# ParsaEsmati/SEA

Hardware: AMD Instinct MI355X
Metric: rollout steps/sec (full-context forward, recompute mode) on cylinder_flow-shaped fields (higher is better)
Workload: dtype bf16

## Files before the change

include/sea_hip.h:

```cpp
#ifndef SEA_HIP_H
#define SEA_HIP_H

#include <stddef.h>
#include <stdint.h>

#ifdef __cplusplus
extern "C" {
#endif

#define SEA_ABI_VERSION 8

enum { SEA_F32 = 0, SEA_BF16 = 1 };

enum {
    SEA_OK = 0,
    SEA_EINVAL = -1,
    SEA_ELAUNCH = -2,
    SEA_EUNSUPPORTED = -3
};

int sea_abi_version(void);
const char* sea_last_error(void);
const char* sea_last_form(int* a, int* b);
int sea_struct_sizes(int* out, int cap);
// ... 368 lines not shown
    int64_t p_stride;
    int32_t S, M, N, ldp, ldr, ldc32, ldcact;
    float bias_scale;
} SeaSplitkGroup;
int sea_splitk_finish(const SeaSplitkGroup* groups, int n_groups, int dtype, void* stream);

#define SEA_MAX_AQKV_GROUPS 4
typedef struct {
    const float* X;
    const float* cond;
    const float* w1;
    const float* b1;
    const void* W2c;
    const float* b2c;
    const float* gamma;
    const float* beta;
    const void* Wqkv;
    const float* bqkv;
    void* Q;
    void* K;
    void* Vt;
    int32_t ldx, ldw2c, ldw, M, E, N3;
    const float* w13;
    const float* b13;
    const void* W3;
    const float* b3;
    void* mod3;
    int32_t ldw3, ldmod3;
    uint32_t* memo_stamps;
    void* memo_mods;
    const uint32_t* memo_epoch;
    int32_t* memo_count;
    uint32_t* memo_rows;
    int32_t ldmemo, pad_;
} SeaAdalnQkv;
int sea_adaln_qkv(const SeaAdalnQkv* groups, int n_groups, const SeaQkvCommon* common, const SeaGemmGroup* riders, int n_riders, const SeaSiluGroup* silu, int n_silu,
                  const float* silu_c, int silu_M, const SeaIbParams* ib, float eps, int dtype, void* stream);

#define SEA_CHAIN_MAX_PROJ 6
#define SEA_CHAIN_MAX_GROUPS 3
typedef struct {
    const void* att[SEA_XTAIL_MAX_SEG];
    const void* Wp[SEA_XTAIL_MAX_SEG];
    const void* a2;
    const void* W2;
    const float* b2;
    const float* Xin;
    float* X;
    void* Xact;
    int32_t n_seg, ldatt, ldwp, lda2, ldw2, ldxin, ldx, ldxact;
    int32_t M, D, E, has_down, n_proj;
    float bias_scale;
    SeaGemmNormGroup down;
    SeaQkvGroup proj[SEA_CHAIN_MAX_PROJ];
} SeaRowChain;

int sea_row_chain(const SeaRowChain* params, int n_groups, const SeaQkvCommon* common, float eps, int dtype, void* stream);
struct SeaIbParams_;
int sea_row_chain_riders(const SeaRowChain* params, int n_groups, const SeaQkvCommon* common, const SeaGemmGroup* riders, int n_riders, int tile0, int n_tiles,
                         const struct SeaIbParams_* ib, float eps, int dtype, void* stream);

enum { SEA_OP_GEMM = 1, SEA_OP_QKV = 2, SEA_OP_ATTN = 3, SEA_OP_NORM = 4, SEA_OP_SILU = 5, SEA_OP_IB = 6, SEA_OP_CONVERT = 8, SEA_OP_GEMM_NORM = 9, SEA_OP_XTAIL = 10, SEA_OP_MLP1 = 11, SEA_OP_MLP2 = 13, SEA_OP_GEMM_FEW = 14, SEA_OP_QKV_FEW = 15, SEA_OP_CHAIN = 16, SEA_OP_ADALN = 17, SEA_OP_MLPB = 18, SEA_OP_AQKV = 19, SEA_OP_SPLITK = 20 };
typedef struct {
    int32_t op, n, dtype, i0, i1, i2, i3;
    float f0;
    const void* p0;
    const void* p1;
    int64_t l0, l1, l2, l3;
} SeaLaunchRec;
int sea_run_list(const SeaLaunchRec* recs, int n_recs, void* stream);

typedef struct {
    void* addr;
    int32_t kind;
    int32_t pad_;
    int64_t base, stride;
} SeaStepPatch;
int sea_run_list_steps(const SeaLaunchRec* recs, int n_recs, const SeaStepPatch* patches, int n_patches, int step0, int n_steps, void* stream);

int sea_unpatchify(const float* in, int64_t sb, int64_t sp, int64_t sf, int64_t sc, const int32_t* index_map, const int32_t* point_slot,
                   const float* scale, const float* shift, float* out, int B, int P, int F, int C, int n_points, void* stream);

int sea_patchify(const float* in, const int32_t* index_map, const float* scale, const float* shift, float* out, int64_t sb, int64_t sp, int64_t sf,
                 int64_t sc, int B, int P, int F, int C_map, int C_out, int n_points, float pad_value, void* stream);

#define SEA_KV_MAX_FIELDS 4
typedef struct {
    const float* gamma;
    const float* beta;
    const void* mod;
    int32_t ldmod, pad_;
} SeaKvNorm;
typedef struct {
// ... 258 lines not shown
```

sea_amd/_native.py:

```python
from __future__ import annotations

import ctypes as C
import os
from typing import Optional

import torch

_HERE = os.path.dirname(os.path.abspath(__file__))
LIB_PATH = os.path.join(_HERE, "csrc", "libsea_hip.so")

SEA_F32, SEA_BF16 = 0, 1
ABI_VERSION = 8
MAX_GROUPS = 16
CTL_GRAD_NORM, CTL_CLIP, CTL_INV_BC1, CTL_INV_SQRT_BC2, CTL_APPLIED, CTL_STEP, CTL_SKIPPED, CTL_CLIPPED, CTL_WORDS = range(9)
MAX_ATTN_PROBLEMS = 8
MAX_NORM_GROUPS = 16
MAX_SILU_GROUPS = 24

_vp, _i32, _i64, _f32 = C.c_void_p, C.c_int32, C.c_int64, C.c_float


class SeaDropout(C.Structure):
    _fields_ = [("seed", C.c_uint32), ("stream", C.c_uint32), ("thr", _i32), ("mode", _i32)]

# ... 84 lines not shown

class SeaLaunchRec(C.Structure):
    _fields_ = [("op", _i32), ("n", _i32), ("dtype", _i32), ("i0", _i32), ("i1", _i32), ("i2", _i32), ("i3", _i32), ("f0", _f32),
                ("p0", _vp), ("p1", _vp), ("l0", _i64), ("l1", _i64), ("l2", _i64), ("l3", _i64)]

MAX_GEMM_NORM_GROUPS = 8


class SeaGemmNormGroup(C.Structure):
    _fields_ = [("A", _vp), ("W", _vp), ("bias", _vp), ("R", _vp), ("C32", _vp), ("mod", _vp), ("gamma", _vp), ("beta", _vp),
                ("Y32", _vp), ("Yact", _vp), ("mean", _vp), ("rstd", _vp),
                ("lda", _i32), ("ldw", _i32), ("ldr", _i32), ("ldc32", _i32), ("ldmod", _i32), ("ldy32", _i32), ("ldyact", _i32),
                ("M", _i32), ("N", _i32), ("K", _i32),
                ("n_seg", _i32), ("a_seg_stride", _i64), ("bias_scale", _f32), ("ldcact", _i32), ("Cact", _vp),
                ("ib_c", _vp), ("ib_w1", _vp), ("ib_b1", _vp), ("ib_lnw", _vp), ("ib_lnb", _vp), ("ib_w2", _vp), ("ib_b2", _vp),
                ("ib_h", _i32), ("pad_", _i32)]


XTAIL_MAX_SEG = 4
XTAIL_MAX_GROUPS = 4
MAX_SILU_IB = 4


class SeaExchangeTail(C.Structure):
    _fields_ = [("att", _vp * XTAIL_MAX_SEG), ("Wp", _vp * XTAIL_MAX_SEG), ("Wup", _vp), ("bup", _vp), ("X", _vp), ("Xact", _vp),
                ("n_seg", _i32), ("ldatt", _i32), ("ldwp", _i32), ("ldwup", _i32), ("ldx", _i32), ("ldxact", _i32),
                ("M", _i32), ("D", _i32), ("E", _i32), ("has_down", _i32), ("bias_scale", _f32),
                ("down", SeaGemmNormGroup)]


CHAIN_MAX_PROJ = 6
CHAIN_MAX_GROUPS = 3
CHAIN_MAX_RIDERS = 8


class SeaRowChain(C.Structure):
    _fields_ = [("att", _vp * XTAIL_MAX_SEG), ("Wp", _vp * XTAIL_MAX_SEG), ("a2", _vp), ("W2", _vp), ("b2", _vp), ("Xin", _vp), ("X", _vp), ("Xact", _vp),
                ("n_seg", _i32), ("ldatt", _i32), ("ldwp", _i32), ("lda2", _i32), ("ldw2", _i32), ("ldxin", _i32), ("ldx", _i32), ("ldxact", _i32),
                ("M", _i32), ("D", _i32), ("E", _i32), ("has_down", _i32), ("n_proj", _i32), ("bias_scale", _f32),
                ("down", SeaGemmNormGroup), ("proj", SeaQkvGroup * CHAIN_MAX_PROJ)]


MAX_ADALN_GROUPS = 16


class SeaAdalnGroup(C.Structure):
    _fields_ = [("A", _vp), ("W", _vp), ("bias", _vp), ("X", _vp), ("gamma", _vp), ("beta", _vp), ("Yact", _vp), ("Y32", _vp), ("mean", _vp), ("rstd", _vp),
                ("lda", _i32), ("ldw", _i32), ("ldx", _i32), ("ldyact", _i32), ("ldy32", _i32), ("M", _i32), ("d", _i32), ("K", _i32)]


MAX_SPLITK_GROUPS = 8


class SeaEncBlock(C.Structure):
    _fields_ = [(n, _vp) for n in ("Zin", "Zout", "wqkv", "bqkv", "wo", "w1", "b1", "lnw", "lnb", "w2", "b2", "g1", "g2", "dZout", "dZin",
                                   "n1", "dqkv", "att", "dz1", "n2", "dh", "hg", "dz2", "u1", "u2", "u3w", "u3b", "ws")] + \
                [("ws_floats", _i64), ("B", _i32), ("P", _i32), ("W", _i32), ("H", _i32), ("eps", _f32), ("pad_", _i32)]


class SeaSplitkGroup(C.Structure):
    _fields_ = [("P", _vp), ("bias", _vp), ("R", _vp), ("C32", _vp), ("Cact", _vp), ("p_stride", _i64), ("S", _i32), ("M", _i32), ("N", _i32), ("ldp", _i32),
                ("ldr", _i32), ("ldc32", _i32), ("ldcact", _i32), ("bias_scale", _f32)]


MAX_AQKV_GROUPS = 4
AQKV_MAX_SILU = 8
# ... 188 lines not shown
    L.sea_rownorm.argtypes = [C.POINTER(SeaNormGroup), C.c_int, C.c_int, C.c_int, C.c_int, C.c_int, C.c_float, C.c_int, _vp]
    L.sea_gemm_fewrows.argtypes = [C.POINTER(SeaGemmGroup), C.POINTER(SeaNormGroup), C.c_int, C.c_int, C.c_int, C.c_float, C.c_int, _vp]
    L.sea_gemm_fewrows.restype = C.c_int
    L.sea_qkv_rope_fewrows.argtypes = [C.POINTER(SeaQkvGroup), C.POINTER(SeaNormGroup), C.c_int, C.POINTER(SeaQkvCommon), C.c_float, C.c_int, _vp]
    L.sea_qkv_rope_fewrows.restype = C.c_int
    L.sea_silu_outer.argtypes = [C.POINTER(SeaSiluGroup), C.c_int, _vp, C.c_int, C.c_int, _vp]
    L.sea_ib_add.argtypes = [C.POINTER(SeaIbParams), _vp]
    L.sea_convert_f32_to_act.argtypes = [_vp, _i64, _vp, _i64, _i64, _i64, C.c_int, _vp]
    L.sea_selftest_mfma.restype = C.c_int
    L.sea_wgrad_grouped.argtypes = [C.POINTER(SeaWgradGroup), C.c_int, C.c_int, _vp]
    L.sea_transpose_weights.argtypes = [_vp, _vp, C.c_int, _vp, _vp, C.c_int, C.c_int, _vp]
    L.sea_rownorm_bwd.argtypes = [C.POINTER(SeaNormBwdGroup), C.c_int, C.c_int, C.c_int, C.c_int, C.c_int, C.c_int, C.c_int, C.c_int, _vp, _i64, _vp]
    L.sea_silu_outer_bwd.argtypes = [C.POINTER(SeaSiluBwdGroup), C.c_int, _vp, C.c_int, C.c_int, _vp, _i64, _vp]
    L.sea_ib_bwd.argtypes = [C.POINTER(SeaIbBwdParams), _vp]
    L.sea_silu_outer_bwd_dc.argtypes = [C.POINTER(SeaSiluBwdGroup), C.c_int, _vp, _vp, C.c_int, C.c_int, _vp, _i64, _vp]
    L.sea_silu_outer_bwd_dc_ws_floats.argtypes = [C.POINTER(SeaSiluBwdGroup), C.c_int, C.c_int]
    L.sea_silu_outer_bwd_dc_ws_floats.restype = _i64
    L.sea_ib_bwd_dc.argtypes = [C.POINTER(SeaIbBwdParams), _vp, _vp]
    L.sea_attention_bwd.argtypes = [C.POINTER(SeaAttnBwdParams), C.c_int, _vp]
    L.sea_dropout_mask.argtypes = [_vp, _i64, _i64, C.c_uint32, C.c_uint32, _i32, _vp]
    L.sea_dropout_mask.restype = C.c_int
    L.sea_unpatchify.argtypes = [_vp, _i64, _i64, _i64, _i64, _vp, _vp, _vp, _vp, _vp, C.c_int, C.c_int, C.c_int, C.c_int, C.c_int, _vp]
    L.sea_unpatchify.restype = C.c_int
    L.sea_gemm_rownorm.argtypes = [C.POINTER(SeaGemmNormGroup), C.c_int, C.c_float, C.c_int, _vp]
    L.sea_gemm_rownorm.restype = C.c_int
    L.sea_exchange_tail.argtypes = [C.POINTER(SeaExchangeTail), C.c_int, C.c_float, C.c_int, _vp]
    L.sea_exchange_tail.restype = C.c_int
    L.sea_gemm_adaln.argtypes = [C.POINTER(SeaAdalnGroup), C.c_int, C.c_float, C.c_int, _vp]
    L.sea_gemm_adaln.restype = C.c_int
    L.sea_row_chain.argtypes = [C.POINTER(SeaRowChain), C.c_int, C.POINTER(SeaQkvCommon), C.c_float, C.c_int, _vp]
    L.sea_row_chain.restype = C.c_int
    L.sea_row_chain_riders.argtypes = [C.POINTER(SeaRowChain), C.c_int, C.POINTER(SeaQkvCommon), C.POINTER(SeaGemmGroup), C.c_int, C.c_int, C.c_int, C.POINTER(SeaIbParams), C.c_float, C.c_int, _vp]
    L.sea_row_chain_riders.restype = C.c_int
    L.sea_patchify.argtypes = [_vp, _vp, _vp, _vp, _vp, _i64, _i64, _i64, _i64, C.c_int, C.c_int, C.c_int, C.c_int, C.c_int, C.c_int, C.c_float, _vp]
    L.sea_patchify.restype = C.c_int
    L.sea_silu_outer_ib.argtypes = [C.POINTER(SeaSiluGroup), C.c_int, _vp, C.c_int, C.c_int, _vp, C.c_int, _vp]
    L.sea_silu_outer_ib.restype = C.c_int
    L.sea_mlp_fc1_ln_gelu.argtypes = [C.POINTER(SeaMlpGroup), C.c_int, C.c_float, C.c_int, _vp]
    L.sea_mlp_fc1_ln_gelu.restype = C.c_int
    L.sea_mlp_fc2_proj_norm.argtypes = [C.POINTER(SeaMlp2Group), C.c_int, C.c_float, C.c_int, _vp]
    L.sea_mlp_fc2_proj_norm.restype = C.c_int
    L.sea_mlp_block.argtypes = [C.POINTER(SeaMlpGroup), C.POINTER(SeaMlp2Group), C.c_int, C.c_float, C.c_int, _vp]
    L.sea_mlp_block.restype = C.c_int
    L.sea_adaln_qkv.argtypes = [C.POINTER(SeaAdalnQkv), C.c_int, C.POINTER(SeaQkvCommon), C.POINTER(SeaGemmGroup), C.c_int, C.POINTER(SeaSiluGroup), C.c_int, _vp, C.c_int,
                                C.POINTER(SeaIbParams), C.c_float, C.c_int, _vp]
    L.sea_adaln_qkv.restype = C.c_int
    L.sea_splitk_finish.argtypes = [C.POINTER(SeaSplitkGroup), C.c_int, C.c_int, _vp]
    L.sea_splitk_finish.restype = C.c_int
    L.sea_encoder_block_ws_floats.argtypes = [C.c_int, C.c_int, C.c_int]
    L.sea_encoder_block_ws_floats.restype = _i64
    for name in ("sea_encoder_block_fwd", "sea_encoder_block_bwd"):
        getattr(L, name).argtypes = [C.POINTER(SeaEncBlock), C.c_int, _vp]
        getattr(L, name).restype = C.c_int
    L.sea_run_list.argtypes = [C.POINTER(SeaLaunchRec), C.c_int, _vp]
    L.sea_run_list.restype = C.c_int
    L.sea_run_list_steps.argtypes = [C.POINTER(SeaLaunchRec), C.c_int, C.POINTER(SeaStepPatch), C.c_int, C.c_int, C.c_int, _vp]
    L.sea_run_list_steps.restype = C.c_int
    L.sea_kv_rollout.argtypes = [C.POINTER(SeaKvGlobal), C.POINTER(SeaKvLayer), C.c_int, C.c_int, C.c_uint32, C.c_int, _vp]
    L.sea_kv_rollout.restype = C.c_int
    L.sea_kv_arena_words.argtypes = [C.POINTER(SeaKvGlobal)]
    L.sea_kv_arena_words.restype = C.c_int64
    L.sea_kv_debug_stamps.argtypes = [_vp]
    L.sea_kv_debug_stamps.restype = None
    L.sea_kv_cache_fill.argtypes = [C.POINTER(SeaKvFill), C.c_int, C.c_int, _vp]
    L.sea_kv_cache_fill.restype = C.c_int
    L.sea_kv_cache_fork.argtypes = [C.POINTER(SeaKvFork), C.c_int, C.c_int, _vp]
# ... 26 lines not shown
    L.sea_ensemble_verify_ws_bytes.restype = _i64
    for name in ("sea_attention_bwd", "sea_wgrad_grouped", "sea_transpose_weights", "sea_rownorm_bwd", "sea_silu_outer_bwd", "sea_ib_bwd",
                 "sea_silu_outer_bwd_dc", "sea_ib_bwd_dc"):
        getattr(L, name).restype = C.c_int
    L.sea_mse_fwd_bwd.argtypes = [_vp, _vp, _vp, _vp, _vp, C.c_int, _i64, C.c_float, _vp]
    L.sea_relative_mse.argtypes = [_vp, _vp, _vp, _i64, C.c_int, _vp]
    L.sea_adamw_flat.argtypes = [_vp, _vp, _vp, _vp, _vp, C.c_int, _i64, C.c_float, C.c_float, C.c_float, C.c_float, C.c_float,
                                 C.c_int, C.c_float, _vp]
    L.sea_grad_norm_ctl.argtypes = [_vp, _i64, C.c_float, C.c_float, C.c_int, C.c_float, C.c_float, _vp, C.c_int, _vp, _vp]
    L.sea_adamw_flat_ctl.argtypes = [_vp, _vp, _vp, _vp, _vp, C.c_int, _i64, C.c_float, C.c_float, C.c_float, C.c_float, C.c_float,
                                     C.c_float, _vp, _vp]
    for name in ("sea_gemm_grouped", "sea_qkv_rope_grouped", "sea_attention_fwd", "sea_rownorm", "sea_silu_outer",
                 "sea_ib_add", "sea_convert_f32_to_act", "sea_device_info", "sea_mse_fwd_bwd", "sea_relative_mse",
                 "sea_adamw_flat", "sea_grad_norm_ctl", "sea_adamw_flat_ctl"):
        getattr(L, name).restype = C.c_int
    if L.sea_abi_version() != ABI_VERSION:
        raise NativeLibraryError(f"{LIB_PATH}: ABI version {L.sea_abi_version()} != {ABI_VERSION}; rebuild (python -m sea_amd.build --force)")
    _lib = L
    return L


ABI_STRUCTS = (SeaGemmGroup, SeaQkvGroup, SeaQkvCommon, SeaAttnProblem, SeaAttnParams, SeaNormGroup, SeaSiluGroup,
               SeaIbParams, SeaWgradGroup, SeaNormBwdGroup, SeaSiluBwdGroup, SeaIbBwdParams, SeaAttnBwdProblem, SeaAttnBwdParams,
               SeaDropout, SeaLaunchRec, SeaGemmNormGroup, SeaExchangeTail, SeaMlpGroup, SeaMlp2Group, SeaKvNorm, SeaKvField, SeaKvPair, SeaKvLayer, SeaKvGlobal, SeaStepPatch, SeaRowChain, SeaAdalnGroup, SeaAdalnQkv, SeaSplitkGroup, SeaEncBlock,
               SeaKvFill, SeaKvFork)

EXPORTED_SYMBOLS = (
    "sea_abi_version", "sea_last_error", "sea_last_form", "sea_struct_sizes", "sea_device_info", "sea_gemm_grouped", "sea_qkv_rope_grouped",
    "sea_attention_fwd", "sea_rownorm", "sea_silu_outer", "sea_ib_add", "sea_convert_f32_to_act", "sea_selftest_mfma",
    "sea_mse_fwd_bwd", "sea_relative_mse", "sea_adamw_flat", "sea_grad_norm_ctl", "sea_adamw_flat_ctl",
    "sea_wgrad_grouped", "sea_transpose_weights", "sea_rownorm_bwd", "sea_silu_outer_bwd", "sea_ib_bwd",
    "sea_attention_bwd", "sea_dropout_mask", "sea_run_list", "sea_run_list_steps", "sea_unpatchify", "sea_gemm_rownorm", "sea_exchange_tail", "sea_patchify", "sea_silu_outer_ib", "sea_mlp_fc1_ln_gelu", "sea_mlp_fc2_proj_norm", "sea_kv_rollout", "sea_kv_arena_words", "sea_kv_debug_stamps",
    "sea_kv_cache_fill", "sea_kv_cache_fork", "sea_kv_cache_gather", "sea_decode_mse", "sea_decode_member_sse", "sea_decode_member_moments", "sea_decode_sensor_sse", "sea_decode_sensor_grad", "sea_resample_systematic", "sea_enkf_transform", "sea_enkf_transform_gram", "sea_decode_member_gram", "sea_ensemble_mix", "sea_ensemble_verify", "sea_ensemble_verify_ws_bytes",
    "sea_gemm_fewrows", "sea_qkv_rope_fewrows", "sea_row_chain", "sea_row_chain_riders", "sea_gemm_adaln", "sea_mlp_block", "sea_adaln_qkv", "sea_splitk_finish",
    "sea_encoder_block_ws_floats", "sea_encoder_block_fwd", "sea_encoder_block_bwd",
    "sea_silu_outer_bwd_dc", "sea_silu_outer_bwd_dc_ws_floats", "sea_ib_bwd_dc",
)


def check(rc: int, what: str = "") -> None:
    if rc != 0:
        msg = lib().sea_last_error()
        raise RuntimeError(f"libsea_hip {what} failed (code {rc}): {msg.decode() if msg else '?'}")


def dtype_code(dt: torch.dtype) -> int:
    if dt == torch.float32:
        return SEA_F32
    if dt == torch.bfloat16:
        return SEA_BF16
    raise ValueError(f"sea_amd: activation dtype must be float32 or bfloat16, got {dt}")


def require_gpu(t: torch.Tensor, name: str = "tensor") -> None:
    if not t.is_cuda:
        raise RuntimeError(
            f"sea_amd: {name} is on {t.device}; this path runs only on an MI355X through libsea_hip.so "
            "(no CPU fallback — the CPU oracle lives under oracle/ for tests only)")


def require_same_operand(out: torch.Tensor, target: torch.Tensor, what: str, f32: bool = False) -> None:
    if target.shape != out.shape:
        raise ValueError(f"sea_amd: {what}: target shape {tuple(target.shape)} does not match output shape {tuple(out.shape)}")
    if target.device != out.device:
        raise ValueError(f"sea_amd: {what}: target is on {target.device}, output on {out.device}")
    if f32 and target.dtype != torch.float32:
        raise ValueError(f"sea_amd: {what}: target dtype {target.dtype} must be torch.float32 (output shape {tuple(out.shape)})")
# ... 9 lines not shown
```

sea_amd/csrc/adaln_qkv.hip:

```cpp
#include "gemm_tile.hpp"
#include "ib_rows.hpp"
#include <stdlib.h>

#define SEA_AQKV_MAX_SILU 8

struct AqkvLaunch {
    SeaAdalnQkv g[SEA_MAX_AQKV_GROUPS];
    int tile_start[SEA_MAX_AQKV_GROUPS + 1];
    int n_groups;
    float eps;
    SeaQkvCommon c;
    ChainRiderPod rg[SEA_CHAIN_MAX_RIDERS];
    int n_riders, rider_n;
    SeaSiluGroup sg[SEA_AQKV_MAX_SILU];
    int n_silu, silu_wgs, ib_wgs, M_r;
    const float* cond_r;
    SeaIbParams ib;
    unsigned long long* stamps;
    int probe;
};
static_assert(sizeof(AqkvLaunch) <= 4096, "kernel arguments of sea_adaln_qkv");

static unsigned long long* g_aqkv_stamps = nullptr;
extern "C" void sea_aqkv_debug_stamps(unsigned long long* buf) { g_aqkv_stamps = buf; }
// ... 43 lines not shown
};

template <bool HAS3>
__global__ __launch_bounds__(512) void adaln_qkv_kernel(const AqkvLaunch L) {
    using T = __bf16;
    using C = AqkvCfg;
    constexpr int E = C::E, KC = C::KC, BM = C::BM, NW = C::NW, KTA = C::KTA, KTB = C::KTB;
    extern __shared__ __attribute__((aligned(16))) char smem[];
    const int total = L.tile_start[L.n_groups];
    if ((int)blockIdx.x >= total + L.rider_n) {
        const int x = (int)blockIdx.x - total - L.rider_n;
        const int lane_ = threadIdx.x & 63, wave_ = threadIdx.x >> 6;
        uint32_t* rst = L.g[0].memo_stamps != nullptr ? L.g[0].memo_rows : nullptr;
        uint32_t r_c = 0, r_e = 0;
        int r_row = -1;
        if (rst != nullptr) {
            const int per_g_ = (L.M_r + 63) >> 6;
            const int set = x < L.silu_wgs ? x / per_g_ : L.n_silu;
            const int b0 = (x < L.silu_wgs ? x - set * per_g_ : x - L.silu_wgs) * 64;
            rst += (int64_t)set * L.M_r * 2;
            int ok = 1;
            if (wave_ == 0 && b0 + lane_ < L.M_r) {
                r_row = b0 + lane_;
                r_c = __float_as_uint(L.cond_r[r_row]);
                r_e = *L.g[0].memo_epoch;
                const uint2 st = reinterpret_cast<const uint2*>(rst)[r_row];
                ok = st.x == r_c && st.y == r_e;
            }
            const int all_ok = __all(ok);
            if (threadIdx.x == 0) *reinterpret_cast<int*>(smem) = all_ok;
            __syncthreads();
            const bool r_hit = __builtin_amdgcn_readfirstlane(*reinterpret_cast<const int*>(smem)) != 0;
            if (L.g[0].memo_count != nullptr && threadIdx.x == 0) atomicAdd(L.g[0].memo_count + (r_hit ? 0 : 1), 1);
            if (r_hit) return;
            if (r_row >= 0) reinterpret_cast<uint2*>(rst)[r_row] = make_uint2(r_c, r_e);
        }
        if (x < L.silu_wgs) {
            const int per_g = (L.M_r + 63) >> 6;
            const int gy = x / per_g;
            const SeaSiluGroup& S = L.sg[gy];
            const int row0 = (x - gy * per_g) * 64 + wave_ * 8;
            if (row0 >= L.M_r) return;
            float cv[8];
#pragma unroll
            for (int i = 0; i < 8; ++i) cv[i] = L.cond_r[row0 + i < L.M_r ? row0 + i : L.M_r - 1];
            T* out = static_cast<T*>(S.Hid) + (int64_t)row0 * S.ld;
            for (int k = lane_ * 4; k < S.K2; k += 256) {
                float w[4], bb[4];
                load4(S.w1 + k, w);
                load4(S.b1 + k, bb);
#pragma unroll
                for (int i = 0; i < 8; ++i) {
                    if (row0 + i < L.M_r)
                        store4(out + (int64_t)i * S.ld + k, silu_f(w[0] * cv[i] + bb[0]), silu_f(w[1] * cv[i] + bb[1]), silu_f(w[2] * cv[i] + bb[2]), silu_f(w[3] * cv[i] + bb[3]));
                }
            }
        } else {
            const int row0 = (x - L.silu_wgs) * 64 + wave_ * 8;
            for (int i = 0; i < 8; ++i) {
                const int row = row0 + i;
                if (row < L.ib.M) ib_store_row(L.ib, L.cond_r[row], row, lane_);
            }
        }
        return;
    }
    if ((int)blockIdx.x >= total) {
// ... 474 lines not shown
    if (memo && !hit && wave == 0 && lane < 32 && m0 + lane < M) reinterpret_cast<uint2*>(G.memo_stamps)[m0 + lane] = make_uint2(my_c, my_e);
}

extern "C" int sea_adaln_qkv(const SeaAdalnQkv* groups, int n_groups, const SeaQkvCommon* common, const SeaGemmGroup* riders, int n_riders, const SeaSiluGroup* silu, int n_silu,
                             const float* silu_c, int silu_M, const SeaIbParams* ib, float eps, int dtype, void* stream) {
    SEA_REQUIRE(groups != nullptr && common != nullptr && n_groups >= 1 && n_groups <= SEA_MAX_AQKV_GROUPS, "sea_adaln_qkv: n_groups=%d out of range", n_groups);
    const int E = groups[0].E;
    if (dtype != SEA_BF16 || E != AqkvCfg::E || common->H * common->hd != E || (common->hd != 32 && common->hd != 16)) {
        sea_set_error("sea_adaln_qkv: unsupported dtype / shape (dtype=%d E=%d H=%d hd=%d): bf16, E = 256, head dim 16 or 32, H * hd = E", dtype, E, common->H, common->hd);
        return SEA_EUNSUPPORTED;
    }
    SEA_REQUIRE(common->rope && common->T >= 1 && common->cap >= common->pos0 + common->T && common->pos0 >= 0 && common->cap % 8 == 0, "sea_adaln_qkv: bad rotary table / cache geometry (T=%d pos0=%d cap=%d)",
                common->T, common->pos0, common->cap);
    AqkvLaunch L;
    memset(&L, 0, sizeof(L));
    const bool memo_count = sea_tune("memo_count", 0) != 0;
    int total = 0;
    for (int i = 0; i < n_groups; ++i) {
        const SeaAdalnQkv& G = groups[i];
        SEA_REQUIRE(G.E == E && G.M >= 1 && G.M % common->T == 0, "sea_adaln_qkv[%d]: the groups of a launch share E; M = B * T", i);
        SEA_REQUIRE(G.X && G.cond && G.w1 && G.b1 && G.W2c && G.gamma && G.Wqkv && G.Q && G.K && G.Vt, "sea_adaln_qkv[%d]: null pointer", i);
        SEA_REQUIRE(G.ldx % 4 == 0 && G.ldx >= E && G.ldw2c % 8 == 0 && G.ldw2c >= 2 * E && G.ldw % 8 == 0 && G.ldw >= E, "sea_adaln_qkv[%d]: bad strides", i);
        SEA_REQUIRE(sea_aligned16(G.X) && sea_aligned16(G.w1) && sea_aligned16(G.b1) && sea_aligned16(G.W2c) && sea_aligned16(G.b2c) && sea_aligned16(G.gamma) && sea_aligned16(G.beta) &&
                        sea_aligned16(G.Wqkv) && sea_aligned16(G.bqkv) && sea_aligned16(G.Q) && sea_aligned16(G.K) && sea_aligned16(G.Vt),
                    "sea_adaln_qkv[%d]: pointers must be 16-byte aligned", i);
        SEA_REQUIRE((int64_t)(G.M / common->T) * common->H * common->cap * common->hd < (1ll << 31), "sea_adaln_qkv[%d]: attention tensors must stay below 2^31 elements", i);
        if (G.W3 != nullptr) {
            SEA_REQUIRE(G.w13 && G.b13 && G.mod3 && G.N3 == AqkvCfg::K3 && G.ldw3 % 8 == 0 && G.ldw3 >= G.N3 && G.ldmod3 % 8 == 0 && G.ldmod3 >= G.N3 && sea_aligned16(G.w13) && sea_aligned16(G.b13) &&
                            sea_aligned16(G.W3) && sea_aligned16(G.b3) && sea_aligned16(G.mod3),
                        "sea_adaln_qkv[%d]: third layer: null / misaligned pointer, bad stride, or N3 = %d != 256", i, G.N3);
        }
        if (G.memo_stamps != nullptr) {
            SEA_REQUIRE(G.memo_mods && G.memo_epoch && G.ldmemo % 8 == 0 && G.ldmemo >= 2 * E && sea_aligned16(G.memo_mods) && ((uintptr_t)G.memo_stamps & 7) == 0 &&
                            ((uintptr_t)G.memo_epoch & 3) == 0 && ((uintptr_t)G.memo_count & 3) == 0 && ((uintptr_t)G.memo_rows & 7) == 0,
                        "sea_adaln_qkv[%d]: condition memo: null / misaligned pointer or bad stride (ldmemo=%d)", i, G.ldmemo);
        }
        L.g[i] = G;
        if (!memo_count) L.g[i].memo_count = nullptr;
        L.tile_start[i] = total;
        total += (G.M + 31) / 32;
    }
    L.tile_start[n_groups] = total;
    L.n_groups = n_groups;
    L.eps = eps;
    L.c = *common;
    SEA_REQUIRE(n_riders >= 0 && n_riders <= SEA_CHAIN_MAX_RIDERS && (n_riders == 0 || riders != nullptr), "sea_adaln_qkv: bad rider arguments");
    int rider_total = 0;
    for (int i = 0; i < n_riders; ++i) {
        const SeaGemmGroup& G = riders[i];
        SEA_REQUIRE(G.A && !G.silu_c && G.W && G.Cact && !G.C32 && !G.R && !G.Z && G.act == 0 && G.drop.thr == 0 && G.n_seg == 1, "sea_adaln_qkv: rider %d is not a plain bf16 group (A, W, bias, Cact only)", i);
        SEA_REQUIRE(G.M >= 1 && G.N >= 8 && G.N % 8 == 0 && G.K >= 64 && G.K % 64 == 0 && G.lda % 8 == 0 && G.lda >= G.K && G.ldw % 8 == 0 && G.ldw >= G.K && G.ldcact % 8 == 0 && G.ldcact >= G.N,
                    "sea_adaln_qkv: rider %d: bad shape M=%d N=%d K=%d (whole 64-wide K-tiles) lda=%d ldw=%d ldcact=%d", i, G.M, G.N, G.K, G.lda, G.ldw, G.ldcact);
        SEA_REQUIRE(sea_aligned16(G.A) && sea_aligned16(G.W) && sea_aligned16(G.bias) && sea_aligned16(G.Cact), "sea_adaln_qkv: rider %d: pointers must be 16-byte aligned", i);
        ChainRiderPod& R = L.rg[i];
        R.A = G.A; R.W = G.W; R.bias = G.bias; R.Cact = G.Cact;
        R.lda = G.lda; R.ldw = G.ldw; R.ldcact = G.ldcact; R.M = G.M; R.N = G.N; R.K = G.K;
        R.tile_start = rider_total;
        rider_total += ((G.M + 127) / 128) * ((G.N + 127) / 128);
    }
    L.n_riders = n_riders;
    L.rider_n = rider_total;
    SEA_REQUIRE(n_silu >= 0 && n_silu <= SEA_AQKV_MAX_SILU && (n_silu == 0 || (silu != nullptr && silu_c != nullptr && silu_M >= 1)), "sea_adaln_qkv: bad silu rider arguments (n_silu=%d)", n_silu);
    for (int i = 0; i < n_silu; ++i) {
        SEA_REQUIRE(silu[i].w1 && silu[i].b1 && silu[i].Hid && silu[i].K2 >= 4 && silu[i].K2 % 4 == 0 && silu[i].ld >= silu[i].K2 && silu[i].ld % 4 == 0 && sea_aligned16(silu[i].w1) &&
                        sea_aligned16(silu[i].b1) && sea_aligned16(silu[i].Hid),
                    "sea_adaln_qkv: silu rider %d: null / misaligned pointer or bad shape", i);
        L.sg[i] = silu[i];
// ... 33 lines not shown
```

sea_amd/csrc/chain.hip:

```cpp
#include "norm_epilogue.hpp"
#include "gemm_tile.hpp"
#include "ib_rows.hpp"
#include <stdlib.h>

struct ChainLaunch {
    SeaRowChain p[SEA_CHAIN_MAX_GROUPS];
    SeaQkvCommon c;
    float eps;
    int n_groups;
    unsigned long long* stamps;
    ChainRiderPod rg[SEA_CHAIN_MAX_RIDERS];
    int n_riders, rider_t0, rider_n, ib_wgs;
    SeaIbParams ib;
};
static_assert(sizeof(ChainLaunch) <= 4096, "kernel arguments of sea_row_chain");

static unsigned long long* g_chain_stamps = nullptr;
extern "C" void sea_chain_debug_stamps(unsigned long long* buf) { g_chain_stamps = buf; }

template <int D, int E, int MI>
struct ChainCfg {
    static constexpr int BM = 16 * MI, BKB = 128, BK = 64;
    static constexpr int KTD = D / BK, KTE = E / BK;
    static constexpr int AT_BYTES = BM * E * 2;
    static constexpr int YT_BYTES = BM * D * 2;
    static constexpr int WH_BYTES = E * D * 2;
    static constexpr int ROPE_BYTES = 2048;
    static constexpr int BIAS_BYTES = 4096;
    static constexpr int RED_BYTES = MI * 512;
    static constexpr int LDS_BYTES = AT_BYTES + YT_BYTES + 2 * WH_BYTES + ROPE_BYTES + BIAS_BYTES + RED_BYTES;
    static constexpr int SMAX = E / D;
    static constexpr int NI1 = D / 64, NI2 = E / 64, NI3 = D / 64, NI4 = 2 * D / 64;
    static_assert(E == 2 * D && LDS_BYTES <= 160 * 1024 && SMAX * D * D * 2 <= WH_BYTES && (KTE / 2) * E * BKB <= WH_BYTES && D * E * 2 <= WH_BYTES, "LDS plan of sea_row_chain");
};

__device__ __forceinline__ void glds16_x4(const void* p0, const void* p1, const void* p2, const void* p3, unsigned l0, unsigned l1, unsigned l2, unsigned l3) {
    unsigned keep;
    asm volatile(
        "s_mov_b32 %0, m0\n\t"
        "s_mov_b32 m0, %5\n\ts_nop 0\n\tglobal_load_lds_dwordx4 %1, off\n\t"
        "s_mov_b32 m0, %6\n\ts_nop 0\n\tglobal_load_lds_dwordx4 %2, off\n\t"
        "s_mov_b32 m0, %7\n\ts_nop 0\n\tglobal_load_lds_dwordx4 %3, off\n\t"
        "s_mov_b32 m0, %8\n\ts_nop 0\n\tglobal_load_lds_dwordx4 %4, off\n\t"
        "s_mov_b32 m0, %0"
        : "=&s"(keep) : "v"(p0), "v"(p1), "v"(p2), "v"(p3), "s"(l0), "s"(l1), "s"(l2), "s"(l3) : "memory");
}
// ... 98 lines not shown
    static constexpr const float* ib_b1 = nullptr;
    static constexpr const float* ib_lnw = nullptr;
    static constexpr const float* ib_lnb = nullptr;
    static constexpr const float* ib_w2 = nullptr;
    static constexpr const float* ib_b2 = nullptr;
    static constexpr int ib_h = 0, ldr = 0, ldc32 = 0, ldcact = 0;
    int M, ldmod, ldy32, ldyact;
    const float* bias;
    const void* mod;
    const float* gamma;
    const float* beta;
    float* Y32;
    void* Yact;
    float* mean;
    float* rstd;
};

template <int D, int E, int MI>
__global__ __launch_bounds__(256) void row_chain_kernel(const ChainLaunch L) {
    using T = __bf16;
    using C = ChainCfg<D, E, MI>;
    constexpr int BM = C::BM, KTD = C::KTD, KTE = C::KTE, NI1 = C::NI1, NI2 = C::NI2, NI3 = C::NI3, NI4 = C::NI4, SMAX = C::SMAX;
    constexpr int A_KTS = BM * 128;
    extern __shared__ __attribute__((aligned(16))) char smem[];
    const int tid = threadIdx.x, lane = tid & 63, wave = tid >> 6;
    const int r = lane & 15, g = lane >> 4;
    if ((int)blockIdx.y == L.n_groups) {
        const int x = blockIdx.x;
        if (x < L.rider_n) {
            const int tile = L.rider_t0 + x;
            int gi = 0;
            while (gi + 1 < L.n_riders && tile >= L.rg[gi + 1].tile_start) ++gi;
            const ChainRiderPod& R = L.rg[gi];
            ChainRiderGroup G;
            G.A = R.A; G.W = R.W; G.bias = R.bias; G.Cact = R.Cact;
            G.lda = R.lda; G.ldw = R.ldw; G.ldcact = R.ldcact; G.M = R.M; G.N = R.N; G.K = R.K;
            const int t = tile - R.tile_start;
            const int tiles_n = (R.N + 127) / 128;
            gemm_tile_body<T, 128, 128, true, true, false>(G, t / tiles_n, t % tiles_n, smem, 0);
        } else if (x < L.rider_n + L.ib_wgs) {
            const int row0 = (x - L.rider_n) * 64 + wave * 16;
            for (int i = 0; i < 16; ++i) {
                const int row = row0 + i;
                if (row < L.ib.M) ib_store_row(L.ib, L.ib.c[row], row, lane);
            }
        }
        return;
    }
    ChainParams pl;
    {
        const uint32_t* raw = reinterpret_cast<const uint32_t*>(&L.p[0]) + (size_t)blockIdx.y * (sizeof(SeaRowChain) / 4);
#pragma unroll
        for (int k = 0; k < 4; ++k) {
            const int dw = k * 64 + lane;
            pl.v[k] = dw < (int)(sizeof(SeaRowChain) / 4) ? raw[dw] : 0u;
        }
    }
    const int M = CP_I32(M), S = CP_I32(n_seg);
    const int m0 = blockIdx.x * BM;
    if (m0 >= M) return;
    unsigned long long* stp = L.stamps != nullptr ? L.stamps + (size_t)(blockIdx.y * gridDim.x + blockIdx.x) * 16 : nullptr;
    int stn = 0;
    auto stamp = [&]() {
        if (stp != nullptr && tid == 0 && stn < 16) stp[stn] = wall_clock64();
        ++stn;
    };
    stamp();
    char* AT = smem;
    char* YT = AT + C::AT_BYTES;
    char* WA = YT + C::YT_BYTES;
    char* WB = WA + C::WH_BYTES;
    float* s_rope = reinterpret_cast<float*>(WB + C::WH_BYTES);
    float* s_bias = reinterpret_cast<float*>(reinterpret_cast<char*>(s_rope) + C::ROPE_BYTES);
    float* red = reinterpret_cast<float*>(reinterpret_cast<char*>(s_bias) + C::BIAS_BYTES);
    const unsigned lds0 = __builtin_amdgcn_readfirstlane((unsigned)(uintptr_t)smem);
    const unsigned at_l = lds0, wa_l = lds0 + C::AT_BYTES + C::YT_BYTES, wb_l = wa_l + C::WH_BYTES;
    const int wv = __builtin_amdgcn_readfirstlane(wave);
    const T* W2 = CP_PTR(const T*, W2);
    const int ldw2 = CP_I32(ldw2);
    const bool has_down = CP_I32(has_down) != 0;
    const int n_proj = has_down ? CP_I32(n_proj) : 0;
    const T* Wd = CP_PTR(const T*, down.W);
    const int ldwd = CP_I32(down.ldw);

    if (S > 0) {
        const int ldatt = CP_I32(ldatt), ldwp = CP_I32(ldwp);
#pragma unroll
        for (int s = 0; s < SMAX; ++s) {
            if (s < S) {
                const T* att = reinterpret_cast<const T*>(cp_dyn_u64(pl, CP_DW(att) + 2 * s));
                const T* Wp = reinterpret_cast<const T*>(cp_dyn_u64(pl, CP_DW(Wp) + 2 * s));
                chain_dma_a(att, ldatt, m0, M - 1, BM, KTD, at_l + (unsigned)(s * KTD * A_KTS), wv, lane);
                chain_dma_w(Wp, ldwp, D, 0, KTD, wa_l + (unsigned)(s * D * D * 2), wv, lane);
            }
        }
        chain_dma_w(W2, ldw2, E, 0, KTD, wb_l, wv, lane);
    } else {
        chain_dma_a(CP_PTR(const T*, a2), CP_I32(lda2), m0, M - 1, BM, KTE, at_l, wv, lane);
        chain_dma_w(W2, ldw2, E, 0, KTE / 2, wa_l, wv, lane);
        chain_dma_w(W2, ldw2, E, (KTE / 2) * 64, KTE / 2, wb_l, wv, lane);
    }
    stamp();
    int mrow[MI];
    bool mok[MI];
#pragma unroll
    for (int i = 0; i < MI; ++i) {
        const int m = m0 + i * 16 + r;
        mok[i] = m < M;
        mrow[i] = mok[i] ? m : M - 1;
    }
    const float* b2 = CP_PTR(const float*, b2);
    const float* Xin = CP_PTR(const float*, Xin);
    const int ldxin = CP_I32(ldxin);
    const float bias_scale = CP_F32(bias_scale);
    float bv2[NI2][4], rv2[MI][NI2][4];
#pragma unroll
    for (int j = 0; j < NI2; ++j) {
        const int n = wave * (E / 4) + j * 16 + g * 4;
#pragma unroll
        for (int q = 0; q < 4; ++q) bv2[j][q] = 0.f;
        if (b2 != nullptr) load4(b2 + n, bv2[j]);
#pragma unroll
        for (int i = 0; i < MI; ++i) load4(Xin + (int64_t)mrow[i] * ldxin + n, rv2[i][j]);
    }
    ChainNormGroup<D, E> Gd;
    Gd.M = M;
    Gd.bias = CP_PTR(const float*, down.bias);
    Gd.mod = CP_PTR(const void*, down.mod);
    Gd.ldmod = CP_I32(down.ldmod);
    Gd.gamma = CP_PTR(const float*, down.gamma);
    Gd.beta = CP_PTR(const float*, down.beta);
    Gd.Y32 = CP_PTR(float*, down.Y32);
    Gd.ldy32 = CP_I32(down.ldy32);
    Gd.Yact = CP_PTR(void*, down.Yact);
    Gd.ldyact = CP_I32(down.ldyact);
    Gd.mean = CP_PTR(float*, down.mean);
    Gd.rstd = CP_PTR(float*, down.rstd);
    NormEpilogue<T, NI3, true, true, true> epi3[MI];
    if (has_down) {
#pragma unroll
        for (int i = 0; i < MI; ++i) epi3[i].prefetch(Gd, mrow[i], wave * (D / 4), g);
    }
    const int hd = L.c.hd, hd2 = hd >> 1, Tlen = L.c.T, pos0 = L.c.pos0;
    if (n_proj > 0) {
        for (int idx = tid; idx < BM * hd2; idx += 256) {
            const int i = idx / hd2, k = idx - i * hd2;
            int m = m0 + i;
            m = m < M ? m : M - 1;
            const int t = m % Tlen;
            const float2 cs = reinterpret_cast<const float2*>(L.c.rope)[(int64_t)(pos0 + t) * hd2 + k];
            reinterpret_cast<float2*>(s_rope)[idx] = cs;
        }
        int boff = 0;
        for (int e = 0; e < n_proj; ++e) {
            const int base = CP_DW(proj) + e * (int)(sizeof(SeaQkvGroup) / 4);
            const float* bias = reinterpret_cast<const float*>(cp_dyn_u64(pl, base + QK_DW(bias)));
            const int N = (int)cp_dyn_u32(pl, base + QK_DW(N));
            for (int n = tid; n < N; n += 256) s_bias[boff + n] = bias != nullptr ? bias[n] : 0.f;
            boff += N;
        }
    }
#pragma unroll
    for (int j = 0; j < NI2; ++j)
#pragma unroll
        for (int q = 0; q < 4; ++q) {
            touch(bv2[j][q]);
#pragma unroll
            for (int i = 0; i < MI; ++i) touch(rv2[i][j][q]);
        }
    if (has_down) {
#pragma unroll
        for (int i = 0; i < MI; ++i)
#pragma unroll
            for (int j = 0; j < NI3; ++j)
#pragma unroll
                for (int q = 0; q < 4; ++q) {
                    touch(epi3[i].bv[j][q]); touch(epi3[i].gm[j][q]); touch(epi3[i].bt[j][q]); touch(epi3[i].mw[j][q]); touch(epi3[i].mb[j][q]);
                }
    }
    stamp();
    asm volatile("s_waitcnt vmcnt(0)" ::: "memory");
    __syncthreads();
    stamp();

    f32x4 acc2[MI][NI2];
#pragma unroll
    for (int i = 0; i < MI; ++i)
#pragma unroll
        for (int j = 0; j < NI2; ++j) acc2[i][j] = f32x4{0.f, 0.f, 0.f, 0.f};
    if (S > 0) {
        float gsum[MI][NI1][4];
#pragma unroll
        for (int i = 0; i < MI; ++i)
#pragma unroll
            for (int j = 0; j < NI1; ++j)
#pragma unroll
                for (int q = 0; q < 4; ++q) gsum[i][j][q] = 0.f;
#pragma unroll
        for (int s = 0; s < SMAX; ++s) {
            if (s < S) {
                f32x4 acc1[MI][NI1];
#pragma unroll
                for (int i = 0; i < MI; ++i)
#pragma unroll
                    for (int j = 0; j < NI1; ++j) acc1[i][j] = f32x4{0.f, 0.f, 0.f, 0.f};
                chain_mma<MI, NI1>(AT + s * KTD * A_KTS, A_KTS, WA + s * D * D * 2, D * 128, wave * (D / 4), KTD, NI1, r, g, acc1);
#pragma unroll
                for (int i = 0; i < MI; ++i)
#pragma unroll
                    for (int j = 0; j < NI1; ++j)
#pragma unroll
                        for (int q = 0; q < 4; ++q) gsum[i][j][q] += gelu_erf(acc1[i][j][q]);
            }
        }
#pragma unroll
        for (int i = 0; i < MI; ++i)
#pragma unroll
            for (int j = 0; j < NI1; ++j) {
                const int kk = wave * (D / 4) + j * 16 + g * 4;
                store4(reinterpret_cast<T*>(YT + (kk >> 6) * A_KTS + (i * 16 + r) * 128 + ((((kk & 63) >> 3) ^ (r & 7)) << 4) + (kk & 7) * 2), gsum[i][j][0], gsum[i][j][1], gsum[i][j][2],
                       gsum[i][j][3]);
            }
        lds_barrier();
        if (has_down) chain_dma_w(Wd, ldwd, D, 0, KTE, wa_l, wv, lane);
        chain_mma<MI, NI2>(YT, A_KTS, WB, E * 128, wave * (E / 4), KTD, NI2, r, g, acc2);
    } else {
        chain_mma<MI, NI2>(AT, A_KTS, WA, E * 128, wave * (E / 4), KTE / 2, NI2, r, g, acc2);
        lds_barrier();
        if (has_down) chain_dma_w(Wd, ldwd, D, 0, KTE, wa_l, wv, lane);
        chain_mma<MI, NI2>(AT + (KTE / 2) * A_KTS, A_KTS, WB, E * 128, wave * (E / 4), KTE / 2, NI2, r, g, acc2);
    }
    lds_barrier();
    stamp();
    int e_next = 0;
    auto burst = [&](unsigned half_l, int& e_lo, int& e_hi) {
        e_lo = e_next;
        int bytes = 0;
        while (e_next < n_proj) {
            const int base = CP_DW(proj) + e_next * (int)(sizeof(SeaQkvGroup) / 4);
            const int N = (int)cp_dyn_u32(pl, base + QK_DW(N));
            if (bytes + N * D * 2 > C::WH_BYTES) break;
            chain_dma_w(reinterpret_cast<const T*>(cp_dyn_u64(pl, base + QK_DW(W))), (int)cp_dyn_u32(pl, base + QK_DW(ldw)), N, 0, KTD, half_l + (unsigned)bytes, wv, lane);
            bytes += N * D * 2;
            ++e_next;
        }
        e_hi = e_next;
    };
    int b_lo[2] = {0, 0}, b_hi[2] = {0, 0};
    if (n_proj > 0) burst(wb_l, b_lo[0], b_hi[0]);
    float v2[MI][NI2][4];
#pragma unroll
    for (int i = 0; i < MI; ++i)
#pragma unroll
        for (int j = 0; j < NI2; ++j) {
            const int n = wave * (E / 4) + j * 16 + g * 4;
#pragma unroll
            for (int q = 0; q < 4; ++q) v2[i][j][q] = acc2[i][j][q] + bv2[j][q] * bias_scale + rv2[i][j][q];
            store4(reinterpret_cast<T*>(AT + (n >> 6) * A_KTS + (i * 16 + r) * 128 + ((((n & 63) >> 3) ^ (r & 7)) << 4) + (n & 7) * 2), v2[i][j][0], v2[i][j][1], v2[i][j][2], v2[i][j][3]);
        }
    asm volatile("s_waitcnt vmcnt(0)" ::: "memory");
    stamp();
    {
        float* X = CP_PTR(float*, X);
        T* Xact = CP_PTR(T*, Xact);
        const int ldx = CP_I32(ldx), ldxact = CP_I32(ldxact);
#pragma unroll
        for (int i = 0; i < MI; ++i) {
            if (!mok[i]) continue;
            float* xr_ = X + (int64_t)(m0 + i * 16 + r) * ldx + wave * (E / 4) + g * 4;
            T* xa_ = Xact != nullptr ? Xact + (int64_t)(m0 + i * 16 + r) * ldxact + wave * (E / 4) + g * 4 : nullptr;
#pragma unroll
            for (int j = 0; j < NI2; ++j) {
                store4(xr_ + j * 16, v2[i][j][0], v2[i][j][1], v2[i][j][2], v2[i][j][3]);
                if (xa_ != nullptr) store4(xa_ + j * 16, v2[i][j][0], v2[i][j][1], v2[i][j][2], v2[i][j][3]);
            }
        }
    }
    stamp();
    if (!has_down) return;
    lds_barrier();
    {
        f32x4 acc3[MI][NI3];
#pragma unroll
        for (int i = 0; i < MI; ++i)
#pragma unroll
            for (int j = 0; j < NI3; ++j) acc3[i][j] = f32x4{0.f, 0.f, 0.f, 0.f};
        chain_mma<MI, NI3>(AT, A_KTS, WA, D * 128, wave * (D / 4), KTE, NI3, r, g, acc3);
#pragma unroll
        for (int i = 0; i < MI; ++i)
            epi3[i].finish(Gd, acc3[i], m0 + i * 16 + r, wave * (D / 4), r, g, wave, L.eps, red + i * 128, n_proj > 0 ? YT + i * 16 * 128 : nullptr, A_KTS);
    }
    stamp();
    if (n_proj == 0) return;
    const int Hh = L.c.H, cap = L.c.cap, Ea = Hh * hd;
    const int hd_sh = 31 - __builtin_clz((unsigned)hd);
    uint32_t offq[MI], offk[MI], offv[MI];
#pragma unroll
    for (int i = 0; i < MI; ++i) {
        const int b_ = mrow[i] / Tlen;
        const int t_ = mrow[i] - b_ * Tlen;
        offq[i] = (uint32_t)((b_ * Hh * Tlen + t_) << hd_sh);
        offk[i] = (uint32_t)((b_ * Hh * cap + pos0 + t_) << hd_sh);
        offv[i] = (uint32_t)(b_ * Hh * hd * cap + pos0 + t_);
    }
    const float q_scale = L.c.q_scale;
    int cur = 0;
    int boff = 0;
    for (;;) {
        asm volatile("s_waitcnt vmcnt(0)" ::: "memory");
        lds_barrier();
        stamp();
        if (e_next < n_proj) burst(cur ? wb_l : wa_l, b_lo[cur ^ 1], b_hi[cur ^ 1]);
        else b_lo[cur ^ 1] = b_hi[cur ^ 1] = 0;
        const char* Wh = cur ? WA : WB;
        int woff = 0;
        for (int e = b_lo[cur]; e < b_hi[cur]; ++e) {
            const int base = CP_DW(proj) + e * (int)(sizeof(SeaQkvGroup) / 4);
            const int N = (int)cp_dyn_u32(pl, base + QK_DW(N));
            if (N == D) {
                constexpr int NQ = D / 64;
                f32x4 acc4[MI][NQ];
#pragma unroll
                for (int i = 0; i < MI; ++i)
#pragma unroll
                    for (int j = 0; j < NQ; ++j) acc4[i][j] = f32x4{0.f, 0.f, 0.f, 0.f};
                chain_mma<MI, NQ>(YT, A_KTS, Wh + woff, D * 128, wave * (D / 4), KTD, NQ, r, g, acc4);
// ... 48 lines not shown
                        const int h = nb >> hd_sh;
                        const uint32_t hoffv = (uint32_t)(((h << hd_sh) + dd) * cap);
                        const float4 bq = *reinterpret_cast<const float4*>(s_bias + boff + D + nb + g * 4);
#pragma unroll
                        for (int i = 0; i < MI; ++i) {
                            if (!mok[i]) continue;
                            const float v0 = acc4[i][j][0] + bq.x, v1 = acc4[i][j][1] + bq.y, v2q = acc4[i][j][2] + bq.z, v3 = acc4[i][j][3] + bq.w;
                            T* d_ = vt + (offv[i] + hoffv);
                            d_[0] = (T)v0;
                            d_[(uint32_t)cap] = (T)v1;
                            d_[2u * (uint32_t)cap] = (T)v2q;
                            d_[3u * (uint32_t)cap] = (T)v3;
                            if (vo != nullptr) store4(vo + (offk[i] + ((uint32_t)(h * cap) << hd_sh) + (uint32_t)dd), v0, v1, v2q, v3);
                        }
                    }
                }
            }
            woff += N * D * 2;
            boff += N;
        }
        stamp();
        if (b_hi[cur ^ 1] == b_lo[cur ^ 1]) break;
        cur ^= 1;
    }
}


template <typename K>
static int set_lds_chain(K kernel, int bytes) {
    return hipFuncSetAttribute(reinterpret_cast<const void*>(kernel), hipFuncAttributeMaxDynamicSharedMemorySize, bytes) == hipSuccess ? 0 : -1;
}

static int row_chain_launch(const SeaRowChain* params, int n_groups, const SeaQkvCommon* common, const SeaGemmGroup* riders, int n_riders, int tile0, int n_tiles,
                            const SeaIbParams* ib, float eps, int dtype, void* stream);

extern "C" int sea_row_chain(const SeaRowChain* params, int n_groups, const SeaQkvCommon* common, float eps, int dtype, void* stream) {
    return row_chain_launch(params, n_groups, common, nullptr, 0, 0, 0, nullptr, eps, dtype, stream);
}

extern "C" int sea_row_chain_riders(const SeaRowChain* params, int n_groups, const SeaQkvCommon* common, const SeaGemmGroup* riders, int n_riders, int tile0, int n_tiles,
                                    const SeaIbParams* ib, float eps, int dtype, void* stream) {
    return row_chain_launch(params, n_groups, common, riders, n_riders, tile0, n_tiles, ib, eps, dtype, stream);
}

static int row_chain_launch(const SeaRowChain* params, int n_groups, const SeaQkvCommon* common, const SeaGemmGroup* riders, int n_riders, int tile0, int n_tiles,
                            const SeaIbParams* ib, float eps, int dtype, void* stream) {
    SEA_REQUIRE(params != nullptr && n_groups >= 1 && n_groups <= SEA_CHAIN_MAX_GROUPS, "sea_row_chain: n_groups=%d out of range", n_groups);
    ChainLaunch L;
    memset(&L, 0, sizeof(L));
    L.eps = eps;
    L.n_groups = n_groups;
    L.stamps = g_chain_stamps;
    SEA_REQUIRE(n_riders >= 0 && n_riders <= SEA_CHAIN_MAX_RIDERS && (n_riders == 0 || riders != nullptr) && tile0 >= 0 && n_tiles >= 0, "sea_row_chain_riders: bad rider arguments");
    int rider_total = 0;
    for (int i = 0; i < n_riders; ++i) {
        const SeaGemmGroup& G = riders[i];
        SEA_REQUIRE(dtype == SEA_BF16 && G.A && !G.silu_c && G.W && G.Cact && !G.C32 && !G.R && !G.Z && G.act == 0 && G.drop.thr == 0 && G.n_seg == 1,
                    "sea_row_chain_riders[%d]: a rider is a plain bf16 group (A, W, bias, Cact only)", i);
        SEA_REQUIRE(G.M >= 1 && G.N >= 8 && G.N % 8 == 0 && G.K >= 64 && G.K % 64 == 0 && G.lda % 8 == 0 && G.lda >= G.K && G.ldw % 8 == 0 && G.ldw >= G.K && G.ldcact % 8 == 0 && G.ldcact >= G.N,
                    "sea_row_chain_riders[%d]: bad shape M=%d N=%d K=%d (whole 64-wide K-tiles) lda=%d ldw=%d ldcact=%d", i, G.M, G.N, G.K, G.lda, G.ldw, G.ldcact);
        SEA_REQUIRE(sea_aligned16(G.A) && sea_aligned16(G.W) && sea_aligned16(G.bias) && sea_aligned16(G.Cact), "sea_row_chain_riders[%d]: pointers must be 16-byte aligned", i);
        ChainRiderPod& R = L.rg[i];
        R.A = G.A; R.W = G.W; R.bias = G.bias; R.Cact = G.Cact;
        R.lda = G.lda; R.ldw = G.ldw; R.ldcact = G.ldcact; R.M = G.M; R.N = G.N; R.K = G.K;
        R.tile_start = rider_total;
        rider_total += ((G.M + 127) / 128) * ((G.N + 127) / 128);
    }
    SEA_REQUIRE(tile0 + n_tiles <= rider_total, "sea_row_chain_riders: tiles [%d, %d) of %d", tile0, tile0 + n_tiles, rider_total);
    L.n_riders = n_riders; L.rider_t0 = tile0; L.rider_n = n_tiles;
    if (ib != nullptr) {
        SEA_REQUIRE(ib->X[0] && ib->c && ib->w1 && ib->M >= 1 && ib->E >= 4 && ib->E % 4 == 0 && ib->ldx >= ib->E && ib->mode >= 0 && ib->mode <= 2 &&
                        (ib->mode != 0 || (ib->b1 && ib->lnw && ib->lnb && ib->w2 && ib->b2 && ib->h >= 1 && ib->h <= 64)),
                    "sea_row_chain_riders: bad info-bottleneck rider");
        L.ib = *ib;
        L.ib_wgs = (ib->M + 63) / 64;
    }
    const int D = params[0].D, E = params[0].E;
    int m_max = 0, any_proj = 0;
    for (int gi = 0; gi < n_groups; ++gi) {
        const SeaRowChain& P = params[gi];
        const bool shape_ok = (P.D == 128 && P.E == 256) || (P.D == 64 && P.E == 128);
        if (dtype != SEA_BF16 || !shape_ok || P.n_seg < 0 || P.n_seg * P.D > P.E) {
            sea_set_error("sea_row_chain: unsupported dtype / shape (dtype=%d D=%d E=%d n_seg=%d): bf16, (D,E) in {(128,256),(64,128)}, n_seg*D <= E", dtype, P.D, P.E, P.n_seg);
            return SEA_EUNSUPPORTED;
        }
        SEA_REQUIRE(P.D == D && P.E == E, "sea_row_chain[%d]: the groups of a launch share their widths", gi);
        SEA_REQUIRE(P.M >= 1 && P.W2 && P.Xin && P.X && sea_aligned16(P.W2) && sea_aligned16(P.b2) && sea_aligned16(P.Xin) && sea_aligned16(P.X) && sea_aligned16(P.Xact),
                    "sea_row_chain[%d]: null / misaligned pointer", gi);
        const int K2 = P.n_seg > 0 ? P.D : P.E;
        SEA_REQUIRE(P.ldw2 % 8 == 0 && P.ldw2 >= K2 && P.ldxin % 4 == 0 && P.ldxin >= P.E && P.ldx % 4 == 0 && P.ldx >= P.E && (!P.Xact || (P.ldxact % 4 == 0 && P.ldxact >= P.E)),
                    "sea_row_chain[%d]: bad strides", gi);
        if (P.n_seg == 0) SEA_REQUIRE(P.a2 && sea_aligned16(P.a2) && P.lda2 % 8 == 0 && P.lda2 >= P.E, "sea_row_chain[%d]: a2: null / misaligned / short rows", gi);
        else SEA_REQUIRE(P.ldatt % 8 == 0 && P.ldatt >= P.D && P.ldwp % 8 == 0 && P.ldwp >= P.D, "sea_row_chain[%d]: bad segment strides", gi);
        for (int s = 0; s < P.n_seg; ++s)
            SEA_REQUIRE(P.att[s] && sea_aligned16(P.att[s]) && P.Wp[s] && sea_aligned16(P.Wp[s]), "sea_row_chain[%d]: segment %d: null / misaligned operand", gi, s);
        L.p[gi] = P;
        SEA_REQUIRE(P.n_proj >= 0 && P.n_proj <= SEA_CHAIN_MAX_PROJ && (P.n_proj == 0 || P.has_down), "sea_row_chain[%d]: n_proj=%d (projections read the normalised rows: has_down)", gi, P.n_proj);
        if (P.has_down) {
            const SeaGemmNormGroup& G = P.down;
            SEA_REQUIRE(G.W && G.gamma && (G.Y32 || G.Yact || P.n_proj > 0) && G.ldw % 8 == 0 && G.ldw >= P.E, "sea_row_chain[%d]: down: null pointer or bad ldw", gi);
            SEA_REQUIRE((!G.Y32 || (G.ldy32 % 4 == 0 && G.ldy32 >= P.D)) && (!G.Yact || (G.ldyact % 4 == 0 && G.ldyact >= P.D)) && (!G.mod || (G.ldmod % 4 == 0 && G.ldmod >= 2 * P.D)),
                        "sea_row_chain[%d]: down: bad output / modulation strides", gi);
            SEA_REQUIRE(sea_aligned16(G.W) && sea_aligned16(G.bias) && sea_aligned16(G.mod) && sea_aligned16(G.gamma) && sea_aligned16(G.beta) && sea_aligned16(G.Y32) && sea_aligned16(G.Yact),
                        "sea_row_chain[%d]: down: pointers must be 16-byte aligned", gi);
            SeaGemmNormGroup& Gd = L.p[gi].down;
            Gd.M = P.M; Gd.N = P.D; Gd.K = P.E; Gd.n_seg = 1; Gd.bias_scale = 1.0f;
            Gd.R = nullptr; Gd.C32 = nullptr; Gd.Cact = nullptr; Gd.ib_c = nullptr;
        }
        int nsum = 0;
        for (int e = 0; e < P.n_proj; ++e) {
            const SeaQkvGroup& Q = P.proj[e];
            SEA_REQUIRE(common != nullptr, "sea_row_chain: projections need the SeaQkvCommon");
            const int Ea = common->H * common->hd;
            SEA_REQUIRE(Q.W && sea_aligned16(Q.W) && sea_aligned16(Q.bias) && Q.ldw % 8 == 0 && Q.ldw >= P.D && Q.K == P.D && (Q.N == P.D / 2 || Q.N == P.D || Q.N == 2 * P.D) && Q.N % 64 == 0,
                        "sea_row_chain[%d]: projection %d: W [N, D] with N in {D, 2D} (multiples of 64), K = D (N=%d K=%d ldw=%d)", gi, e, Q.N, Q.K, Q.ldw);
            SEA_REQUIRE((Q.N == P.D && Q.col0 == 0) || (Q.N == 2 * P.D && Q.col0 == P.D), "sea_row_chain[%d]: projection %d: a q entry (N = D, col0 = 0) or a k | v entry (N = 2 D, col0 = D), not N=%d col0=%d", gi, e, Q.N, Q.col0);
            SEA_REQUIRE(Q.col0 >= 0 && Q.col0 % 16 == 0 && Q.col0 + Q.N <= 3 * Ea && Ea == P.D, "sea_row_chain[%d]: projection %d: columns [%d,%d) outside [0,%d) / H hd != D", gi, e, Q.col0, Q.col0 + Q.N, 3 * Ea);
            const bool hasq = Q.col0 < Ea, hask = Q.col0 < 2 * Ea && Q.col0 + Q.N > Ea, hasv = Q.col0 + Q.N > 2 * Ea;
            SEA_REQUIRE((!hasq || Q.Qout) && (!hask || Q.Kout) && (!hasv || Q.Vtout) && sea_aligned16(Q.Qout) && sea_aligned16(Q.Kout) && sea_aligned16(Q.Vtout) && sea_aligned16(Q.Vout),
                        "sea_row_chain[%d]: projection %d: missing / misaligned output pointer", gi, e);
            nsum += Q.N;
            any_proj = 1;
        }
        SEA_REQUIRE(nsum * 4 <= 4096, "sea_row_chain[%d]: the projections' output columns sum to %d (at most 1024)", gi, nsum);
        m_max = P.M > m_max ? P.M : m_max;
    }
    if (any_proj) {
        const SeaQkvCommon& c = *common;
        if (c.hd < 16 || (c.hd & (c.hd - 1)) != 0) {
            sea_set_error("sea_row_chain: unsupported head dim %d (a power of two >= 16: a 16-column block of a projection lies inside one head)", c.hd);
            return SEA_EUNSUPPORTED;
        }
        SEA_REQUIRE(c.rope != nullptr && c.H >= 1 && c.hd >= 4 && c.hd % 4 == 0 && c.T >= 1 && c.pos0 >= 0 && c.cap >= c.pos0 + c.T && m_max % c.T == 0,
                    "sea_row_chain: bad common H=%d hd=%d T=%d pos0=%d cap=%d (M=%d)", c.H, c.hd, c.T, c.pos0, c.cap, m_max);
        SEA_REQUIRE((int64_t)(m_max / c.T + 1) * c.H * c.cap * c.hd < ((int64_t)1 << 31) && (int64_t)(c.pos0 + c.T) * (c.hd / 2) < ((int64_t)1 << 30),
                    "sea_row_chain: attention tensors too large for 32-bit element offsets");
        L.c = c;
    }
    const int forced = sea_tune("chain_rows", 0);
    int mi = ((m_max + 15) / 16) * n_groups <= 256 ? 1 : 2;
    if (forced == 16) mi = 1;
    if (forced == 32) mi = 2;
    if (any_proj && 16 * mi * (L.c.hd / 2) * 8 > 2048) {
        if (mi == 2 && 16 * (L.c.hd / 2) * 8 <= 2048) mi = 1;
        else {
            sea_set_error("sea_row_chain: head dim %d: the rotary rows of a workgroup do not fit their LDS block", L.c.hd);
            return SEA_EUNSUPPORTED;
        }
    }
    hipStream_t s = static_cast<hipStream_t>(stream);
    const int chain_x = (m_max + 16 * mi - 1) / (16 * mi), rider_x = L.rider_n + L.ib_wgs;
    const dim3 grid(chain_x > rider_x ? chain_x : rider_x, n_groups + (rider_x > 0 ? 1 : 0));
    constexpr int rider_lds = GemmMainloop<__bf16, 128, 128>::DMA_LDS_BYTES;
#define LAUNCH_CH(DD, EE, MM)                                                                                   \
    do {                                                                                                        \
        constexpr int own_ = ChainCfg<DD, EE, MM>::LDS_BYTES;                                                   \
        constexpr int max_ = own_ > rider_lds ? own_ : rider_lds;                                               \
        static int once = set_lds_chain(row_chain_kernel<DD, EE, MM>, max_);                                    \
        (void)once;                                                                                             \
        row_chain_kernel<DD, EE, MM><<<grid, dim3(256), (L.rider_n > 0 ? max_ : own_), s>>>(L);                 \
    } while (0)
    if (D == 128) { if (mi == 1) LAUNCH_CH(128, 256, 1); else LAUNCH_CH(128, 256, 2); }
    else { if (mi == 1) LAUNCH_CH(64, 128, 1); else LAUNCH_CH(64, 128, 2); }
#undef LAUNCH_CH
    SEA_CHECK_LAUNCH("sea_row_chain");
    return SEA_OK;
}
```

sea_amd/csrc/core.hip:

```cpp
#include "sea_common.hpp"
#include <stdlib.h>

static thread_local char g_err[512] = "";

void sea_set_error(const char* fmt, ...) {
    va_list ap;
    va_start(ap, fmt);
    vsnprintf(g_err, sizeof(g_err), fmt, ap);
    va_end(ap);
}

int sea_tune(const char* key, int dflt) {
    const char* e = getenv("SEA_TUNE");
    if (e == nullptr) return dflt;
    const size_t n = strlen(key);
    for (const char* p = e; *p;) {
        while (*p == ',' || *p == ' ') ++p;
        if (strncmp(p, key, n) == 0 && p[n] == '=') return atoi(p + n + 1);
        while (*p && *p != ',') ++p;
    }
    return dflt;
}

static thread_local const char* g_form = "";
// ... 28 lines not shown
    const int sizes[] = {(int)sizeof(SeaGemmGroup), (int)sizeof(SeaQkvGroup), (int)sizeof(SeaQkvCommon), (int)sizeof(SeaAttnProblem),
                         (int)sizeof(SeaAttnParams), (int)sizeof(SeaNormGroup), (int)sizeof(SeaSiluGroup), (int)sizeof(SeaIbParams),
                         (int)sizeof(SeaWgradGroup), (int)sizeof(SeaNormBwdGroup), (int)sizeof(SeaSiluBwdGroup), (int)sizeof(SeaIbBwdParams),
                         (int)sizeof(SeaAttnBwdProblem), (int)sizeof(SeaAttnBwdParams), (int)sizeof(SeaDropout), (int)sizeof(SeaLaunchRec),
                         (int)sizeof(SeaGemmNormGroup), (int)sizeof(SeaExchangeTail), (int)sizeof(SeaMlpGroup), (int)sizeof(SeaMlp2Group), (int)sizeof(SeaKvNorm), (int)sizeof(SeaKvField),
                         (int)sizeof(SeaKvPair), (int)sizeof(SeaKvLayer), (int)sizeof(SeaKvGlobal), (int)sizeof(SeaStepPatch), (int)sizeof(SeaRowChain), (int)sizeof(SeaAdalnGroup), (int)sizeof(SeaAdalnQkv), (int)sizeof(SeaSplitkGroup), (int)sizeof(SeaEncBlock),
                         (int)sizeof(SeaKvFill), (int)sizeof(SeaKvFork)};
    const int n = (int)(sizeof(sizes) / sizeof(sizes[0]));
    for (int i = 0; i < n && i < cap; ++i) out[i] = sizes[i];
    return n;
}

extern "C" int sea_run_list(const SeaLaunchRec* recs, int n_recs, void* stream) {
    SEA_REQUIRE(recs != nullptr && n_recs >= 0, "sea_run_list: bad arguments");
    for (int i = 0; i < n_recs; ++i) {
        const SeaLaunchRec& R = recs[i];
        int rc;
        switch (R.op) {
            case SEA_OP_GEMM: rc = sea_gemm_grouped(static_cast<const SeaGemmGroup*>(R.p0), R.n, R.dtype, stream); break;
            case SEA_OP_QKV: rc = sea_qkv_rope_grouped(static_cast<const SeaQkvGroup*>(R.p0), R.n, static_cast<const SeaQkvCommon*>(R.p1), R.dtype, stream); break;
            case SEA_OP_ATTN: rc = sea_attention_fwd(static_cast<const SeaAttnParams*>(R.p0), R.dtype, stream); break;
            case SEA_OP_NORM: rc = sea_rownorm(static_cast<const SeaNormGroup*>(R.p0), R.n, R.i0, R.i1, R.i2, R.i3, R.f0, R.dtype, stream); break;
            case SEA_OP_SILU: rc = sea_silu_outer_ib(static_cast<const SeaSiluGroup*>(R.p0), R.n, static_cast<const float*>(R.p1), R.i0, R.dtype,
                                                     reinterpret_cast<const SeaIbParams*>(static_cast<intptr_t>(R.l0)), (int)R.l1, stream); break;
            case SEA_OP_IB: rc = sea_ib_add(static_cast<const SeaIbParams*>(R.p0), stream); break;
            case SEA_OP_CONVERT: rc = sea_convert_f32_to_act(static_cast<const float*>(R.p0), R.l0, const_cast<void*>(R.p1), R.l1, R.l2, R.l3, R.dtype, stream); break;
            case SEA_OP_GEMM_NORM: rc = sea_gemm_rownorm(static_cast<const SeaGemmNormGroup*>(R.p0), R.n, R.f0, R.dtype, stream); break;
            case SEA_OP_XTAIL: rc = sea_exchange_tail(static_cast<const SeaExchangeTail*>(R.p0), R.n, R.f0, R.dtype, stream); break;
            case SEA_OP_MLP1: rc = sea_mlp_fc1_ln_gelu(static_cast<const SeaMlpGroup*>(R.p0), R.n, R.f0, R.dtype, stream); break;
            case SEA_OP_MLP2: rc = sea_mlp_fc2_proj_norm(static_cast<const SeaMlp2Group*>(R.p0), R.n, R.f0, R.dtype, stream); break;
            case SEA_OP_GEMM_FEW: rc = sea_gemm_fewrows(static_cast<const SeaGemmGroup*>(R.p0), static_cast<const SeaNormGroup*>(R.p1), R.n, R.i0, R.i1, R.f0, R.dtype, stream); break;
            case SEA_OP_QKV_FEW: rc = sea_qkv_rope_fewrows(static_cast<const SeaQkvGroup*>(R.p0), reinterpret_cast<const SeaNormGroup*>(R.l0), R.n, static_cast<const SeaQkvCommon*>(R.p1), R.f0,
                                                           R.dtype, stream); break;
            case SEA_OP_CHAIN: rc = sea_row_chain_riders(static_cast<const SeaRowChain*>(R.p0), R.n, static_cast<const SeaQkvCommon*>(R.p1), reinterpret_cast<const SeaGemmGroup*>(static_cast<intptr_t>(R.l0)),
                                                         R.i0, R.i1, R.i2, reinterpret_cast<const SeaIbParams*>(static_cast<intptr_t>(R.l1)), R.f0, R.dtype, stream); break;
            case SEA_OP_ADALN: rc = sea_gemm_adaln(static_cast<const SeaAdalnGroup*>(R.p0), R.n, R.f0, R.dtype, stream); break;
            case SEA_OP_SPLITK: rc = sea_splitk_finish(static_cast<const SeaSplitkGroup*>(R.p0), R.n, R.dtype, stream); break;
            case SEA_OP_MLPB: rc = sea_mlp_block(static_cast<const SeaMlpGroup*>(R.p0), static_cast<const SeaMlp2Group*>(R.p1), R.n, R.f0, R.dtype, stream); break;
            case SEA_OP_AQKV: rc = sea_adaln_qkv(static_cast<const SeaAdalnQkv*>(R.p0), R.n, static_cast<const SeaQkvCommon*>(R.p1), reinterpret_cast<const SeaGemmGroup*>(static_cast<intptr_t>(R.l0)), R.i0,
                                                 reinterpret_cast<const SeaSiluGroup*>(static_cast<intptr_t>(R.l1)), R.i1, reinterpret_cast<const float*>(static_cast<intptr_t>(R.l2)), R.i2,
                                                 reinterpret_cast<const SeaIbParams*>(static_cast<intptr_t>(R.l3)), R.f0, R.dtype, stream); break;
            default: sea_set_error("sea_run_list[%d]: unknown op %d", i, R.op); return SEA_EINVAL;
        }
        if (rc != SEA_OK) return rc;
    }
    return SEA_OK;
}

extern "C" int sea_run_list_steps(const SeaLaunchRec* recs, int n_recs, const SeaStepPatch* patches, int n_patches, int step0, int n_steps, void* stream) {
    SEA_REQUIRE(recs != nullptr && n_recs >= 0 && n_patches >= 0 && (n_patches == 0 || patches != nullptr) && step0 >= 0 && n_steps >= 0, "sea_run_list_steps: bad arguments");
    for (int i = 0; i < n_patches; ++i)
        SEA_REQUIRE(patches[i].addr != nullptr && (patches[i].kind == 0 || patches[i].kind == 1), "sea_run_list_steps: patch %d: null address or bad kind %d", i, patches[i].kind);
    for (int s = step0; s < step0 + n_steps; ++s) {
        for (int i = 0; i < n_patches; ++i) {
            const SeaStepPatch& P = patches[i];
            const int64_t v = P.base + (int64_t)s * P.stride;
            if (P.kind == 0) *static_cast<int32_t*>(P.addr) = (int32_t)v;
            else *static_cast<int64_t*>(P.addr) = v;
        }
        const int rc = sea_run_list(recs, n_recs, stream);
        if (rc != SEA_OK) return rc;
    }
    return SEA_OK;
}

extern "C" int sea_device_info(int* cu_count, char* arch, int arch_len) {
    hipDeviceProp_t prop;
    int dev = 0;
// ... 72 lines not shown
```

sea_amd/csrc/norm_epilogue.hpp:

```cpp
#pragma once
#include "gemm_core.hpp"

__device__ __forceinline__ float group_sum4(float x) {
    x += __shfl_xor(x, 16);
    x += __shfl_xor(x, 32);
    return x;
}

#define SEA_IB_FUSED_MAX_H 8

template <typename GT>
__device__ __forceinline__ void ib_hidden(const GT& G, int row, float (&hid)[SEA_IB_FUSED_MAX_H]) {
    const int h = G.ib_h;
    const float cv = G.ib_c[row];
    float pre[SEA_IB_FUSED_MAX_H], mean = 0.f, var = 0.f;
#pragma unroll
    for (int k = 0; k < SEA_IB_FUSED_MAX_H; ++k) {
        pre[k] = k < h ? G.ib_w1[k] * cv + G.ib_b1[k] : 0.f;
        mean += pre[k];
    }
    mean /= (float)h;
#pragma unroll
    for (int k = 0; k < SEA_IB_FUSED_MAX_H; ++k) {
        pre[k] = k < h ? pre[k] - mean : 0.f;
// ... 120 lines not shown
#pragma unroll
        for (int j = 0; j < NI; ++j) {
            if (col0 + j * 16 < N) {
#pragma unroll
                for (int q = 0; q < 4; ++q) {
                    const float c = v[j][q] - mean;
                    sq4[q] = fma1(c, c, sq4[q]);
                }
            }
        }
        float sq = add1(add1(sq4[0], sq4[1]), add1(sq4[2], sq4[3]));
        sq = group_sum4(sq);
        if constexpr (XWAVE) {
            if (g == 0) red[64 + wave * 16 + r] = sq;
            norm_barrier<RAWBAR>();
            sq = (red[64 + r] + red[80 + r]) + (red[96 + r] + red[112 + r]);
        }
        const float rstd = 1.0f / sqrtf(sq * inv_n + eps);
        if (lds_y != nullptr) {
#pragma unroll
            for (int j = 0; j < NI; ++j) {
                const int n = col0 + j * 16 + g * 4;
                if (n >= N) continue;
                if constexpr (!HOIST) fetch_post(G, 0, n, mc);
                const int js = HOIST ? j : 0;
                float o[4];
#pragma unroll
                for (int q = 0; q < 4; ++q) {
                    const float gq = G.mod != nullptr ? gm[js][q] + 1.0f + mw[js][q] : gm[js][q];
                    const float bq = G.mod != nullptr ? bt[js][q] + mb[js][q] : bt[js][q];
                    o[q] = (v[j][q] - mean) * rstd * gq + bq;
                }
                store4(reinterpret_cast<__bf16*>(lds_y + (n >> 6) * lds_kts + r * 128 + ((((n & 63) >> 3) ^ (r & 7)) << 4) + (n & 7) * 2), o[0], o[1], o[2], o[3]);
            }
        }
        if (!mok) return;
        if (g == 0 && (!XWAVE || wave == 0)) {
            if (G.mean != nullptr) G.mean[m] = mean;
            if (G.rstd != nullptr) G.rstd[m] = rstd;
        }
        float* y32 = G.Y32 != nullptr ? G.Y32 + (int64_t)m * G.ldy32 : nullptr;
        T* yact = G.Yact != nullptr ? static_cast<T*>(G.Yact) + (int64_t)m * G.ldyact : nullptr;
        const bool has_mod = G.mod != nullptr;
#pragma unroll
        for (int j = 0; j < NI; ++j) {
            const int n = col0 + j * 16 + g * 4;
            const int js = HOIST ? j : 0;
            if (n >= N) continue;
            if constexpr (!HOIST) fetch_post(G, 0, n, mc);
            float o[4];
#pragma unroll
            for (int q = 0; q < 4; ++q) {
                const float gq = has_mod ? gm[js][q] + 1.0f + mw[js][q] : gm[js][q];
                const float bq = has_mod ? bt[js][q] + mb[js][q] : bt[js][q];
                o[q] = (v[j][q] - mean) * rstd * gq + bq;
            }
            if (y32 != nullptr) store4(y32 + n, o[0], o[1], o[2], o[3]);
            if (yact != nullptr) store4(yact + n, o[0], o[1], o[2], o[3]);
        }
    }
};

__device__ __forceinline__ void glds16_gn(const void* gsrc, unsigned lds_addr) {
    unsigned keep;
    asm volatile("s_mov_b32 %0, m0\n\ts_mov_b32 m0, %2\n\ts_nop 0\n\tglobal_load_lds_dwordx4 %1, off\n\ts_mov_b32 m0, %0"
                 : "=&s"(keep) : "v"(gsrc), "s"(lds_addr) : "memory");
}
```

sea_amd/engine.py:

```python
from __future__ import annotations

import os

import ctypes as C
import re
from typing import Dict, List, Optional, Tuple

import torch

from . import _native as N
from . import _switches
from . import ops
from . import ptrcheck
from .plan_forms import INFERENCE, resolve_forms

_QKV = re.compile(r"^(.*\.)(k|q|v)\.(weight|bias)$")
_QKV_RANK = {("q", "weight"): 0, ("k", "weight"): 1, ("v", "weight"): 2, ("q", "bias"): 3, ("k", "bias"): 4, ("v", "bias"): 5}


_BIND_KEYS = {"X_is_x": ("_x_patches", "X"), "R_is_x": ("_x_patches", "R"), "Xin_is_x": ("_x_patches", "Xin"), "Y_is_out": ("_out_patches", "Y32"),
              "dY_is_dout": ("_dout_patches", "dY")}


KV_NO_POOL = ("sea_amd: the KV-cache rollout does not cover exchange_mode='pool' (its sinusoidal positions are relative to the window); "
# ... 170 lines not shown
                                                  self._t_desc.data_ptr(), self._t_tiles.data_ptr(), self._t_desc.shape[0], self._t_total,
                                                  N.stream_ptr()), "weight transpose")
            self._synced_T_version = v

    def actT(self, name: str, rows: Optional[int] = None) -> torch.Tensor:
        o, shp = self.offsets[name]
        r = shp[0] if rows is None else rows
        return self.flat_actT[o:o + r * shp[1]].view(shp[1], r)

    def sync(self, force: bool = False) -> None:
        if self.act_dtype == torch.float32:
            return
        v = self.flat32._version
        if force or v != self._synced_version or self._data_reads != _WatchedParameter.reads:
            self._data_reads = _WatchedParameter.reads
            N.check(N.lib().sea_convert_f32_to_act(self.flat32.data_ptr(), self.n_total, self.flat_act.data_ptr(), self.n_total, 1,
                                                   self.n_total, N.dtype_code(self.act_dtype), N.stream_ptr()), "weight shadow")
            self._synced_version = v
            self.weights_changed()

    def weights_changed(self) -> None:
        self.memo_epoch.add_(1)


class _Rec:
    __slots__ = ("fn", "args", "name", "keep", "lane")

    def __init__(self, fn, args, name, keep=None, lane=0):
        self.fn, self.args, self.name, self.keep, self.lane = fn, list(args), name, keep, lane


class _Riders:

    def __init__(self, arr, tiles: int, hosts: int, caps: Optional[Tuple[int, ...]]):
        self.arr, self.tiles, self.done = arr, tiles, 0
        self.hosts_total = self.hosts_left = hosts
        self.caps, self.host_no = caps, 0

    def take(self):
        left = self.tiles - self.done
        if left <= 0:
            return None
        if self.caps is not None:
            take = min(left, self.caps[self.host_no] if self.host_no < len(self.caps) else 0)
            self.host_no += 1
        else:
            take = left if self.hosts_left <= 1 else min(left, (self.tiles + self.hosts_total - 1) // self.hosts_total)
            self.hosts_left -= 1
        t0, self.done = self.done, self.done + take
        return self.arr, len(self.arr), t0, take


class Plan:
    kind = INFERENCE

    def __init__(self, eng: "TemporalEngine", B: int, T: int, mode: str = "full", save_for_backward: bool = False, cond=None):
        assert mode in ("full", "step")
        self.eng, self.B, self.T, self.mode = eng, B, T, mode
        self._cond_src = cond
        self._hoisted: List[Tuple[object, str, int, int]] = []
        m = eng.model
        self.F, self.H, self.L = m.num_variables, m.n_heads, m.num_layers
        self.Eo, self.E = m.embed_dim, m.internal_embed_dim
        self.concat = m.ib_addition_mode.lower() == "concat"
        self.ib_dim = self.E - self.Eo if self.concat else self.E
        self.D = m.down_dim
        self.S = m.mlp_hidden
        self.M = B * T
        self.dt = eng.act_dtype
        self.code = N.dtype_code(self.dt)
        self.adaln = m.LN_type.lower() == "adaln"
        self.cap = _round_up(m.max_len, 8) if mode == "step" else _round_up(T, 8)
        self.pos0 = 0
        self.records: List[_Rec] = []
        self._cur: List[_Rec] = self.records
        self._keep: List[object] = []
        self._x_patches: List[Tuple[object, str, int]] = []
        self._out_patches: List[Tuple[object, str, int]] = []
        self._c_patches: List[Tuple[object, object]] = []
        self._pos_structs: List[object] = []
        self._drop_structs: List[object] = []
        self._bound = (None, None, None)
        self._bound_tensors = None
        self._audited = False
        self._lane = 0
        self._lane_streams: Dict[int, torch.cuda.Stream] = {}
        self._zero_ib: Optional[torch.Tensor] = None
        self.forms = resolve_forms(m, B, T, mode, self.dt, self.kind, hoisted=cond is not None, hoisted_ib=cond is not None and len(cond.ibufs) == self.L)
        self._mods: Dict[str, torch.Tensor] = {}
        self._riders: Optional[_Riders] = None
        self._front = None
        self.memo_count: Optional[torch.Tensor] = None
        self._build()
        self._find_hoisted()
        self._clist = None
        self._compile_list()

    def _find_hoisted(self) -> None:
        src = self._cond_src
        if src is None:
            return
        spans = []
        for t in list(src.mods.values()) + list(src.ibufs):
            step = self.M * t.stride(0) * t.element_size()
            spans.append((t.data_ptr(), t.data_ptr() + step, step))
        for r in self.records:
            if r.fn is None:
                continue
            roots = [a for a in r.args if isinstance(a, (C.Structure, C.Array))] + ([r.keep] if r.keep is not None else [])
            seen = set()
            for root in roots:
                for st in ptrcheck._walk_structs(root):
                    for path, pval in ptrcheck.iter_pointers(st):
                        name = path[1:]
                        if "[" in name or (C.addressof(st), name) in seen:
                            continue
                        for lo, hi, step in spans:
                            if lo <= pval < hi:
                                seen.add((C.addressof(st), name))
                                self._hoisted.append((st, name, pval, step))
                                break
        self._keep.append(src)

    def set_hoisted_step(self, s: int) -> None:
        for st, field, base, step in self._hoisted:
# ... 104 lines not shown
        common = N.SeaQkvCommon(rope.data_ptr(), self.H, hd, self.T, self.pos0, self.cap, ops.q_scale(hd))
        self._pos_structs.append(common)
        return common

    def _qkv_few(self, groups: List[dict], rope: torch.Tensor, hd: int, name: str, pre=None) -> None:
        n = len(groups)
        assert n <= N.FEW_MAX_GROUPS
        arr = self._array(N.SeaQkvGroup, groups, lambda g, A=None, **d: ops.fill_qkv_group(g, A, M=self.M, **d))
        pa = self._norm_specs(pre, n)
        common = self._qkv_common(rope, hd)
        self._cur.append(self._rec(N.lib().sea_qkv_rope_fewrows, [arr, pa, n, C.byref(common), 1e-5, self.code], name, (arr, pa, common)))

    def _gemm_norm(self, groups: List[dict], name: str) -> None:
        self._grouped(N.lib().sea_gemm_rownorm, N.SeaGemmNormGroup, groups, N.MAX_GEMM_NORM_GROUPS, ops.fill_gemm_norm_group, name, 1e-5, self.code)

    def _xtail(self, att, Wp, Wup, bup, bias_scale, X, down, name: str) -> None:
        P = (N.SeaExchangeTail * 1)()
        ops.fill_exchange_tail(P[0], att, Wp, Wup, bup, bias_scale, X, None, down)
        self._cur.append(self._rec(N.lib().sea_exchange_tail, [P, 1, 1e-5, self.code], name, P))

    def _adaln(self, groups: List[dict], name: str) -> None:
        self._grouped(N.lib().sea_gemm_adaln, N.SeaAdalnGroup, groups, N.MAX_ADALN_GROUPS, ops.fill_adaln_group, name, 1e-5, self.code)

    def _chain(self, groups: List[dict], rope: torch.Tensor, hd: int, name: str) -> None:
        for s in range(0, len(groups), N.CHAIN_MAX_GROUPS):
            chunk = groups[s:s + N.CHAIN_MAX_GROUPS]
            arr = self._array(N.SeaRowChain, chunk, ops.fill_row_chain)
            common = self._qkv_common(rope, hd)
            rd = self._riders.take() if s == 0 and self._riders is not None else None
            if rd is None:
                self._cur.append(self._rec(N.lib().sea_row_chain, [arr, len(chunk), C.byref(common), 1e-5, self.code], name, (arr, common)))
            else:
                rarr, n_r, t0, nt = rd
                self._cur.append(self._rec(N.lib().sea_row_chain_riders, [arr, len(chunk), C.byref(common), rarr, n_r, t0, nt, None, 1e-5, self.code], name, (arr, common, rarr, None)))

    def _qkv(self, groups: List[dict], rope: torch.Tensor, hd: int, name: str) -> None:
        arr = self._array(N.SeaQkvGroup, groups, lambda g, **d: ops.fill_qkv_group(g, M=self.M, **d))
        common = self._qkv_common(rope, hd)
        self._cur.append(self._rec(N.lib().sea_qkv_rope_grouped, [arr, len(groups), C.byref(common), self.code], name, (arr, common)))

    def _attn(self, problems: List[dict], hd: int, ldo: int, name: str, drop=None, src_len: Optional[int] = None) -> None:
        for s in range(0, len(problems), N.MAX_ATTN_PROBLEMS):
            P = N.SeaAttnParams()
            ops.fill_attn_params(P, problems[s:s + N.MAX_ATTN_PROBLEMS], self.B, self.H, hd, self.T, self.pos0 + self.T, self.cap, self.pos0,
                                 (self.eng.model.src_len if src_len is None else src_len), ldo, drop=((0, drop[1] + s, drop[0]) if drop is not None else None))
            if drop is not None:
                self._drop_structs.append(P)
            self._pos_structs.append(P)
            self._cur.append(self._rec(N.lib().sea_attention_fwd, [C.byref(P), self.code], name, P))

    def _cond_mods(self, ib_fold=()) -> Dict[str, torch.Tensor]:
        P, F, E, D, M, L, fm = self.eng.params, self.F, self.E, self.D, self.M, N.lib(), self.forms
        mods: Dict[str, torch.Tensor] = {}
        if not self.adaln:
            return mods
        if self._cond_src is not None:
            return {pre: t[:M] for pre, t in self._cond_src.mods.items()}
        first, rest = [], []
        for l in range(self.L):
            pre = f"blocks.{l}."
            for i in range(F):
                (first if l == 0 else rest).append((f"{pre}ln.exp.{i}.0.", E))
                rest.append((f"{pre}ln.exp.{i}.2.", E))
            if self.eng.model.exchange_mode != "simple":
                for i in range(F):
                    rest.append((f"{pre}ln_cross.{i}.", D))
        for i in range(F):
# ... 13 lines not shown
            self._c_patches.append((rec.args, 2))
            self._cur.append(rec)
        if fm.riders:
            front = first + [(pre_, d) for pre_, d in rest if "ln_cross." in pre_]
            later = [(pre_, d) for pre_, d in rest if (pre_, d) not in front]
            silu_groups, hids = [], {}
            for pre_, d in front + later:
                mods[pre_] = self._buf(M, 2 * d)
                if fm.front_chain and ((pre_, d) in first or (fm.front3 and "ln_cross." in pre_)):
                    continue
                hids[pre_] = self._buf(M, 2 * d)
                silu_groups.append(dict(w1=P.f32_vec(pre_ + "cond_mlp.0.weight", 2 * d), b1=P.f32_vec(pre_ + "cond_mlp.0.bias"), Hid=hids[pre_]))
            front_rows = None
            if fm.front3:
                sarr = (N.SeaSiluGroup * max(len(silu_groups), 1))()
                for g, gd in zip(sarr, silu_groups):
                    ops.fill_silu_group(g, **gd)
                ibp = None
                if ib_todo:
                    ibp = N.SeaIbParams()
                    lpre, ibuf = ib_todo[0]
                    ops.fill_ib_params(ibp, [ibuf], None, **self._ib_layer(lpre))
                    ib_todo.clear()
                front_rows = (sarr, len(silu_groups), ibp)
                silu_groups = []
            for s_ in range(0, len(silu_groups), N.MAX_SILU_GROUPS):
                silu_launch(silu_groups[s_:s_ + N.MAX_SILU_GROUPS], "adaln.silu")
            if fm.adaln_front:
                self._front = ({pre_: hids.get(pre_) for pre_, _ in front}, front_rows)
            else:
                self._gemm([dict(A=hids[pre_], W=P.act(pre_ + "cond_mlp.2.weight"), bias=P.f32_vec(pre_ + "cond_mlp.2.bias"), Cact=mods[pre_]) for pre_, _ in front], "adaln.cond_gemm.front")
            arr = self._array(N.SeaGemmGroup, [dict(A=hids[pre_], W=P.act(pre_ + "cond_mlp.2.weight"), bias=P.f32_vec(pre_ + "cond_mlp.2.bias"),
                                                    Cact=mods[pre_]) for pre_, _ in later], ops.fill_gemm_group)
            self._riders = _Riders(arr, sum(((M + 127) // 128) * ((2 * d + 127) // 128) for _, d in later), F, fm.rider_caps)
            self._keep.append(arr)
            return mods

        def emit(inst, tag):
            silu_groups, gemm_groups = [], []
            if fm.gen_a:
                if ib_todo:
                    silu_launch([], "ib.rows")
                for pre, d in inst:
                    mod = self._buf(M, 2 * d)
                    mods[pre] = mod
                    gemm_groups.append(dict(A=None, M=M, W=P.act(pre + "cond_mlp.2.weight"), bias=P.f32_vec(pre + "cond_mlp.2.bias"), Cact=mod,
                                            silu=dict(w1=P.f32_vec(pre + "cond_mlp.0.weight", 2 * d), b1=P.f32_vec(pre + "cond_mlp.0.bias"))))
                self._gemm(gemm_groups, "adaln.cond_gemm" + tag)
                return
            for pre, d in inst:
                hid = self._buf(M, 2 * d)
                mod = self._buf(M, 2 * d)
                mods[pre] = mod
                silu_groups.append(dict(w1=P.f32_vec(pre + "cond_mlp.0.weight", 2 * d), b1=P.f32_vec(pre + "cond_mlp.0.bias"), Hid=hid))
                gemm_groups.append(dict(A=hid, W=P.act(pre + "cond_mlp.2.weight"), bias=P.f32_vec(pre + "cond_mlp.2.bias"), Cact=mod))
            for s in range(0, len(silu_groups), N.MAX_SILU_GROUPS):
                silu_launch(silu_groups[s:s + N.MAX_SILU_GROUPS], "adaln.silu" + tag)
            self._gemm(gemm_groups, "adaln.cond_gemm" + tag)

        if fm.front_big:
            first = []
        if not fm.split_cond:
            emit(first + rest, "")
            return mods
        if first:
            emit(first, ".first")
        self._fork(1)
# ... 82 lines not shown
                               col0=0, Q=Qs[i], K=Ks[l][i], Vt=Vs[l][i]) for i in range(F)]
            if few:
                self._qkv_few(qkv_groups, rope_s, hd_s, "self.qkv_rope", pre=norm0())
            elif l == 0 and fm.one_launch_front:
                self._front_launch(pre, first, xr, Qs, Ks[l], Vs[l])
            else:
                if l == 0 and fm.adaln_front:
                    hid = self._front[0]
                    ag = []
                    for i in range(F):
                        mp = f"{pre}ln.exp.{i}.0."
                        g = dict(A=hid[mp], W=P.act(mp + "cond_mlp.2.weight"), bias=P.f32_vec(mp + "cond_mlp.2.bias"), X=xr[i], gamma=P.f32_vec(mp + "weight"), beta=P.f32_vec(mp + "bias"), Yact=n_e[i])
                        if first:
                            g.update(ldx=FE, X_is_x=i * Eo * 4)
                        ag.append(g)
                    for key, hid_ in hid.items():
                        if "ln_cross." in key:
                            ag.append(dict(A=hid_, W=P.act(key + "cond_mlp.2.weight"), bias=P.f32_vec(key + "cond_mlp.2.bias"), Yact=mods[key]))
                    self._adaln(ag, "self.cond_adaln0")
                else:
                    self._norm(norm0(), E, "self.adaln0")
                self._qkv([dict(A=n_e[i], **g) for i, g in enumerate(qkv_groups)], rope_s, hd_s, "self.qkv_rope")
            self._attn([dict(Q=Qs[i], K=Ks[l][i], Vt=Vs[l][i], O=att_e[i]) for i in range(F)], hd_s, E, "self.attention")
            groups = []
            for i in range(F):
                g = dict(A=att_e[i], W=P.act(f"{pre}attn.self.{i}.projection.weight"), C32=xr[i], Cact=xa[i])
                if first:
                    g.update(R=xr[i], ldr=FE, R_is_x=i * Eo * 4)
                else:
                    g.update(R=xr[i])
                groups.append(g)
            if chain:
                groups = []
                for i in range(F):
                    proj = []
                    for s_, j in enumerate([j for j in range(F) if j != i]):
                        ca = f"{pre}cross_attn.{i}.{j}."
                        proj.append(dict(W=P.act(ca + "q.weight"), bias=P.f32_vec(ca + "q.bias"), col0=0, Q=Qc2[i][s_]))
                    for a in range(i):
                        ca = f"{pre}cross_attn.{a}.{i}."
                        proj.append(dict(W=P.act(ca + "k.weight", 2 * D), bias=P.f32_vec(ca + "k.bias", 2 * D), col0=D, K=Kc[l][a][i], Vt=Vc[l][a][i]))
                    g = dict(a2=att_e[i], W2=P.act(f"{pre}attn.self.{i}.projection.weight"), Xin=xr[i], X=xr[i], proj=proj,
                             down=dict(W=P.act(f"{pre}cross_down.{i}.weight"), bias=P.f32_vec(f"{pre}cross_down.{i}.bias"), **self._norm_params(f"{pre}ln_cross.{i}.")))
                    if first:
                        g.update(ldxin=FE, Xin_is_x=i * Eo * 4)
                    groups.append(g)
                self._chain(groups, rope_c, hd_c, "self.out_proj_down_qkv")
            else:
                (self._gemm_few if few else self._gemm)(groups, "self.out_proj")
            first = False
            if not cond_joined:
                self._join(1)
                cond_joined = True
            if xmode == "addition":
                ndall = self._buf(F, M, D)
                self._down_norm(pre, range(F), xa, dn, ndall, "add")
                sg = self._buf(M, D)
                self._gemm([dict(A=ndall[0], W=eng.eye(D), n_seg=F, a_seg_stride=M * D, Cact=sg, act=1)], "add.sum_gelu")
                self._gemm([dict(A=sg, W=P.act(f"{pre}cross_up.{i}.weight"), bias=P.f32_vec(f"{pre}cross_up.{i}.bias"), R=xr[i], C32=xr[i])
                            for i in range(F)], "add.up")
            if xmode == "pool":
                FD = F * D
                big = self._buf(M, 2 * FD)
                nrm = [self._buf(M, D) for _ in range(F)]
                pe_t = self._buf(M, D, dtype=f32)
                pe_t.copy_(blk_pe(eng, l)[:T].repeat(B, 1))
                self._down_norm(pre, range(F), xa, dn, nrm, "pool")
                self._gemm([dict(A=nrm[j], W=eng.eye(D), R=pe_t, Cact=big[:, j * D:(j + 1) * D]) for j in range(F)], "pool.pe_add")
                hp, pool = self._buf(M, 2 * D), self._buf(M, D)
                self._gemm([dict(A=big[:, :FD], W=P.act(f"{pre}pool_update.0.weight"), bias=P.f32_vec(f"{pre}pool_update.0.bias"), Cact=hp, act=1)], "pool.update0")
                self._gemm([dict(A=hp, W=P.act(f"{pre}pool_update.2.weight"), bias=P.f32_vec(f"{pre}pool_update.2.bias"), Cact=pool)], "pool.update2")
                Qp = [self._buf(B, H, T, hd_c) for _ in range(F)]
                Kp = [self._buf(B, H, cap, hd_c, zero=True) for _ in range(F)]
                Vp = [self._buf(B, H, hd_c, cap, zero=True) for _ in range(F)]
                att_p = [self._buf(M, D) for _ in range(F)]
                qg = []
# ... 3 lines not shown
                    qg.append(dict(A=pool, W=P.act(ca + "k.weight", 2 * D), bias=P.f32_vec(ca + "k.bias", 2 * D), col0=D, K=Kp[i], Vt=Vp[i]))
                self._qkv(qg, rope_c, hd_c, "pool.qkv_rope")
                self._attn([dict(Q=Qp[i], K=Kp[i], Vt=Vp[i], O=att_p[i]) for i in range(F)], hd_c, D, "pool.attention")
                self._gemm([dict(A=att_p[i], W=P.act(f"{pre}cross_attn.{i}.projection.weight"), Cact=big[:, FD + i * D:FD + (i + 1) * D]) for i in range(F)], "pool.proj")
                sg = [self._buf(M, D) for _ in range(F)]
                self._gemm([dict(A=big[:, i * D:(i + 1) * D], W=eng.eye(D), n_seg=2, a_seg_stride=FD, Cact=sg[i], act=1) for i in range(F)], "pool.sum_gelu")
                self._gemm([dict(A=sg[i], W=P.act(f"{pre}cross_up.{i}.weight"), bias=P.f32_vec(f"{pre}cross_up.{i}.bias"), R=xr[i], C32=xr[i])
                            for i in range(F)], "pool.up")
            if F > 1 and xmode == "sea" and few:
                self._gemm_few([dict(A=xa[j], W=P.act(f"{pre}cross_down.{j}.weight"), bias=P.f32_vec(f"{pre}cross_down.{j}.bias"), C32=dn[j]) for j in range(F)], "cross.down_old")
                for i in range(F):
                    others = [j for j in range(F) if j != i]
                    qkv_groups, qkv_pre, probs, proj_groups = [], [], [], []
                    for s, j in enumerate(others):
                        ca = f"{pre}cross_attn.{i}.{j}."
                        qkv_groups.append(dict(W=P.act(ca + "q.weight"), bias=P.f32_vec(ca + "q.bias"), col0=0, Q=Qc[s]))
                        qkv_pre.append(dict(X=dn[i], **self._norm_params(f"{pre}ln_cross.{i}.")))
                        qkv_groups.append(dict(W=P.act(ca + "k.weight", 2 * D), bias=P.f32_vec(ca + "k.bias", 2 * D), col0=D, K=Kc[l][i][j], Vt=Vc[l][i][j]))
                        qkv_pre.append(dict(X=dn[j], **self._norm_params(f"{pre}ln_cross.{j}.")))
                        probs.append(dict(Q=Qc[s], K=Kc[l][i][j], Vt=Vc[l][i][j], O=att_c[s]))
                        proj_groups.append(dict(A=att_c[s], W=P.act(ca + "projection.weight"), Cact=gp[s], act=1))
                    self._qkv_few(qkv_groups, rope_c, hd_c, f"cross{i}.qkv_rope", pre=qkv_pre)
                    self._attn(probs, hd_c, D, f"cross{i}.attention")
                    self._gemm_few(proj_groups, f"cross{i}.proj_gelu")
                    up = dict(A=gp[0], W=P.act(f"{pre}cross_up.{i}.weight"), bias=P.f32_vec(f"{pre}cross_up.{i}.bias"),
                              bias_scale=float(F - 1), n_seg=F - 1, a_seg_stride=M * D, R=xr[i], C32=xr[i], Cact=(xa[i] if i < F - 1 else None))
                    (self._gemm_few if F == 2 else self._gemm)([up], f"cross{i}.up_sum")
                    if i < F - 1:
                        self._gemm_few([dict(A=xa[i], W=P.act(f"{pre}cross_down.{i}.weight"), bias=P.f32_vec(f"{pre}cross_down.{i}.bias"), C32=dn[i])], f"cross{i}.down_new")
            elif F > 1 and xmode == "sea" and chain:
                for i in range(F):
                    others = [j for j in range(F) if j != i]
                    self._attn([dict(Q=Qc2[i][s_], K=Kc[l][i][j], Vt=Vc[l][i][j], O=att_c[s_]) for s_, j in enumerate(others)], hd_c, D, f"cross{i}.attention")
                    proj = []
                    for b_ in range(i + 1, F):
                        ca = f"{pre}cross_attn.{b_}.{i}."
                        proj.append(dict(W=P.act(ca + "k.weight", 2 * D), bias=P.f32_vec(ca + "k.bias", 2 * D), col0=D, K=Kc[l][b_][i], Vt=Vc[l][b_][i]))
                    down = None
                    if i < F - 1:
                        down = dict(W=P.act(f"{pre}cross_down.{i}.weight"), bias=P.f32_vec(f"{pre}cross_down.{i}.bias"), **self._norm_params(f"{pre}ln_cross.{i}."))
                    self._chain([dict(att=[att_c[s_] for s_ in range(len(others))], Wp=[P.act(f"{pre}cross_attn.{i}.{j}.projection.weight") for j in others],
                                      W2=P.act(f"{pre}cross_up.{i}.weight"), b2=P.f32_vec(f"{pre}cross_up.{i}.bias"), bias_scale=float(F - 1), Xin=xr[i], X=xr[i],
                                      down=down, proj=proj)], rope_c, hd_c, f"cross{i}.tail")
            elif F > 1 and xmode == "sea":
                self._down_norm(pre, range(F), xa, dn, nd_old, "cross", "_old")
                for i in range(F):
                    others = [j for j in range(F) if j != i]
                    qkv_groups, probs, proj_groups = [], [], []
                    for s, j in enumerate(others):
                        src = nd_new[j] if j < i else nd_old[j]
                        ca = f"{pre}cross_attn.{i}.{j}."
                        qkv_groups.append(dict(A=nd_old[i], W=P.act(ca + "q.weight"), bias=P.f32_vec(ca + "q.bias"), col0=0, Q=Qc[s]))
                        qkv_groups.append(dict(A=src, W=P.act(ca + "k.weight", 2 * D), bias=P.f32_vec(ca + "k.bias", 2 * D), col0=D,
                                               K=Kc[l][i][j], Vt=Vc[l][i][j]))
                        probs.append(dict(Q=Qc[s], K=Kc[l][i][j], Vt=Vc[l][i][j], O=att_c[s]))
                        proj_groups.append(dict(A=att_c[s], W=P.act(ca + "projection.weight"), Cact=gp[s], act=1))
                    self._qkv(qkv_groups, rope_c, hd_c, f"cross{i}.qkv_rope")
                    self._attn(probs, hd_c, D, f"cross{i}.attention")
                    if fm.xtail:
                        down = None
                        if i < F - 1:
                            down = dict(W=P.act(f"{pre}cross_down.{i}.weight"), bias=P.f32_vec(f"{pre}cross_down.{i}.bias"), Yact=nd_new[i],
                                        **self._norm_params(f"{pre}ln_cross.{i}."))
                        self._xtail([att_c[s] for s in range(len(others))], [P.act(f"{pre}cross_attn.{i}.{j}.projection.weight") for j in others],
                                    P.act(f"{pre}cross_up.{i}.weight"), P.f32_vec(f"{pre}cross_up.{i}.bias"), float(F - 1), xr[i], down, f"cross{i}.tail")
                        continue
                    self._gemm(proj_groups, f"cross{i}.proj_gelu")
                    up = dict(A=gp[0], W=P.act(f"{pre}cross_up.{i}.weight"), bias=P.f32_vec(f"{pre}cross_up.{i}.bias"),
                              bias_scale=float(F - 1), n_seg=F - 1, a_seg_stride=M * D, R=xr[i], C32=xr[i],
                              Cact=(xa[i] if i < F - 1 else None))
                    self._gemm([up], f"cross{i}.up_sum")
                    if lanes:
                        if i < F - 1:
                            self._fork(2 + i)
                        self._ib(pre, [xr[i]])
                        self._mlp_proj(pre, [i], xr, xm, n_e, hbuf, hg, last, tag=f".f{i}")
# ... 8 lines not shown
            if eng.model.add_info_after_cross and has_ib and not fold_ib:
                self._ib(pre, xr)
            if eng.model.add_info_after_cross and ib_attn:
                self._ib_attn(pre, xr)
            self._mlp_proj(pre, list(range(F)), xr, xa, n_e, hbuf, hg, last, addend=(ibufs[l] if fold_ib else None))

    def _norm_params(self, pre: str) -> dict:
        P = self.eng.params
        if self.adaln:
            return dict(mod=self._mods[pre], gamma=P.f32_vec(pre + "weight"), beta=P.f32_vec(pre + "bias"))
        return dict(gamma=P.f32_vec(pre + "weight"))

    def _down_norm(self, pre, fields, xa, dn, Y, stem: str, suffix: str = "") -> None:
        P = self.eng.params
        lin = lambda j: dict(A=xa[j], W=P.act(f"{pre}cross_down.{j}.weight"), bias=P.f32_vec(f"{pre}cross_down.{j}.bias"))
        if self.forms.down_norm:
            self._gemm_norm([dict(Yact=Y[j], **lin(j), **self._norm_params(f"{pre}ln_cross.{j}.")) for j in fields], f"{stem}.down_norm{suffix}")
        else:
            self._gemm([dict(C32=dn[j], **lin(j)) for j in fields], f"{stem}.down{suffix}")
            self._norm([dict(X=dn[j], Yact=Y[j], **self._norm_params(f"{pre}ln_cross.{j}.")) for j in fields], self.D, f"{stem}.norm{suffix}")

    def _front_launch(self, pre, first, xr, Qs, Ks, Vs) -> None:
        P, F, E, D, M, Eo, fm = self.eng.params, self.F, self.E, self.D, self.M, self.Eo, self.forms
        hid, rows = self._front if fm.front_chain else (None, None)
        if fm.cond_memo and self.memo_count is None:
            self.memo_count = self._buf(2, dtype=torch.int32, zero=True)
        arr = (N.SeaAdalnQkv * F)()
        for g_, i in zip(arr, range(F)):
            mp, lc = f"{pre}ln.exp.{i}.0.", f"{pre}ln_cross.{i}."
            third = dict(w1=P.f32_vec(lc + "cond_mlp.0.weight", 2 * D), b1=P.f32_vec(lc + "cond_mlp.0.bias"), W=P.act(lc + "cond_mlp.2.weight"), bias=P.f32_vec(lc + "cond_mlp.2.bias"),
                         out=self._mods[lc]) if fm.front3 else None
            memo = dict(stamps=self._buf(M, 2, dtype=torch.int32, zero=True), mods=self._mods[mp], epoch=P.memo_epoch, count=self.memo_count) if fm.cond_memo else None
            if memo is not None and i == 0 and rows is not None:
                memo["rows"] = self._buf(rows[1] + 1, M, 2, dtype=torch.int32, zero=True)
            ops.fill_adaln_qkv(g_, X=xr[i], cond=None, w1=P.f32_vec(mp + "cond_mlp.0.weight", 2 * E), b1=P.f32_vec(mp + "cond_mlp.0.bias"), W2c=P.act(mp + "cond_mlp.2.weight"),
                               b2c=P.f32_vec(mp + "cond_mlp.2.bias"), gamma=P.f32_vec(mp + "weight"), beta=P.f32_vec(mp + "bias"), Wqkv=P.act(f"{pre}attn.self.{i}.q.weight", 3 * E),
                               bqkv=P.f32_vec(f"{pre}attn.self.{i}.q.bias", 3 * E), Q=Qs[i], K=Ks[i], Vt=Vs[i], ldx=(F * Eo if first else None), third=third, memo=memo)
            g_.M = M
            self._c_patches.append((g_, "cond"))
            if first:
                self._x_patches.append((g_, "X", i * Eo * 4))
        rg = [key for key in hid if "ln_cross." in key] if fm.front_chain and not fm.front3 else []
        rarr = (N.SeaGemmGroup * max(len(rg), 1))() if fm.front_chain else None
        for g_, key in zip(rarr or (), rg):
            ops.fill_gemm_group(g_, hid[key], P.act(key + "cond_mlp.2.weight"), P.f32_vec(key + "cond_mlp.2.bias"), Cact=self._mods[key])
        common = self._qkv_common(self.eng.rope_self, E // self.H)
        sarr, n_s, ibp = rows if rows is not None else (None, 0, None)
        rec = self._rec(N.lib().sea_adaln_qkv, [arr, F, C.byref(common), (rarr if rg else None), len(rg), (sarr if n_s else None), n_s, None, (M if (n_s or ibp is not None) else 0),
                                                (C.byref(ibp) if ibp is not None else None), 1e-5, self.code], "self.cond_adaln0_qkv_rope", (arr, common, rarr, sarr, ibp))
        if n_s or ibp is not None:
            self._c_patches.append((rec.args, 7))
        self._cur.append(rec)

    def _mlp_proj(self, pre, fields, xr, xm, n_e, hbuf, hg, final_norm, tag="", addend=None) -> bool:
        P, E, S, Eo, FE = self.eng.params, self.E, self.S, self.Eo, self.F * self.Eo
        xo = xr if Eo == E else [t[:, :Eo] for t in xr]

        fm = self.forms
        if fm.few:
            xq = [self._buf(self.M, E, dtype=torch.float32) for _ in fields] if addend is not None else None
            res = xq if addend is not None else [xr[i] for i in fields]
            pre_n = [dict(X=xr[i], **(dict(addend=addend, Xout=xq[k]) if addend is not None else {}), **self._norm_params(f"{pre}ln.exp.{i}.2.")) for k, i in enumerate(fields)]
            self._gemm_few([dict(W=P.act(f"{pre}mlp.{i}.layers.0.weight"), bias=P.f32_vec(f"{pre}mlp.{i}.layers.0.bias"), Cact=hbuf[i]) for i in fields], "mlp.fc1" + tag, pre=pre_n)
            ln_h = [dict(X=hbuf[i], gamma=P.f32_vec(f"{pre}mlp.{i}.layers.1.weight"), beta=P.f32_vec(f"{pre}mlp.{i}.layers.1.bias")) for i in fields]
            fold_ln = fm.few_fold_ln
            if not fold_ln:
                self._norm([dict(Yact=hg[i], **g_) for i, g_ in zip(fields, ln_h)], S, "mlp.ln_gelu" + tag, x_is_act=True, gelu=True)
# ... 259 lines not shown
                c.op, c.p0, c.n, c.i0, c.i1, c.f0, c.dtype = N.OP_GEMM_FEW, addr(a[0]), a[2], a[3], a[4], a[5], a[6]
                c.p1 = addr(a[1]) if a[1] is not None else None
            elif r.fn is L.sea_qkv_rope_fewrows:
                c.op, c.p0, c.n, c.p1, c.f0, c.dtype = N.OP_QKV_FEW, addr(a[0]), a[2], addr(r.keep[2]), a[4], a[5]
                c.l0 = addr(a[1]) if a[1] is not None else 0
            elif r.fn is L.sea_attention_fwd:
                c.op, c.p0, c.dtype = N.OP_ATTN, addr(r.keep), a[1]
            elif r.fn is L.sea_mlp_fc1_ln_gelu:
                c.op, c.p0, c.n, c.f0, c.dtype = N.OP_MLP1, addr(a[0]), a[1], a[2], a[3]
            elif r.fn is L.sea_mlp_fc2_proj_norm:
                c.op, c.p0, c.n, c.f0, c.dtype = N.OP_MLP2, addr(a[0]), a[1], a[2], a[3]
            elif r.fn is L.sea_adaln_qkv:
                c.op, c.p0, c.n, c.p1, c.f0, c.dtype = N.OP_AQKV, addr(a[0]), a[1], addr(r.keep[1]), a[10], a[11]
                c.l0, c.i0 = (addr(a[3]) if a[3] is not None else 0), a[4]
                c.l1, c.i1 = (addr(a[5]) if a[5] is not None else 0), a[6]
                c.l2, c.i2 = (a[7] or 0), a[8]
                if a[8]:
                    relink.append((i, "l2", a, 7))
                c.l3 = addr(r.keep[4]) if r.keep[4] is not None else 0
            elif r.fn is L.sea_splitk_finish:
                c.op, c.p0, c.n, c.dtype = N.OP_SPLITK, addr(a[0]), a[1], a[2]
            elif r.fn is L.sea_mlp_block:
                c.op, c.p0, c.p1, c.n, c.f0, c.dtype = N.OP_MLPB, addr(a[0]), addr(a[1]), a[2], a[3], a[4]
            elif r.fn is L.sea_exchange_tail:
                c.op, c.p0, c.n, c.f0, c.dtype = N.OP_XTAIL, addr(r.keep), a[1], a[2], a[3]
            elif r.fn is L.sea_gemm_adaln:
                c.op, c.p0, c.n, c.f0, c.dtype = N.OP_ADALN, addr(a[0]), a[1], a[2], a[3]
            elif r.fn is L.sea_row_chain:
                c.op, c.p0, c.n, c.p1, c.f0, c.dtype = N.OP_CHAIN, addr(a[0]), a[1], addr(r.keep[1]), a[3], a[4]
            elif r.fn is L.sea_row_chain_riders:
                c.op, c.p0, c.n, c.p1, c.f0, c.dtype = N.OP_CHAIN, addr(a[0]), a[1], addr(r.keep[1]), a[8], a[9]
                c.l0, c.i0, c.i1, c.i2 = addr(a[3]), a[4], a[5], a[6]
                c.l1 = addr(r.keep[3]) if r.keep[3] is not None else 0
            elif r.fn is L.sea_gemm_rownorm:
                c.op, c.p0, c.n, c.f0, c.dtype = N.OP_GEMM_NORM, addr(a[0]), a[1], a[2], a[3]
            elif r.fn is L.sea_rownorm:
                c.op, c.p0, c.n, c.i0, c.i1, c.i2, c.i3, c.f0, c.dtype = N.OP_NORM, addr(a[0]), a[1], a[2], a[3], a[4], a[5], a[6], a[7]
            elif r.fn is L.sea_silu_outer or r.fn is L.sea_silu_outer_ib:
                c.op, c.p0, c.n, c.i0, c.dtype = N.OP_SILU, (addr(a[0]) if a[0] is not None else None), a[1], a[3], a[4]
                if r.fn is L.sea_silu_outer_ib and a[5] is not None:
                    c.l0, c.l1 = addr(a[5]), a[6]
                relink.append((i, "p1", a, 2))
            elif r.fn is L.sea_ib_add:
                c.op, c.p0 = N.OP_IB, addr(r.keep)
            elif r.fn is L.sea_convert_f32_to_act:
                c.op, c.l0, c.p1, c.l1, c.l2, c.l3, c.dtype = N.OP_CONVERT, a[1], a[2], a[3], a[4], a[5], a[6]
                relink.append((i, "p0", a, 0))
            else:
                return
        self._clist = (arr, len(recs), relink)
        self._relink()

    def _relink(self) -> None:
        if self._clist is not None:
            arr, _, relink = self._clist
            for i, field, args, k in relink:
                setattr(arr[i], field, args[k] if (args[k] is not None or field[0] == "p") else 0)

    def run(self, concurrent: bool = False) -> None:
        main = torch.cuda.current_stream()
        stream = main.cuda_stream
        if not concurrent and self._clist is not None:
            rc = N.lib().sea_run_list(self._clist[0], self._clist[1], stream)
            if rc != 0:
                N.check(rc, "plan replay (sea_run_list)")
            return
# ... 343 lines not shown
```

sea_amd/ops.py:

```python
from __future__ import annotations

import ctypes as C
import math
from typing import Dict, Optional, Sequence

import torch

from . import _native as N


def _mat(t: torch.Tensor, name: str) -> torch.Tensor:
    N.require_gpu(t, name)
    if t.dim() != 2 or t.stride(1) != 1:
        raise ValueError(f"{name}: need a 2-D tensor with unit inner stride, got shape {tuple(t.shape)} strides {t.stride()}")
    return t


def fill_gemm_group(g: N.SeaGemmGroup, A, W, bias=None, R=None, C32=None, Cact=None, n_seg=1, a_seg_stride=0, act=0,
                    bias_scale=1.0, M=None, N_=None, K=None, Z=None, silu=None, drop=None, ldr=None, ldc32=None) -> None:
    if silu is not None:
        c = silu.get("c")
        g.silu_c, g.silu_w1, g.silu_b1 = N.ptr(c), silu["w1"].data_ptr(), silu["b1"].data_ptr()
        A, R, Z, n_seg, a_seg_stride, act = None, None, None, 1, 0, 0
        M = c.numel() if M is None else M
# ... 242 lines not shown
    for p_, d in zip(P, groups):
        fill_exchange_tail(p_, d["att"], d["Wp"], d["Wup"], d.get("bup"), d.get("bias_scale", 1.0), d["X"], d.get("Xact"), d.get("down"))
    N.check(N.lib().sea_exchange_tail(P, len(groups), eps, N.dtype_code(dtype), N.stream_ptr()), "sea_exchange_tail")


def fill_adaln_group(g: N.SeaAdalnGroup, A, W, bias=None, X=None, gamma=None, beta=None, Yact=None, Y32=None, mean=None, rstd=None, ldx=None, ldy32=None) -> None:
    g.A, g.lda, g.W, g.ldw, g.bias = A.data_ptr(), A.stride(0), W.data_ptr(), W.stride(0), N.ptr(bias)
    g.X, g.ldx = N.ptr(X), ((ldx if ldx is not None else X.stride(0)) if X is not None else 0)
    g.gamma, g.beta = N.ptr(gamma), N.ptr(beta)
    g.Yact, g.ldyact = N.ptr(Yact), (Yact.stride(0) if Yact is not None else 0)
    g.Y32, g.ldy32 = N.ptr(Y32), ((ldy32 if ldy32 is not None else Y32.stride(0)) if Y32 is not None else 0)
    g.mean, g.rstd = N.ptr(mean), N.ptr(rstd)
    g.M, g.d, g.K = A.shape[0], W.shape[0] // 2, W.shape[1]


def gemm_adaln(groups: Sequence[Dict], eps: float = 1e-5, dtype: torch.dtype = torch.bfloat16) -> None:
    arr = (N.SeaAdalnGroup * len(groups))()
    for g, d in zip(arr, groups):
        fill_adaln_group(g, **d)
    N.check(N.lib().sea_gemm_adaln(arr, len(groups), eps, N.dtype_code(dtype), N.stream_ptr()), "sea_gemm_adaln")


def adaln_qkv_supported(dtype: torch.dtype, E: int, H: int) -> bool:
    return dtype == torch.bfloat16 and E == 256 and H > 0 and E % H == 0 and E // H in (16, 32)


def fill_adaln_qkv(g: N.SeaAdalnQkv, X, cond, w1, b1, W2c, b2c, gamma, beta, Wqkv, bqkv, Q, K, Vt, ldx=None, third=None, memo=None) -> None:
    if memo is not None:
        st, tab = memo["stamps"], memo["mods"]
        if st.dtype != torch.int32 or tuple(st.shape) != (X.shape[0], 2) or not st.is_contiguous() or tab.shape[0] != X.shape[0] or tab.shape[1] != W2c.shape[0] or tab.stride(1) != 1:
            raise ValueError(f"adaln_qkv memo: stamps {tuple(st.shape)} {st.dtype} / mods {tuple(tab.shape)} do not fit M = {X.shape[0]}, 2E = {W2c.shape[0]}")
        g.memo_stamps, g.memo_mods, g.ldmemo = st.data_ptr(), tab.data_ptr(), tab.stride(0)
        g.memo_epoch, g.memo_count, g.memo_rows = memo["epoch"].data_ptr(), N.ptr(memo.get("count")), N.ptr(memo.get("rows"))
    g.X, g.ldx, g.cond = X.data_ptr(), (ldx if ldx is not None else X.stride(0)), N.ptr(cond)
    g.w1, g.b1, g.W2c, g.ldw2c, g.b2c = w1.data_ptr(), b1.data_ptr(), W2c.data_ptr(), W2c.stride(0), N.ptr(b2c)
    g.gamma, g.beta, g.Wqkv, g.ldw, g.bqkv = gamma.data_ptr(), N.ptr(beta), Wqkv.data_ptr(), Wqkv.stride(0), N.ptr(bqkv)
    g.Q, g.K, g.Vt = Q.data_ptr(), K.data_ptr(), Vt.data_ptr()
    g.M, g.E = X.shape[0], Wqkv.shape[1]
    if third is not None:
        W3, o3 = third["W"], third["out"]
        g.w13, g.b13, g.W3, g.ldw3, g.b3 = third["w1"].data_ptr(), third["b1"].data_ptr(), W3.data_ptr(), W3.stride(0), N.ptr(third.get("bias"))
        g.mod3, g.ldmod3, g.N3 = o3.data_ptr(), o3.stride(0), W3.shape[0]


def adaln_qkv(groups: Sequence[Dict], rope: torch.Tensor, H: int, hd: int, T: int, pos0: int, cap: int, q_scale: float, riders: Sequence[Dict] = (), silu: Sequence[Dict] = (),
              silu_c: Optional[torch.Tensor] = None, eps: float = 1e-5, dtype: torch.dtype = torch.bfloat16) -> None:
    arr = (N.SeaAdalnQkv * len(groups))()
    for g, d in zip(arr, groups):
        fill_adaln_qkv(g, **d)
    c = N.SeaQkvCommon()
    c.rope, c.H, c.hd, c.T, c.pos0, c.cap, c.q_scale = rope.data_ptr(), H, hd, T, pos0, cap, q_scale
    rarr = None
    if riders:
        rarr = (N.SeaGemmGroup * len(riders))()
        for g, d in zip(rarr, riders):
            fill_gemm_group(g, **d)
    sarr = None
    if silu:
        sarr = (N.SeaSiluGroup * len(silu))()
        for g, gd in zip(sarr, silu):
            fill_silu_group(g, gd["w1"], gd["b1"], gd["Hid"])
    N.check(N.lib().sea_adaln_qkv(arr, len(groups), C.byref(c), rarr, len(riders), sarr, len(silu), (silu_c.data_ptr() if silu_c is not None else None),
                                  (silu_c.numel() if silu_c is not None else 0), None, eps, N.dtype_code(dtype), N.stream_ptr()), "sea_adaln_qkv")


def row_chain_supported(dtype: torch.dtype, D: int, E: int, n_seg: int, hd: int) -> bool:
    return dtype == torch.bfloat16 and (D, E) in ((128, 256), (64, 128)) and 0 <= n_seg and n_seg * D <= E and hd in (16, 32)


def fill_row_chain(P: N.SeaRowChain, W2, Xin, X, att: Sequence[torch.Tensor] = (), Wp: Sequence[torch.Tensor] = (), a2=None, b2=None, bias_scale: float = 1.0, Xact=None,
                   down: Optional[Dict] = None, proj: Sequence[Dict] = (), ldxin: Optional[int] = None) -> None:
    for s_, a in enumerate(att):
        P.att[s_] = a.data_ptr()
        P.Wp[s_] = Wp[s_].data_ptr()
    P.n_seg = len(att)
    if att:
        P.ldatt, P.ldwp = att[0].stride(0), Wp[0].stride(0)
    if a2 is not None:
        P.a2, P.lda2 = a2.data_ptr(), a2.stride(0)
    P.W2, P.ldw2, P.b2, P.bias_scale = W2.data_ptr(), W2.stride(0), N.ptr(b2), bias_scale
    P.Xin, P.ldxin = Xin.data_ptr(), (ldxin if ldxin is not None else Xin.stride(0))
    P.X, P.ldx = X.data_ptr(), X.stride(0)
    P.Xact, P.ldxact = N.ptr(Xact), (Xact.stride(0) if Xact is not None else 0)
    P.M, P.E = X.shape[0], W2.shape[0]
    P.D = P.E // 2
    P.has_down = int(down is not None)
    if down is not None:
        g = P.down
        g.W, g.ldw, g.bias = down["W"].data_ptr(), down["W"].stride(0), N.ptr(down.get("bias"))
        g.gamma, g.beta = down["gamma"].data_ptr(), N.ptr(down.get("beta"))
        mod, y32, yact = down.get("mod"), down.get("Y32"), down.get("Yact")
        g.mod, g.ldmod = N.ptr(mod), (mod.stride(0) if mod is not None else 0)
        g.Y32, g.ldy32 = N.ptr(y32), (y32.stride(0) if y32 is not None else 0)
        g.Yact, g.ldyact = N.ptr(yact), (yact.stride(0) if yact is not None else 0)
        g.mean, g.rstd = N.ptr(down.get("mean")), N.ptr(down.get("rstd"))
        g.M, g.N, g.K, g.n_seg = P.M, P.D, P.E, 1
    if len(proj) > N.CHAIN_MAX_PROJ:
        raise ValueError(f"row_chain: {len(proj)} projection entries (at most {N.CHAIN_MAX_PROJ})")
    P.n_proj = len(proj)
    for q, d in zip(P.proj, proj):
        W = d["W"]
        q.A, q.lda, q.M = None, 0, P.M
        q.W, q.ldw, q.bias = W.data_ptr(), W.stride(0), N.ptr(d.get("bias"))
        q.N, q.K, q.col0 = W.shape[0], W.shape[1], d.get("col0", 0)
        q.Qout, q.Kout, q.Vtout, q.Vout = N.ptr(d.get("Q")), N.ptr(d.get("K")), N.ptr(d.get("Vt")), N.ptr(d.get("V"))


def row_chain(groups: Sequence[Dict], rope: Optional[torch.Tensor] = None, H: int = 1, hd: int = 4, T: int = 1, pos0: int = 0, cap: int = 0, q_scale_: float = 1.0,
              eps: float = 1e-5, dtype: torch.dtype = torch.bfloat16) -> None:
    P = (N.SeaRowChain * len(groups))()
    for p_, d in zip(P, groups):
        fill_row_chain(p_, **d)
    common = N.SeaQkvCommon(N.ptr(rope), H, hd, T, pos0, cap, q_scale_) if rope is not None else None
    N.check(N.lib().sea_row_chain(P, len(groups), C.byref(common) if common is not None else None, eps, N.dtype_code(dtype), N.stream_ptr()), "sea_row_chain")


def fill_silu_group(g: N.SeaSiluGroup, w1, b1, Hid) -> None:
    g.w1, g.b1, g.Hid, g.K2, g.ld = w1.data_ptr(), b1.data_ptr(), Hid.data_ptr(), Hid.shape[1], Hid.stride(0)


def silu_outer(groups: Sequence[Dict], c: torch.Tensor, M: int, dtype: torch.dtype) -> None:
    n = len(groups)
    arr = (N.SeaSiluGroup * n)()
    for g, gd in zip(arr, groups):
        fill_silu_group(g, gd["w1"], gd["b1"], _mat(gd["Hid"], "Hid"))
    N.require_gpu(c, "c")
    assert c.dtype == torch.float32 and c.is_contiguous() and c.numel() == M
    N.check(N.lib().sea_silu_outer(arr, n, c.data_ptr(), M, N.dtype_code(dtype), N.stream_ptr()), "sea_silu_outer")


def fill_ib_params(P: N.SeaIbParams, xs: Sequence[torch.Tensor], c, w1, b1=None, lnw=None, lnb=None, w2=None, b2=None, mode: int = 0, M=None, E=None,
# ... 1082 lines not shown
```

sea_amd/plan_forms.py:

```python
from __future__ import annotations

from dataclasses import dataclass, field
from typing import Dict, Optional, Tuple

import torch

from . import _native as N
from . import _switches
from . import ops

INFERENCE, TRAINING, CONDITION = "inference", "training", "condition"


@dataclass(frozen=True)
class PlanForms:
    lanes: bool
    split_cond: bool
    chain: bool
    riders: bool
    rider_caps: Optional[Tuple[int, ...]]
    gen_a: bool
    fold_ib: bool
    hoist_ib: bool
    ib_rows_here: bool
    xtail: bool
    few: bool
    few_fold_ln: bool
    hidden_pad: int
    front_chain: bool
    front3: bool
    adaln_front: bool
    front_big: bool
    mlp_fc1: bool
    mlp_norm_in: bool
    mlp_block: bool
    mlp_fc2_proj: bool
    down_norm: bool
    proj_norm: bool
    splitk: bool
    cond_memo: bool = field(default=False, compare=False)

    @property
    def one_launch_front(self) -> bool:
        return self.front_big or self.front_chain


def resolve_forms(model, B: int, T: int, mode: str, dt: torch.dtype, kind: str = INFERENCE, hoisted: bool = False, hoisted_ib: bool = False,
                  plan_switches: Optional[Dict[str, str]] = None, kv_switches: Optional[Dict[str, str]] = None) -> PlanForms:
    assert kind in (INFERENCE, TRAINING, CONDITION)
    sw = (_switches.parse("SEA_PLAN") if plan_switches is None else plan_switches).get
    kvsw = (_switches.parse("SEA_KV") if kv_switches is None else kv_switches).get
    inference = kind == INFERENCE
    F, H, L = model.num_variables, model.n_heads, model.num_layers
    Eo, E, D, S, M = model.embed_dim, model.internal_embed_dim, model.down_dim, model.mlp_hidden, B * T
    xmode, ib_add = model.exchange_mode, model.ib_addition_mode.lower()
    has_ib, ib_attn, concat = ib_add == "add", ib_add == "attention", ib_add == "concat"
    after, adaln = bool(model.add_info_after_cross), model.LN_type.lower() == "adaln"

    lane_mode = sw("lanes", "auto") if inference and xmode == "sea" and has_ib else "none"
    if lane_mode == "auto":
        lane_mode = "cond" if M >= 8192 else "none"
    lanes = lane_mode == "all" and F >= 2 and after
    split_cond = lane_mode in ("cond", "all") and adaln
    fuse_norm = inference and sw("norm", "1") != "0"
    chain = (inference and mode == "full" and xmode == "sea" and 1 < F <= 3 and fuse_norm and not lanes and not concat
             and sw("chain", "1") != "0" and sw("xtail", "1") != "0" and ops.row_chain_supported(dt, D, E, F - 1, D // H)
             and M <= int(sw("chain_max_rows", "4096")))
    riders = (chain and adaln and L == 1 and not split_cond and sw("riders", "1") != "0"
              and (not has_ib or (after and E <= 2048)) and not ib_attn and F + F <= N.CHAIN_MAX_RIDERS)
    caps = sw("rider_caps", "") if riders else ""
    want = sw("silu", "auto")
    gen_a = inference and 2 * max(E, D) <= 1024 and (want == "1" or (want == "auto" and M >= 8192))
    fold_ib = (inference and has_ib and after and adaln and not lanes and L <= N.MAX_SILU_IB and E <= 2048 and sw("fold_ib", "1") != "0"
               and (riders or (gen_a and sw("fold_ib_gen", "0") != "0") or (not gen_a and not split_cond)))
    hoist_ib = hoisted and hoisted_ib and has_ib and after and E <= 2048
    ib_rows_here = fold_ib and not hoist_ib
    xtail = (fuse_norm and not lanes and xmode == "sea" and F > 1 and sw("xtail", "1") != "0"
             and ops.exchange_tail_supported(dt, D, E, F - 1) and M <= int(sw("xtail_max_rows", "1000000000")))
    few = (inference and mode == "step" and T == 1 and xmode == "sea" and not concat and not ib_attn
           and kvsw("gemv", "1") != "0" and 2 * (F - 1) <= N.FEW_MAX_GROUPS and F <= N.FEW_MAX_GROUPS
           and ops.fewrows_supported(dt, M, [E], qkv=True, pre=True) and ops.fewrows_supported(dt, M, [S])
           and (F == 1 or ops.fewrows_supported(dt, M, [D], qkv=True, pre=True)))

    aqkv = ops.adaln_qkv_supported(dt, E, H) and F <= N.MAX_AQKV_GROUPS and not concat
    adaln_front = riders and not hoisted and sw("adaln_gemm", "1") != "0"
    front_chain = adaln_front and sw("front", "1") != "0" and aqkv
    front3 = (front_chain and D == 128 and F + F <= N.AQKV_MAX_SILU and (L if ib_rows_here else 0) <= 1
              and sw("front3", "1") != "0")
    front_big = (inference and adaln and not hoisted and not riders and mode == "full" and sw("front_big", "0") == "1" and aqkv and M >= 1024)

    mlp_ok = ops.mlp_fc1_supported(dt, E, S) and (1 if lanes else F) <= N.MAX_MLP_GROUPS
    w1, wn, w2 = sw("mlp1", "auto"), sw("mlpnorm", "auto"), sw("mlp2", "auto")
    mlp_fc1 = inference and w1 != "0" and (w1 == "1" or M >= 1024) and mlp_ok
    mlp_norm_in = mlp_fc1 and (wn == "1" or (wn == "auto" and M <= 4096))
    mlp_block = (mlp_fc1 and inference and (w2 == "1" or (w2 == "auto" and 1024 <= M)) and mlp_ok and Eo == E and sw("mlpblock", "1") != "0")
    if mlp_block:
        mlp_norm_in = mlp_norm_in or (M > 4096 and wn != "0")
    mlp_fc2_proj = not mlp_block and inference and (w2 == "1" or (w2 == "auto" and 1024 <= M <= 4096)) and mlp_ok and Eo == E

    return PlanForms(
        lanes=lanes, split_cond=split_cond, chain=chain, riders=riders, rider_caps=(tuple(int(v) for v in caps.split(":")) if caps else None),
        gen_a=gen_a, fold_ib=fold_ib or hoist_ib, hoist_ib=hoist_ib, ib_rows_here=ib_rows_here, xtail=xtail, few=few, few_fold_ln=S <= 8192,
        hidden_pad=(64 if inference and S % 1024 == 0 else 0), front_chain=front_chain, front3=front3, adaln_front=adaln_front, front_big=front_big,
        mlp_fc1=mlp_fc1, mlp_norm_in=mlp_norm_in, mlp_block=mlp_block, mlp_fc2_proj=mlp_fc2_proj,
        down_norm=(fuse_norm if inference else kind == TRAINING and sw("norm", "1") != "0") and D <= 256 and D % 16 == 0,
        proj_norm=fuse_norm and Eo <= 256 and Eo % 16 == 0 and Eo == E and sw("projnorm", "1") != "0", splitk=sw("splitk", "1") != "0",
        cond_memo=front_chain and riders and sw("cond_memo", "1") != "0")
```

sea_amd/ptrcheck.py:

```python
from __future__ import annotations

import ctypes as C
import os
from typing import Iterable, Iterator, List, Optional, Tuple

import torch

from . import _native as N

_HOST_STRUCTS = (N.SeaLaunchRec, N.SeaStepPatch)


def always() -> bool:
    return os.environ.get("SEA_CHECK_PTRS", "0") == "1"


class Ranges:

    def __init__(self) -> None:
        self._r: List[Tuple[int, int, str]] = []

    def add_tensor(self, t: Optional[torch.Tensor], label: str) -> None:
        if t is None or not isinstance(t, torch.Tensor) or not t.is_cuda or t.numel() == 0:
            return
# ... 90 lines not shown
        if st.bias:
            yield "bias", st.bias, st.N * f32
        if st.R:
            yield "R", st.R, ((st.M - 1) * st.ldr + st.N) * f32
        if st.C32:
            yield "C32", st.C32, ((st.M - 1) * st.ldc32 + st.N) * f32
        if st.Cact:
            yield "Cact", st.Cact, ((st.M - 1) * st.ldcact + st.N) * esz
    elif isinstance(st, N.SeaAdalnQkv):
        E = st.E
        yield "X", st.X, ((st.M - 1) * st.ldx + E) * f32
        yield "cond", st.cond, st.M * f32
        yield "w1", st.w1, 2 * E * f32
        yield "b1", st.b1, 2 * E * f32
        yield "W2c", st.W2c, ((2 * E - 1) * st.ldw2c + 2 * E) * esz
        if st.b2c:
            yield "b2c", st.b2c, 2 * E * f32
        yield "gamma", st.gamma, E * f32
        yield "Wqkv", st.Wqkv, ((3 * E - 1) * st.ldw + E) * esz
        if st.bqkv:
            yield "bqkv", st.bqkv, 3 * E * f32
        if st.W3:
            yield "w13", st.w13, st.N3 * f32
            yield "b13", st.b13, st.N3 * f32
            yield "W3", st.W3, ((st.N3 - 1) * st.ldw3 + st.N3) * esz
            yield "mod3", st.mod3, ((st.M - 1) * st.ldmod3 + st.N3) * esz
        if st.memo_stamps:
            yield "memo_stamps", st.memo_stamps, st.M * 8
            yield "memo_mods", st.memo_mods, ((st.M - 1) * st.ldmemo + 2 * E) * esz
            yield "memo_epoch", st.memo_epoch, 4
            if st.memo_count:
                yield "memo_count", st.memo_count, 8
            if st.memo_rows:
                yield "memo_rows", st.memo_rows, st.M * 8
    elif isinstance(st, N.SeaRowChain):
        K2 = st.D if st.n_seg > 0 else st.E
        for s_ in range(st.n_seg):
            yield f"att[{s_}]", st.att[s_], ((st.M - 1) * st.ldatt + st.D) * esz
            yield f"Wp[{s_}]", st.Wp[s_], ((st.D - 1) * st.ldwp + st.D) * esz
        if st.a2:
            yield "a2", st.a2, ((st.M - 1) * st.lda2 + st.E) * esz
        yield "W2", st.W2, ((st.E - 1) * st.ldw2 + K2) * esz
        if st.b2:
            yield "b2", st.b2, st.E * f32
        yield "Xin", st.Xin, ((st.M - 1) * st.ldxin + st.E) * f32
        yield "X", st.X, ((st.M - 1) * st.ldx + st.E) * f32
        if st.Xact:
            yield "Xact", st.Xact, ((st.M - 1) * st.ldxact + st.E) * esz
    elif isinstance(st, N.SeaMlpGroup):
        if st.A:
            yield "A", st.A, ((st.M - 1) * st.lda + st.E) * esz
        if st.X32:
            yield "X32", st.X32, ((st.M - 1) * st.ldx32 + st.E) * f32
        if st.addend:
            yield "addend", st.addend, ((st.M - 1) * st.ldadd + st.E) * f32
        if st.Xout:
            yield "Xout", st.Xout, ((st.M - 1) * st.ldxout + st.E) * f32
        if st.mod:
            yield "mod", st.mod, ((st.M - 1) * st.ldmod + 2 * st.E) * esz
        yield "W1", st.W1, ((st.S - 1) * st.ldw + st.E) * esz
        yield "Hg", st.Hg, ((st.M - 1) * st.ldh + st.S) * esz
        for k in ("b1", "lnw", "lnb"):
            yield k, getattr(st, k), st.S * f32
    elif isinstance(st, N.SeaKvFill):
        bh = st.B * st.H
        last_src, last_dst = (bh - 1) * st.cap_src * st.hd, (bh - 1) * st.cap_dst * st.hd
        yield "K", st.K, (last_src + st.n_pos * st.hd) * esz
# ... 27 lines not shown
def _walk_structs(obj) -> Iterator[C.Structure]:
    if isinstance(obj, _HOST_STRUCTS):
        return
    if isinstance(obj, C.Structure):
        yield obj
        for name, _ in obj._fields_:
            v = getattr(obj, name)
            if isinstance(v, (C.Structure, C.Array)):
                yield from _walk_structs(v)
    elif isinstance(obj, C.Array):
        for i in range(len(obj)):
            e = obj[i]
            if isinstance(e, (C.Structure, C.Array)):
                yield from _walk_structs(e)
    elif isinstance(obj, (tuple, list)):
        for e in obj:
            yield from _walk_structs(e)


def _raw_extents(r, esz: int) -> Iterable[Tuple[str, int, int]]:
    name, a = getattr(r.fn, "__name__", ""), r.args
    if name == "sea_convert_f32_to_act":
        rows, cols = a[4], a[5]
        if isinstance(a[0], int):
            yield "src", a[0], ((rows - 1) * a[1] + cols) * 4
        if isinstance(a[2], int):
            yield "dst", a[2], ((rows - 1) * a[3] + cols) * (4 if a[6] == N.SEA_F32 else esz)
    elif name == "sea_silu_outer_bwd_dc":
        for label, k in (("c", 2), ("dc", 3)):
            if isinstance(a[k], int):
                yield label, a[k], a[4] * 4
        if isinstance(a[6], int):
            yield "ws", a[6], a[7] * 4
    elif name == "sea_ib_bwd_dc" and isinstance(a[1], int) and isinstance(r.keep, N.SeaIbBwdParams):
        yield "dc", a[1], r.keep.M * 4


def check_records(records, ranges: Ranges, esz: int, what: str) -> int:
    n = 0
    for r in records:
        if r.fn is None:
            continue
        roots = [a for a in r.args if isinstance(a, (C.Structure, C.Array))]
        if r.keep is not None:
            roots.append(r.keep)
        for root in roots:
            for st in _walk_structs(root):
                for path, p in iter_pointers(st, type(st).__name__):
                    n += 1
                    if ranges.find(p) is None:
                        raise RuntimeError(f"sea_amd pointer audit ({what}): launch '{r.name}': {path} = {p:#x} lies in no buffer this plan knows "
                                           "(stale address, unpatched field or a tensor that was freed)")
                for field, p, nbytes in _extents(st, esz):
                    if not p:
                        continue
                    hit = ranges.find(p)
                    if hit is not None and nbytes > 0 and p + nbytes > hit[1]:
                        raise RuntimeError(f"sea_amd pointer audit ({what}): launch '{r.name}': {type(st).__name__}.{field} = {p:#x} + {nbytes} bytes runs "
                                           f"{p + nbytes - hit[1]} bytes past the end of its buffer ({hit[2]})")
        for field, p, nbytes in _raw_extents(r, esz):
            hit = ranges.find(p)
            if hit is not None and nbytes > 0 and p + nbytes > hit[1]:
                raise RuntimeError(f"sea_amd pointer audit ({what}): launch '{r.name}': argument {field} = {p:#x} + {nbytes} bytes runs "
                                   f"{p + nbytes - hit[1]} bytes past the end of its buffer ({hit[2]})")
        for a in r.args:
            if isinstance(a, int) and a >= (1 << 32) and ranges.find(a) is None and r.fn is not None and r.name not in ("",):
                if _looks_like_device_pointer(a):
                    raise RuntimeError(f"sea_amd pointer audit ({what}): launch '{r.name}': raw argument {a:#x} lies in no buffer this plan knows")
    return n


def _looks_like_device_pointer(a: int) -> bool:
    return a >= (1 << 40) and a % 4 == 0
```

Measured before the change: 5587.

## Defer chain QKV projection to a projection-only group and skip memo-hit rider tiles

Adds a projection-only mode to the row-chain kernel, so the QKV projection can be deferred into a separate group that reads the normalized rows directly. The adaLN-QKV front now records per-tile memo hits, and a new memo-aware row-chain entry point reads those flags so rider GEMM tiles whose conditioning rows were all memo hits return early. The intent is to cut redundant conditioning/rider work and rebalance the fused chain schedule during rollout. It adds plan complexity, new pointer-audit extents, and depends on the memo hit flags being correct.

```diff
diff --git a/include/sea_hip.h b/include/sea_hip.h
--- a/include/sea_hip.h
+++ b/include/sea_hip.h
@@ -424,13 +424,15 @@
     const uint32_t* memo_epoch;
     int32_t* memo_count;
     uint32_t* memo_rows;
-    int32_t ldmemo, pad_;
+    int32_t ldmemo;
+    int32_t memo_tile_off;
 } SeaAdalnQkv;
 int sea_adaln_qkv(const SeaAdalnQkv* groups, int n_groups, const SeaQkvCommon* common, const SeaGemmGroup* riders, int n_riders, const SeaSiluGroup* silu, int n_silu,
                   const float* silu_c, int silu_M, const SeaIbParams* ib, float eps, int dtype, void* stream);
 
 #define SEA_CHAIN_MAX_PROJ 6
 #define SEA_CHAIN_MAX_GROUPS 3
+#define SEA_CHAIN_PROJ_ONLY (-1)
 typedef struct {
     const void* att[SEA_XTAIL_MAX_SEG];
     const void* Wp[SEA_XTAIL_MAX_SEG];
@@ -451,6 +453,8 @@
 struct SeaIbParams_;
 int sea_row_chain_riders(const SeaRowChain* params, int n_groups, const SeaQkvCommon* common, const SeaGemmGroup* riders, int n_riders, int tile0, int n_tiles,
                          const struct SeaIbParams_* ib, float eps, int dtype, void* stream);
+int sea_row_chain_riders_memo(const SeaRowChain* params, int n_groups, const SeaQkvCommon* common, const SeaGemmGroup* riders, int n_riders, int tile0, int n_tiles,
+                              const struct SeaIbParams_* ib, const uint32_t* rider_hit, int32_t* rider_count, float eps, int dtype, void* stream);
 
 enum { SEA_OP_GEMM = 1, SEA_OP_QKV = 2, SEA_OP_ATTN = 3, SEA_OP_NORM = 4, SEA_OP_SILU = 5, SEA_OP_IB = 6, SEA_OP_CONVERT = 8, SEA_OP_GEMM_NORM = 9, SEA_OP_XTAIL = 10, SEA_OP_MLP1 = 11, SEA_OP_MLP2 = 13, SEA_OP_GEMM_FEW = 14, SEA_OP_QKV_FEW = 15, SEA_OP_CHAIN = 16, SEA_OP_ADALN = 17, SEA_OP_MLPB = 18, SEA_OP_AQKV = 19, SEA_OP_SPLITK = 20 };
 typedef struct {
diff --git a/sea_amd/_native.py b/sea_amd/_native.py
--- a/sea_amd/_native.py
+++ b/sea_amd/_native.py
@@ -140,6 +140,7 @@
 CHAIN_MAX_PROJ = 6
 CHAIN_MAX_GROUPS = 3
 CHAIN_MAX_RIDERS = 8
+CHAIN_PROJ_ONLY = -1
 
 
 class SeaRowChain(C.Structure):
@@ -394,6 +395,9 @@
     L.sea_row_chain.restype = C.c_int
     L.sea_row_chain_riders.argtypes = [C.POINTER(SeaRowChain), C.c_int, C.POINTER(SeaQkvCommon), C.POINTER(SeaGemmGroup), C.c_int, C.c_int, C.c_int, C.POINTER(SeaIbParams), C.c_float, C.c_int, _vp]
     L.sea_row_chain_riders.restype = C.c_int
+    L.sea_row_chain_riders_memo.argtypes = [C.POINTER(SeaRowChain), C.c_int, C.POINTER(SeaQkvCommon), C.POINTER(SeaGemmGroup), C.c_int, C.c_int, C.c_int, C.POINTER(SeaIbParams), _vp, _vp,
+                                            C.c_float, C.c_int, _vp]
+    L.sea_row_chain_riders_memo.restype = C.c_int
     L.sea_patchify.argtypes = [_vp, _vp, _vp, _vp, _vp, _i64, _i64, _i64, _i64, C.c_int, C.c_int, C.c_int, C.c_int, C.c_int, C.c_int, C.c_float, _vp]
     L.sea_patchify.restype = C.c_int
     L.sea_silu_outer_ib.argtypes = [C.POINTER(SeaSiluGroup), C.c_int, _vp, C.c_int, C.c_int, _vp, C.c_int, _vp]
@@ -486,7 +490,7 @@
     "sea_wgrad_grouped", "sea_transpose_weights", "sea_rownorm_bwd", "sea_silu_outer_bwd", "sea_ib_bwd",
     "sea_attention_bwd", "sea_dropout_mask", "sea_run_list", "sea_run_list_steps", "sea_unpatchify", "sea_gemm_rownorm", "sea_exchange_tail", "sea_patchify", "sea_silu_outer_ib", "sea_mlp_fc1_ln_gelu", "sea_mlp_fc2_proj_norm", "sea_kv_rollout", "sea_kv_arena_words", "sea_kv_debug_stamps",
     "sea_kv_cache_fill", "sea_kv_cache_fork", "sea_kv_cache_gather", "sea_decode_mse", "sea_decode_member_sse", "sea_decode_member_moments", "sea_decode_sensor_sse", "sea_decode_sensor_grad", "sea_resample_systematic", "sea_enkf_transform", "sea_enkf_transform_gram", "sea_decode_member_gram", "sea_ensemble_mix", "sea_ensemble_verify", "sea_ensemble_verify_ws_bytes",
-    "sea_gemm_fewrows", "sea_qkv_rope_fewrows", "sea_row_chain", "sea_row_chain_riders", "sea_gemm_adaln", "sea_mlp_block", "sea_adaln_qkv", "sea_splitk_finish",
+    "sea_gemm_fewrows", "sea_qkv_rope_fewrows", "sea_row_chain", "sea_row_chain_riders", "sea_row_chain_riders_memo", "sea_gemm_adaln", "sea_mlp_block", "sea_adaln_qkv", "sea_splitk_finish",
     "sea_encoder_block_ws_floats", "sea_encoder_block_fwd", "sea_encoder_block_bwd",
     "sea_silu_outer_bwd_dc", "sea_silu_outer_bwd_dc_ws_floats", "sea_ib_bwd_dc",
 )
diff --git a/sea_amd/csrc/adaln_qkv.hip b/sea_amd/csrc/adaln_qkv.hip
--- a/sea_amd/csrc/adaln_qkv.hip
+++ b/sea_amd/csrc/adaln_qkv.hip
@@ -99,6 +99,7 @@
             __syncthreads();
             const bool r_hit = __builtin_amdgcn_readfirstlane(*reinterpret_cast<const int*>(smem)) != 0;
             if (L.g[0].memo_count != nullptr && threadIdx.x == 0) atomicAdd(L.g[0].memo_count + (r_hit ? 0 : 1), 1);
+            if (x < L.silu_wgs && L.g[0].memo_tile_off > 0 && threadIdx.x == 0) L.g[0].memo_rows[L.g[0].memo_tile_off + x] = r_hit ? 1u : 0u;
             if (r_hit) return;
             if (r_row >= 0) reinterpret_cast<uint2*>(rst)[r_row] = make_uint2(r_c, r_e);
         }
@@ -639,7 +640,8 @@
         }
         if (G.memo_stamps != nullptr) {
             SEA_REQUIRE(G.memo_mods && G.memo_epoch && G.ldmemo % 8 == 0 && G.ldmemo >= 2 * E && sea_aligned16(G.memo_mods) && ((uintptr_t)G.memo_stamps & 7) == 0 &&
-                            ((uintptr_t)G.memo_epoch & 3) == 0 && ((uintptr_t)G.memo_count & 3) == 0 && ((uintptr_t)G.memo_rows & 7) == 0,
+                            ((uintptr_t)G.memo_epoch & 3) == 0 && ((uintptr_t)G.memo_count & 3) == 0 && ((uintptr_t)G.memo_rows & 7) == 0 && G.memo_tile_off >= 0 &&
+                            (G.memo_tile_off == 0 || G.memo_rows != nullptr),
                         "sea_adaln_qkv[%d]: condition memo: null / misaligned pointer or bad stride (ldmemo=%d)", i, G.ldmemo);
         }
         L.g[i] = G;
diff --git a/sea_amd/csrc/chain.hip b/sea_amd/csrc/chain.hip
--- a/sea_amd/csrc/chain.hip
+++ b/sea_amd/csrc/chain.hip
@@ -12,6 +12,8 @@
     ChainRiderPod rg[SEA_CHAIN_MAX_RIDERS];
     int n_riders, rider_t0, rider_n, ib_wgs;
     SeaIbParams ib;
+    const uint32_t* rider_hit;
+    int32_t* rider_count;
 };
 static_assert(sizeof(ChainLaunch) <= 4096, "kernel arguments of sea_row_chain");
 
@@ -176,6 +178,13 @@
             int gi = 0;
             while (gi + 1 < L.n_riders && tile >= L.rg[gi + 1].tile_start) ++gi;
             const ChainRiderPod& R = L.rg[gi];
+            if (L.rider_hit != nullptr) {
+                const int nblk = (R.M + 63) >> 6, b0 = ((tile - R.tile_start) / ((R.N + 127) / 128)) * 2;
+                const uint32_t* f = L.rider_hit + gi * nblk + b0;
+                const bool hit = f[0] != 0u && (b0 + 1 >= nblk || f[1] != 0u);
+                if (L.rider_count != nullptr && tid == 0) atomicAdd(L.rider_count + (hit ? 0 : 1), 1);
+                if (hit) return;
+            }
             ChainRiderGroup G;
             G.A = R.A; G.W = R.W; G.bias = R.bias; G.Cact = R.Cact;
             G.lda = R.lda; G.ldw = R.ldw; G.ldcact = R.ldcact; G.M = R.M; G.N = R.N; G.K = R.K;
@@ -223,28 +232,10 @@
     const T* W2 = CP_PTR(const T*, W2);
     const int ldw2 = CP_I32(ldw2);
     const bool has_down = CP_I32(has_down) != 0;
-    const int n_proj = has_down ? CP_I32(n_proj) : 0;
+    const bool proj_only = S < 0;
+    const int n_proj = has_down || proj_only ? CP_I32(n_proj) : 0;
     const T* Wd = CP_PTR(const T*, down.W);
     const int ldwd = CP_I32(down.ldw);
-
-    if (S > 0) {
-        const int ldatt = CP_I32(ldatt), ldwp = CP_I32(ldwp);
-#pragma unroll
-        for (int s = 0; s < SMAX; ++s) {
-            if (s < S) {
-                const T* att = reinterpret_cast<const T*>(cp_dyn_u64(pl, CP_DW(att) + 2 * s));
-                const T* Wp = reinterpret_cast<const T*>(cp_dyn_u64(pl, CP_DW(Wp) + 2 * s));
-                chain_dma_a(att, ldatt, m0, M - 1, BM, KTD, at_l + (unsigned)(s * KTD * A_KTS), wv, lane);
-                chain_dma_w(Wp, ldwp, D, 0, KTD, wa_l + (unsigned)(s * D * D * 2), wv, lane);
-            }
-        }
-        chain_dma_w(W2, ldw2, E, 0, KTD, wb_l, wv, lane);
-    } else {
-        chain_dma_a(CP_PTR(const T*, a2), CP_I32(lda2), m0, M - 1, BM, KTE, at_l, wv, lane);
-        chain_dma_w(W2, ldw2, E, 0, KTE / 2, wa_l, wv, lane);
-        chain_dma_w(W2, ldw2, E, (KTE / 2) * 64, KTE / 2, wb_l, wv, lane);
-    }
-    stamp();
     int mrow[MI];
     bool mok[MI];
 #pragma unroll
@@ -253,40 +244,8 @@
         mok[i] = m < M;
         mrow[i] = mok[i] ? m : M - 1;
     }
-    const float* b2 = CP_PTR(const float*, b2);
-    const float* Xin = CP_PTR(const float*, Xin);
-    const int ldxin = CP_I32(ldxin);
-    const float bias_scale = CP_F32(bias_scale);
-    float bv2[NI2][4], rv2[MI][NI2][4];
-#pragma unroll
-    for (int j = 0; j < NI2; ++j) {
-        const int n = wave * (E / 4) + j * 16 + g * 4;
-#pragma unroll
-        for (int q = 0; q < 4; ++q) bv2[j][q] = 0.f;
-        if (b2 != nullptr) load4(b2 + n, bv2[j]);
-#pragma unroll
-        for (int i = 0; i < MI; ++i) load4(Xin + (int64_t)mrow[i] * ldxin + n, rv2[i][j]);
-    }
-    ChainNormGroup<D, E> Gd;
-    Gd.M = M;
-    Gd.bias = CP_PTR(const float*, down.bias);
-    Gd.mod = CP_PTR(const void*, down.mod);
-    Gd.ldmod = CP_I32(down.ldmod);
-    Gd.gamma = CP_PTR(const float*, down.gamma);
-    Gd.beta = CP_PTR(const float*, down.beta);
-    Gd.Y32 = CP_PTR(float*, down.Y32);
-    Gd.ldy32 = CP_I32(down.ldy32);
-    Gd.Yact = CP_PTR(void*, down.Yact);
-    Gd.ldyact = CP_I32(down.ldyact);
-    Gd.mean = CP_PTR(float*, down.mean);
-    Gd.rstd = CP_PTR(float*, down.rstd);
-    NormEpilogue<T, NI3, true, true, true> epi3[MI];
-    if (has_down) {
-#pragma unroll
-        for (int i = 0; i < MI; ++i) epi3[i].prefetch(Gd, mrow[i], wave * (D / 4), g);
-    }
     const int hd = L.c.hd, hd2 = hd >> 1, Tlen = L.c.T, pos0 = L.c.pos0;
-    if (n_proj > 0) {
+    auto load_rope_bias = [&]() {
         for (int idx = tid; idx < BM * hd2; idx += 256) {
             const int i = idx / hd2, k = idx - i * hd2;
             int m = m0 + i;
@@ -303,79 +262,7 @@
             for (int n = tid; n < N; n += 256) s_bias[boff + n] = bias != nullptr ? bias[n] : 0.f;
             boff += N;
         }
-    }
-#pragma unroll
-    for (int j = 0; j < NI2; ++j)
-#pragma unroll
-        for (int q = 0; q < 4; ++q) {
-            touch(bv2[j][q]);
-#pragma unroll
-            for (int i = 0; i < MI; ++i) touch(rv2[i][j][q]);
-        }
-    if (has_down) {
-#pragma unroll
-        for (int i = 0; i < MI; ++i)
-#pragma unroll
-            for (int j = 0; j < NI3; ++j)
-#pragma unroll
-                for (int q = 0; q < 4; ++q) {
-                    touch(epi3[i].bv[j][q]); touch(epi3[i].gm[j][q]); touch(epi3[i].bt[j][q]); touch(epi3[i].mw[j][q]); touch(epi3[i].mb[j][q]);
-                }
-    }
-    stamp();
-    asm volatile("s_waitcnt vmcnt(0)" ::: "memory");
-    __syncthreads();
-    stamp();
-
-    f32x4 acc2[MI][NI2];
-#pragma unroll
-    for (int i = 0; i < MI; ++i)
-#pragma unroll
-        for (int j = 0; j < NI2; ++j) acc2[i][j] = f32x4{0.f, 0.f, 0.f, 0.f};
-    if (S > 0) {
-        float gsum[MI][NI1][4];
-#pragma unroll
-        for (int i = 0; i < MI; ++i)
-#pragma unroll
-            for (int j = 0; j < NI1; ++j)
-#pragma unroll
-                for (int q = 0; q < 4; ++q) gsum[i][j][q] = 0.f;
-#pragma unroll
-        for (int s = 0; s < SMAX; ++s) {
-            if (s < S) {
-                f32x4 acc1[MI][NI1];
-#pragma unroll
-                for (int i = 0; i < MI; ++i)
-#pragma unroll
-                    for (int j = 0; j < NI1; ++j) acc1[i][j] = f32x4{0.f, 0.f, 0.f, 0.f};
-                chain_mma<MI, NI1>(AT + s * KTD * A_KTS, A_KTS, WA + s * D * D * 2, D * 128, wave * (D / 4), KTD, NI1, r, g, acc1);
-#pragma unroll
-                for (int i = 0; i < MI; ++i)
-#pragma unroll
-                    for (int j = 0; j < NI1; ++j)
-#pragma unroll
-                        for (int q = 0; q < 4; ++q) gsum[i][j][q] += gelu_erf(acc1[i][j][q]);
-            }
-        }
-#pragma unroll
-        for (int i = 0; i < MI; ++i)
-#pragma unroll
-            for (int j = 0; j < NI1; ++j) {
-                const int kk = wave * (D / 4) + j * 16 + g * 4;
-                store4(reinterpret_cast<T*>(YT + (kk >> 6) * A_KTS + (i * 16 + r) * 128 + ((((kk & 63) >> 3) ^ (r & 7)) << 4) + (kk & 7) * 2), gsum[i][j][0], gsum[i][j][1], gsum[i][j][2],
-                       gsum[i][j][3]);
-            }
-        lds_barrier();
-        if (has_down) chain_dma_w(Wd, ldwd, D, 0, KTE, wa_l, wv, lane);
-        chain_mma<MI, NI2>(YT, A_KTS, WB, E * 128, wave * (E / 4), KTD, NI2, r, g, acc2);
-    } else {
-        chain_mma<MI, NI2>(AT, A_KTS, WA, E * 128, wave * (E / 4), KTE / 2, NI2, r, g, acc2);
-        lds_barrier();
-        if (has_down) chain_dma_w(Wd, ldwd, D, 0, KTE, wa_l, wv, lane);
-        chain_mma<MI, NI2>(AT + (KTE / 2) * A_KTS, A_KTS, WB, E * 128, wave * (E / 4), KTE / 2, NI2, r, g, acc2);
-    }
-    lds_barrier();
-    stamp();
+    };
     int e_next = 0;
     auto burst = [&](unsigned half_l, int& e_lo, int& e_hi) {
         e_lo = e_next;
@@ -391,51 +278,182 @@
         e_hi = e_next;
     };
     int b_lo[2] = {0, 0}, b_hi[2] = {0, 0};
-    if (n_proj > 0) burst(wb_l, b_lo[0], b_hi[0]);
-    float v2[MI][NI2][4];
-#pragma unroll
-    for (int i = 0; i < MI; ++i)
-#pragma unroll
+
+    if (proj_only) {
+        chain_dma_a(CP_PTR(const T*, a2), CP_I32(lda2), m0, M - 1, BM, KTD, at_l + (unsigned)C::AT_BYTES, wv, lane);
+        burst(wb_l, b_lo[0], b_hi[0]);
+        stamp();
+        load_rope_bias();
+    } else {
+        if (S > 0) {
+            const int ldatt = CP_I32(ldatt), ldwp = CP_I32(ldwp);
+    #pragma unroll
+            for (int s = 0; s < SMAX; ++s) {
+                if (s < S) {
+                    const T* att = reinterpret_cast<const T*>(cp_dyn_u64(pl, CP_DW(att) + 2 * s));
+                    const T* Wp = reinterpret_cast<const T*>(cp_dyn_u64(pl, CP_DW(Wp) + 2 * s));
+                    chain_dma_a(att, ldatt, m0, M - 1, BM, KTD, at_l + (unsigned)(s * KTD * A_KTS), wv, lane);
+                    chain_dma_w(Wp, ldwp, D, 0, KTD, wa_l + (unsigned)(s * D * D * 2), wv, lane);
+                }
+            }
+            chain_dma_w(W2, ldw2, E, 0, KTD, wb_l, wv, lane);
+        } else {
+            chain_dma_a(CP_PTR(const T*, a2), CP_I32(lda2), m0, M - 1, BM, KTE, at_l, wv, lane);
+            chain_dma_w(W2, ldw2, E, 0, KTE / 2, wa_l, wv, lane);
+            chain_dma_w(W2, ldw2, E, (KTE / 2) * 64, KTE / 2, wb_l, wv, lane);
+        }
+        stamp();
+        const float* b2 = CP_PTR(const float*, b2);
+        const float* Xin = CP_PTR(const float*, Xin);
+        const int ldxin = CP_I32(ldxin);
+        const float bias_scale = CP_F32(bias_scale);
+        float bv2[NI2][4], rv2[MI][NI2][4];
+    #pragma unroll
         for (int j = 0; j < NI2; ++j) {
             const int n = wave * (E / 4) + j * 16 + g * 4;
-#pragma unroll
-            for (int q = 0; q < 4; ++q) v2[i][j][q] = acc2[i][j][q] + bv2[j][q] * bias_scale + rv2[i][j][q];
-            store4(reinterpret_cast<T*>(AT + (n >> 6) * A_KTS + (i * 16 + r) * 128 + ((((n & 63) >> 3) ^ (r & 7)) << 4) + (n & 7) * 2), v2[i][j][0], v2[i][j][1], v2[i][j][2], v2[i][j][3]);
-        }
-    asm volatile("s_waitcnt vmcnt(0)" ::: "memory");
-    stamp();
-    {
-        float* X = CP_PTR(float*, X);
-        T* Xact = CP_PTR(T*, Xact);
-        const int ldx = CP_I32(ldx), ldxact = CP_I32(ldxact);
-#pragma unroll
-        for (int i = 0; i < MI; ++i) {
-            if (!mok[i]) continue;
-            float* xr_ = X + (int64_t)(m0 + i * 16 + r) * ldx + wave * (E / 4) + g * 4;
-            T* xa_ = Xact != nullptr ? Xact + (int64_t)(m0 + i * 16 + r) * ldxact + wave * (E / 4) + g * 4 : nullptr;
-#pragma unroll
+    #pragma unroll
+            for (int q = 0; q < 4; ++q) bv2[j][q] = 0.f;
+            if (b2 != nullptr) load4(b2 + n, bv2[j]);
+    #pragma unroll
+            for (int i = 0; i < MI; ++i) load4(Xin + (int64_t)mrow[i] * ldxin + n, rv2[i][j]);
+        }
+        ChainNormGroup<D, E> Gd;
+        Gd.M = M;
+        Gd.bias = CP_PTR(const float*, down.bias);
+        Gd.mod = CP_PTR(const void*, down.mod);
+        Gd.ldmod = CP_I32(down.ldmod);
+        Gd.gamma = CP_PTR(const float*, down.gamma);
+        Gd.beta = CP_PTR(const float*, down.beta);
+        Gd.Y32 = CP_PTR(float*, down.Y32);
+        Gd.ldy32 = CP_I32(down.ldy32);
+        Gd.Yact = CP_PTR(void*, down.Yact);
+        Gd.ldyact = CP_I32(down.ldyact);
+        Gd.mean = CP_PTR(float*, down.mean);
+        Gd.rstd = CP_PTR(float*, down.rstd);
+        NormEpilogue<T, NI3, true, true, true> epi3[MI];
+        if (has_down) {
+    #pragma unroll
+            for (int i = 0; i < MI; ++i) epi3[i].prefetch(Gd, mrow[i], wave * (D / 4), g);
+        }
+        if (n_proj > 0) load_rope_bias();
+    #pragma unroll
+        for (int j = 0; j < NI2; ++j)
+    #pragma unroll
+            for (int q = 0; q < 4; ++q) {
+                touch(bv2[j][q]);
+    #pragma unroll
+                for (int i = 0; i < MI; ++i) touch(rv2[i][j][q]);
+            }
+        if (has_down) {
+    #pragma unroll
+            for (int i = 0; i < MI; ++i)
+    #pragma unroll
+                for (int j = 0; j < NI3; ++j)
+    #pragma unroll
+                    for (int q = 0; q < 4; ++q) {
+                        touch(epi3[i].bv[j][q]); touch(epi3[i].gm[j][q]); touch(epi3[i].bt[j][q]); touch(epi3[i].mw[j][q]); touch(epi3[i].mb[j][q]);
+                    }
+        }
+        stamp();
+        asm volatile("s_waitcnt vmcnt(0)" ::: "memory");
+        __syncthreads();
+        stamp();
+
+        f32x4 acc2[MI][NI2];
+    #pragma unroll
+        for (int i = 0; i < MI; ++i)
+    #pragma unroll
+            for (int j = 0; j < NI2; ++j) acc2[i][j] = f32x4{0.f, 0.f, 0.f, 0.f};
+        if (S > 0) {
+            float gsum[MI][NI1][4];
+    #pragma unroll
+            for (int i = 0; i < MI; ++i)
+    #pragma unroll
+                for (int j = 0; j < NI1; ++j)
+    #pragma unroll
+                    for (int q = 0; q < 4; ++q) gsum[i][j][q] = 0.f;
+    #pragma unroll
+            for (int s = 0; s < SMAX; ++s) {
+                if (s < S) {
+                    f32x4 acc1[MI][NI1];
+    #pragma unroll
+                    for (int i = 0; i < MI; ++i)
+    #pragma unroll
+                        for (int j = 0; j < NI1; ++j) acc1[i][j] = f32x4{0.f, 0.f, 0.f, 0.f};
+                    chain_mma<MI, NI1>(AT + s * KTD * A_KTS, A_KTS, WA + s * D * D * 2, D * 128, wave * (D / 4), KTD, NI1, r, g, acc1);
+    #pragma unroll
+                    for (int i = 0; i < MI; ++i)
+    #pragma unroll
+                        for (int j = 0; j < NI1; ++j)
+    #pragma unroll
+                            for (int q = 0; q < 4; ++q) gsum[i][j][q] += gelu_erf(acc1[i][j][q]);
+                }
+            }
+    #pragma unroll
+            for (int i = 0; i < MI; ++i)
+    #pragma unroll
+                for (int j = 0; j < NI1; ++j) {
+                    const int kk = wave * (D / 4) + j * 16 + g * 4;
+                    store4(reinterpret_cast<T*>(YT + (kk >> 6) * A_KTS + (i * 16 + r) * 128 + ((((kk & 63) >> 3) ^ (r & 7)) << 4) + (kk & 7) * 2), gsum[i][j][0], gsum[i][j][1], gsum[i][j][2],
+                           gsum[i][j][3]);
+                }
+            lds_barrier();
+            if (has_down) chain_dma_w(Wd, ldwd, D, 0, KTE, wa_l, wv, lane);
+            chain_mma<MI, NI2>(YT, A_KTS, WB, E * 128, wave * (E / 4), KTD, NI2, r, g, acc2);
+        } else {
+            chain_mma<MI, NI2>(AT, A_KTS, WA, E * 128, wave * (E / 4), KTE / 2, NI2, r, g, acc2);
+            lds_barrier();
+            if (has_down) chain_dma_w(Wd, ldwd, D, 0, KTE, wa_l, wv, lane);
+            chain_mma<MI, NI2>(AT + (KTE / 2) * A_KTS, A_KTS, WB, E * 128, wave * (E / 4), KTE / 2, NI2, r, g, acc2);
+        }
+        lds_barrier();
+        stamp();
+        if (n_proj > 0) burst(wb_l, b_lo[0], b_hi[0]);
+        float v2[MI][NI2][4];
+    #pragma unroll
+        for (int i = 0; i < MI; ++i)
+    #pragma unroll
             for (int j = 0; j < NI2; ++j) {
-                store4(xr_ + j * 16, v2[i][j][0], v2[i][j][1], v2[i][j][2], v2[i][j][3]);
-                if (xa_ != nullptr) store4(xa_ + j * 16, v2[i][j][0], v2[i][j][1], v2[i][j][2], v2[i][j][3]);
-            }
-        }
-    }
-    stamp();
-    if (!has_down) return;
-    lds_barrier();
-    {
-        f32x4 acc3[MI][NI3];
-#pragma unroll
-        for (int i = 0; i < MI; ++i)
-#pragma unroll
-            for (int j = 0; j < NI3; ++j) acc3[i][j] = f32x4{0.f, 0.f, 0.f, 0.f};
-        chain_mma<MI, NI3>(AT, A_KTS, WA, D * 128, wave * (D / 4), KTE, NI3, r, g, acc3);
-#pragma unroll
-        for (int i = 0; i < MI; ++i)
-            epi3[i].finish(Gd, acc3[i], m0 + i * 16 + r, wave * (D / 4), r, g, wave, L.eps, red + i * 128, n_proj > 0 ? YT + i * 16 * 128 : nullptr, A_KTS);
-    }
-    stamp();
-    if (n_proj == 0) return;
+                const int n = wave * (E / 4) + j * 16 + g * 4;
+    #pragma unroll
+                for (int q = 0; q < 4; ++q) v2[i][j][q] = acc2[i][j][q] + bv2[j][q] * bias_scale + rv2[i][j][q];
+                store4(reinterpret_cast<T*>(AT + (n >> 6) * A_KTS + (i * 16 + r) * 128 + ((((n & 63) >> 3) ^ (r & 7)) << 4) + (n & 7) * 2), v2[i][j][0], v2[i][j][1], v2[i][j][2], v2[i][j][3]);
+            }
+        asm volatile("s_waitcnt vmcnt(0)" ::: "memory");
+        stamp();
+        {
+            float* X = CP_PTR(float*, X);
+            T* Xact = CP_PTR(T*, Xact);
+            const int ldx = CP_I32(ldx), ldxact = CP_I32(ldxact);
+    #pragma unroll
+            for (int i = 0; i < MI; ++i) {
+                if (!mok[i]) continue;
+                float* xr_ = X + (int64_t)(m0 + i * 16 + r) * ldx + wave * (E / 4) + g * 4;
+                T* xa_ = Xact != nullptr ? Xact + (int64_t)(m0 + i * 16 + r) * ldxact + wave * (E / 4) + g * 4 : nullptr;
+    #pragma unroll
+                for (int j = 0; j < NI2; ++j) {
+                    store4(xr_ + j * 16, v2[i][j][0], v2[i][j][1], v2[i][j][2], v2[i][j][3]);
+                    if (xa_ != nullptr) store4(xa_ + j * 16, v2[i][j][0], v2[i][j][1], v2[i][j][2], v2[i][j][3]);
+                }
+            }
+        }
+        stamp();
+        if (!has_down) return;
+        lds_barrier();
+        {
+            f32x4 acc3[MI][NI3];
+    #pragma unroll
+            for (int i = 0; i < MI; ++i)
+    #pragma unroll
+                for (int j = 0; j < NI3; ++j) acc3[i][j] = f32x4{0.f, 0.f, 0.f, 0.f};
+            chain_mma<MI, NI3>(AT, A_KTS, WA, D * 128, wave * (D / 4), KTE, NI3, r, g, acc3);
+    #pragma unroll
+            for (int i = 0; i < MI; ++i)
+                epi3[i].finish(Gd, acc3[i], m0 + i * 16 + r, wave * (D / 4), r, g, wave, L.eps, red + i * 128, n_proj > 0 || Gd.Yact != nullptr ? YT + i * 16 * 128 : nullptr, A_KTS);
+        }
+        stamp();
+        if (n_proj == 0) return;
+    }
     const int Hh = L.c.H, cap = L.c.cap, Ea = Hh * hd;
     const int hd_sh = 31 - __builtin_clz((unsigned)hd);
     uint32_t offq[MI], offk[MI], offv[MI];
@@ -550,19 +568,24 @@
 }
 
 static int row_chain_launch(const SeaRowChain* params, int n_groups, const SeaQkvCommon* common, const SeaGemmGroup* riders, int n_riders, int tile0, int n_tiles,
-                            const SeaIbParams* ib, float eps, int dtype, void* stream);
+                            const SeaIbParams* ib, const uint32_t* rider_hit, int32_t* rider_count, float eps, int dtype, void* stream);
 
 extern "C" int sea_row_chain(const SeaRowChain* params, int n_groups, const SeaQkvCommon* common, float eps, int dtype, void* stream) {
-    return row_chain_launch(params, n_groups, common, nullptr, 0, 0, 0, nullptr, eps, dtype, stream);
+    return row_chain_launch(params, n_groups, common, nullptr, 0, 0, 0, nullptr, nullptr, nullptr, eps, dtype, stream);
 }
 
 extern "C" int sea_row_chain_riders(const SeaRowChain* params, int n_groups, const SeaQkvCommon* common, const SeaGemmGroup* riders, int n_riders, int tile0, int n_tiles,
                                     const SeaIbParams* ib, float eps, int dtype, void* stream) {
-    return row_chain_launch(params, n_groups, common, riders, n_riders, tile0, n_tiles, ib, eps, dtype, stream);
+    return row_chain_launch(params, n_groups, common, riders, n_riders, tile0, n_tiles, ib, nullptr, nullptr, eps, dtype, stream);
+}
+
+extern "C" int sea_row_chain_riders_memo(const SeaRowChain* params, int n_groups, const SeaQkvCommon* common, const SeaGemmGroup* riders, int n_riders, int tile0, int n_tiles,
+                                         const SeaIbParams* ib, const uint32_t* rider_hit, int32_t* rider_count, float eps, int dtype, void* stream) {
+    return row_chain_launch(params, n_groups, common, riders, n_riders, tile0, n_tiles, ib, rider_hit, rider_count, eps, dtype, stream);
 }
 
 static int row_chain_launch(const SeaRowChain* params, int n_groups, const SeaQkvCommon* common, const SeaGemmGroup* riders, int n_riders, int tile0, int n_tiles,
-                            const SeaIbParams* ib, float eps, int dtype, void* stream) {
+                            const SeaIbParams* ib, const uint32_t* rider_hit, int32_t* rider_count, float eps, int dtype, void* stream) {
     SEA_REQUIRE(params != nullptr && n_groups >= 1 && n_groups <= SEA_CHAIN_MAX_GROUPS, "sea_row_chain: n_groups=%d out of range", n_groups);
     ChainLaunch L;
     memset(&L, 0, sizeof(L));
@@ -586,6 +609,12 @@
     }
     SEA_REQUIRE(tile0 + n_tiles <= rider_total, "sea_row_chain_riders: tiles [%d, %d) of %d", tile0, tile0 + n_tiles, rider_total);
     L.n_riders = n_riders; L.rider_t0 = tile0; L.rider_n = n_tiles;
+    if (rider_hit != nullptr) {
+        SEA_REQUIRE(n_riders >= 1 && ((uintptr_t)rider_hit & 3) == 0 && ((uintptr_t)rider_count & 3) == 0, "sea_row_chain_riders: rider memo: no riders or a misaligned pointer");
+        for (int i = 1; i < n_riders; ++i) SEA_REQUIRE(riders[i].M == riders[0].M, "sea_row_chain_riders[%d]: rider memo: M=%d differs from the first group's %d", i, riders[i].M, riders[0].M);
+        L.rider_hit = rider_hit;
+        L.rider_count = sea_tune("memo_count", 0) != 0 ? rider_count : nullptr;
+    }
     if (ib != nullptr) {
         SEA_REQUIRE(ib->X[0] && ib->c && ib->w1 && ib->M >= 1 && ib->E >= 4 && ib->E % 4 == 0 && ib->ldx >= ib->E && ib->mode >= 0 && ib->mode <= 2 &&
                         (ib->mode != 0 || (ib->b1 && ib->lnw && ib->lnb && ib->w2 && ib->b2 && ib->h >= 1 && ib->h <= 64)),
@@ -598,22 +627,29 @@
     for (int gi = 0; gi < n_groups; ++gi) {
         const SeaRowChain& P = params[gi];
         const bool shape_ok = (P.D == 128 && P.E == 256) || (P.D == 64 && P.E == 128);
-        if (dtype != SEA_BF16 || !shape_ok || P.n_seg < 0 || P.n_seg * P.D > P.E) {
+        const bool proj_only = P.n_seg == SEA_CHAIN_PROJ_ONLY;
+        if (dtype != SEA_BF16 || !shape_ok || (P.n_seg < 0 && !proj_only) || P.n_seg * P.D > P.E) {
             sea_set_error("sea_row_chain: unsupported dtype / shape (dtype=%d D=%d E=%d n_seg=%d): bf16, (D,E) in {(128,256),(64,128)}, n_seg*D <= E", dtype, P.D, P.E, P.n_seg);
             return SEA_EUNSUPPORTED;
         }
         SEA_REQUIRE(P.D == D && P.E == E, "sea_row_chain[%d]: the groups of a launch share their widths", gi);
-        SEA_REQUIRE(P.M >= 1 && P.W2 && P.Xin && P.X && sea_aligned16(P.W2) && sea_aligned16(P.b2) && sea_aligned16(P.Xin) && sea_aligned16(P.X) && sea_aligned16(P.Xact),
-                    "sea_row_chain[%d]: null / misaligned pointer", gi);
-        const int K2 = P.n_seg > 0 ? P.D : P.E;
-        SEA_REQUIRE(P.ldw2 % 8 == 0 && P.ldw2 >= K2 && P.ldxin % 4 == 0 && P.ldxin >= P.E && P.ldx % 4 == 0 && P.ldx >= P.E && (!P.Xact || (P.ldxact % 4 == 0 && P.ldxact >= P.E)),
-                    "sea_row_chain[%d]: bad strides", gi);
-        if (P.n_seg == 0) SEA_REQUIRE(P.a2 && sea_aligned16(P.a2) && P.lda2 % 8 == 0 && P.lda2 >= P.E, "sea_row_chain[%d]: a2: null / misaligned / short rows", gi);
-        else SEA_REQUIRE(P.ldatt % 8 == 0 && P.ldatt >= P.D && P.ldwp % 8 == 0 && P.ldwp >= P.D, "sea_row_chain[%d]: bad segment strides", gi);
-        for (int s = 0; s < P.n_seg; ++s)
-            SEA_REQUIRE(P.att[s] && sea_aligned16(P.att[s]) && P.Wp[s] && sea_aligned16(P.Wp[s]), "sea_row_chain[%d]: segment %d: null / misaligned operand", gi, s);
+        if (proj_only) {
+            SEA_REQUIRE(P.M >= 1 && P.a2 && sea_aligned16(P.a2) && P.lda2 % 8 == 0 && P.lda2 >= P.D, "sea_row_chain[%d]: projection-only group: y (a2): null / misaligned / short rows", gi);
+            SEA_REQUIRE(!P.has_down && P.n_proj >= 1 && P.n_proj <= SEA_CHAIN_MAX_PROJ, "sea_row_chain[%d]: projection-only group: n_proj=%d has_down=%d (1..%d entries, no down-projection)", gi,
+                        P.n_proj, P.has_down, SEA_CHAIN_MAX_PROJ);
+        } else {
+            SEA_REQUIRE(P.M >= 1 && P.W2 && P.Xin && P.X && sea_aligned16(P.W2) && sea_aligned16(P.b2) && sea_aligned16(P.Xin) && sea_aligned16(P.X) && sea_aligned16(P.Xact),
+                        "sea_row_chain[%d]: null / misaligned pointer", gi);
+            const int K2 = P.n_seg > 0 ? P.D : P.E;
+            SEA_REQUIRE(P.ldw2 % 8 == 0 && P.ldw2 >= K2 && P.ldxin % 4 == 0 && P.ldxin >= P.E && P.ldx % 4 == 0 && P.ldx >= P.E && (!P.Xact || (P.ldxact % 4 == 0 && P.ldxact >= P.E)),
+                        "sea_row_chain[%d]: bad strides", gi);
+            if (P.n_seg == 0) SEA_REQUIRE(P.a2 && sea_aligned16(P.a2) && P.lda2 % 8 == 0 && P.lda2 >= P.E, "sea_row_chain[%d]: a2: null / misaligned / short rows", gi);
+            else SEA_REQUIRE(P.ldatt % 8 == 0 && P.ldatt >= P.D && P.ldwp % 8 == 0 && P.ldwp >= P.D, "sea_row_chain[%d]: bad segment strides", gi);
+            for (int s = 0; s < P.n_seg; ++s)
+                SEA_REQUIRE(P.att[s] && sea_aligned16(P.att[s]) && P.Wp[s] && sea_aligned16(P.Wp[s]), "sea_row_chain[%d]: segment %d: null / misaligned operand", gi, s);
+        }
         L.p[gi] = P;
-        SEA_REQUIRE(P.n_proj >= 0 && P.n_proj <= SEA_CHAIN_MAX_PROJ && (P.n_proj == 0 || P.has_down), "sea_row_chain[%d]: n_proj=%d (projections read the normalised rows: has_down)", gi, P.n_proj);
+        SEA_REQUIRE(P.n_proj >= 0 && P.n_proj <= SEA_CHAIN_MAX_PROJ && (P.n_proj == 0 || P.has_down || proj_only), "sea_row_chain[%d]: n_proj=%d (projections read the normalised rows: has_down)", gi, P.n_proj);
         if (P.has_down) {
             const SeaGemmNormGroup& G = P.down;
             SEA_REQUIRE(G.W && G.gamma && (G.Y32 || G.Yact || P.n_proj > 0) && G.ldw % 8 == 0 && G.ldw >= P.E, "sea_row_chain[%d]: down: null pointer or bad ldw", gi);
@@ -629,6 +665,7 @@
         for (int e = 0; e < P.n_proj; ++e) {
             const SeaQkvGroup& Q = P.proj[e];
             SEA_REQUIRE(common != nullptr, "sea_row_chain: projections need the SeaQkvCommon");
+            SEA_REQUIRE(common->T >= 1 && P.M % common->T == 0, "sea_row_chain[%d]: M=%d rows are not whole trajectories of T=%d (groups of a launch may differ in M)", gi, P.M, common->T);
             const int Ea = common->H * common->hd;
             SEA_REQUIRE(Q.W && sea_aligned16(Q.W) && sea_aligned16(Q.bias) && Q.ldw % 8 == 0 && Q.ldw >= P.D && Q.K == P.D && (Q.N == P.D / 2 || Q.N == P.D || Q.N == 2 * P.D) && Q.N % 64 == 0,
                         "sea_row_chain[%d]: projection %d: W [N, D] with N in {D, 2D} (multiples of 64), K = D (N=%d K=%d ldw=%d)", gi, e, Q.N, Q.K, Q.ldw);
@@ -649,14 +686,18 @@
             sea_set_error("sea_row_chain: unsupported head dim %d (a power of two >= 16: a 16-column block of a projection lies inside one head)", c.hd);
             return SEA_EUNSUPPORTED;
         }
-        SEA_REQUIRE(c.rope != nullptr && c.H >= 1 && c.hd >= 4 && c.hd % 4 == 0 && c.T >= 1 && c.pos0 >= 0 && c.cap >= c.pos0 + c.T && m_max % c.T == 0,
+        SEA_REQUIRE(c.rope != nullptr && c.H >= 1 && c.hd >= 4 && c.hd % 4 == 0 && c.T >= 1 && c.pos0 >= 0 && c.cap >= c.pos0 + c.T ,
                     "sea_row_chain: bad common H=%d hd=%d T=%d pos0=%d cap=%d (M=%d)", c.H, c.hd, c.T, c.pos0, c.cap, m_max);
         SEA_REQUIRE((int64_t)(m_max / c.T + 1) * c.H * c.cap * c.hd < ((int64_t)1 << 31) && (int64_t)(c.pos0 + c.T) * (c.hd / 2) < ((int64_t)1 << 30),
                     "sea_row_chain: attention tensors too large for 32-bit element offsets");
         L.c = c;
     }
     const int forced = sea_tune("chain_rows", 0);
-    int mi = ((m_max + 15) / 16) * n_groups <= 256 ? 1 : 2;
+    int n_own = 0, m_own = 0;
+    for (int gi = 0; gi < n_groups; ++gi)
+        if (params[gi].n_seg != SEA_CHAIN_PROJ_ONLY) { ++n_own; m_own = params[gi].M > m_own ? params[gi].M : m_own; }
+    if (n_own == 0) { n_own = n_groups; m_own = m_max; }
+    int mi = ((m_own + 15) / 16) * n_own <= 256 ? 1 : 2;
     if (forced == 16) mi = 1;
     if (forced == 32) mi = 2;
     if (any_proj && 16 * mi * (L.c.hd / 2) * 8 > 2048) {
diff --git a/sea_amd/csrc/core.hip b/sea_amd/csrc/core.hip
--- a/sea_amd/csrc/core.hip
+++ b/sea_amd/csrc/core.hip
@@ -84,8 +84,9 @@
             case SEA_OP_GEMM_FEW: rc = sea_gemm_fewrows(static_cast<const SeaGemmGroup*>(R.p0), static_cast<const SeaNormGroup*>(R.p1), R.n, R.i0, R.i1, R.f0, R.dtype, stream); break;
             case SEA_OP_QKV_FEW: rc = sea_qkv_rope_fewrows(static_cast<const SeaQkvGroup*>(R.p0), reinterpret_cast<const SeaNormGroup*>(R.l0), R.n, static_cast<const SeaQkvCommon*>(R.p1), R.f0,
                                                            R.dtype, stream); break;
-            case SEA_OP_CHAIN: rc = sea_row_chain_riders(static_cast<const SeaRowChain*>(R.p0), R.n, static_cast<const SeaQkvCommon*>(R.p1), reinterpret_cast<const SeaGemmGroup*>(static_cast<intptr_t>(R.l0)),
-                                                         R.i0, R.i1, R.i2, reinterpret_cast<const SeaIbParams*>(static_cast<intptr_t>(R.l1)), R.f0, R.dtype, stream); break;
+            case SEA_OP_CHAIN: rc = sea_row_chain_riders_memo(static_cast<const SeaRowChain*>(R.p0), R.n, static_cast<const SeaQkvCommon*>(R.p1), reinterpret_cast<const SeaGemmGroup*>(static_cast<intptr_t>(R.l0)),
+                                                         R.i0, R.i1, R.i2, reinterpret_cast<const SeaIbParams*>(static_cast<intptr_t>(R.l1)), reinterpret_cast<const uint32_t*>(static_cast<intptr_t>(R.l2)),
+                                                         reinterpret_cast<int32_t*>(static_cast<intptr_t>(R.l3)), R.f0, R.dtype, stream); break;
             case SEA_OP_ADALN: rc = sea_gemm_adaln(static_cast<const SeaAdalnGroup*>(R.p0), R.n, R.f0, R.dtype, stream); break;
             case SEA_OP_SPLITK: rc = sea_splitk_finish(static_cast<const SeaSplitkGroup*>(R.p0), R.n, R.dtype, stream); break;
             case SEA_OP_MLPB: rc = sea_mlp_block(static_cast<const SeaMlpGroup*>(R.p0), static_cast<const SeaMlp2Group*>(R.p1), R.n, R.f0, R.dtype, stream); break;
diff --git a/sea_amd/csrc/norm_epilogue.hpp b/sea_amd/csrc/norm_epilogue.hpp
--- a/sea_amd/csrc/norm_epilogue.hpp
+++ b/sea_amd/csrc/norm_epilogue.hpp
@@ -176,6 +176,7 @@
                     o[q] = (v[j][q] - mean) * rstd * gq + bq;
                 }
                 store4(reinterpret_cast<__bf16*>(lds_y + (n >> 6) * lds_kts + r * 128 + ((((n & 63) >> 3) ^ (r & 7)) << 4) + (n & 7) * 2), o[0], o[1], o[2], o[3]);
+                if (mok && G.Yact != nullptr) store4(static_cast<T*>(G.Yact) + (int64_t)m * G.ldyact + n, o[0], o[1], o[2], o[3]);
             }
         }
         if (!mok) return;
@@ -184,7 +185,7 @@
             if (G.rstd != nullptr) G.rstd[m] = rstd;
         }
         float* y32 = G.Y32 != nullptr ? G.Y32 + (int64_t)m * G.ldy32 : nullptr;
-        T* yact = G.Yact != nullptr ? static_cast<T*>(G.Yact) + (int64_t)m * G.ldyact : nullptr;
+        T* yact = G.Yact != nullptr && lds_y == nullptr ? static_cast<T*>(G.Yact) + (int64_t)m * G.ldyact : nullptr;
         const bool has_mod = G.mod != nullptr;
 #pragma unroll
         for (int j = 0; j < NI; ++j) {
diff --git a/sea_amd/engine.py b/sea_amd/engine.py
--- a/sea_amd/engine.py
+++ b/sea_amd/engine.py
@@ -226,8 +226,9 @@
 
 class _Riders:
 
-    def __init__(self, arr, tiles: int, hosts: int, caps: Optional[Tuple[int, ...]]):
+    def __init__(self, arr, tiles: int, hosts: int, caps: Optional[Tuple[int, ...]], hit: Optional[torch.Tensor] = None, count: Optional[torch.Tensor] = None):
         self.arr, self.tiles, self.done = arr, tiles, 0
+        self.hit, self.count = hit, count
         self.hosts_total = self.hosts_left = hosts
         self.caps, self.host_no = caps, 0
 
@@ -285,6 +286,9 @@
         self._riders: Optional[_Riders] = None
         self._front = None
         self.memo_count: Optional[torch.Tensor] = None
+        self.memo_tile_count: Optional[torch.Tensor] = None
+        self._memo_rows: Optional[torch.Tensor] = None
+        self._rider_tiles: Optional[torch.Tensor] = None
         self._build()
         self._find_hoisted()
         self._clist = None
@@ -455,7 +459,12 @@
                 self._cur.append(self._rec(N.lib().sea_row_chain, [arr, len(chunk), C.byref(common), 1e-5, self.code], name, (arr, common)))
             else:
                 rarr, n_r, t0, nt = rd
-                self._cur.append(self._rec(N.lib().sea_row_chain_riders, [arr, len(chunk), C.byref(common), rarr, n_r, t0, nt, None, 1e-5, self.code], name, (arr, common, rarr, None)))
+                hit, cnt = self._riders.hit, self._riders.count
+                if hit is None:
+                    self._cur.append(self._rec(N.lib().sea_row_chain_riders, [arr, len(chunk), C.byref(common), rarr, n_r, t0, nt, None, 1e-5, self.code], name, (arr, common, rarr, None)))
+                else:
+                    self._cur.append(self._rec(N.lib().sea_row_chain_riders_memo, [arr, len(chunk), C.byref(common), rarr, n_r, t0, nt, None, hit.data_ptr(), cnt.data_ptr(), 1e-5, self.code],
+                                               name, (arr, common, rarr, None)))
 
     def _qkv(self, groups: List[dict], rope: torch.Tensor, hd: int, name: str) -> None:
         arr = self._array(N.SeaQkvGroup, groups, lambda g, **d: ops.fill_qkv_group(g, M=self.M, **d))
@@ -535,7 +544,12 @@
                 self._gemm([dict(A=hids[pre_], W=P.act(pre_ + "cond_mlp.2.weight"), bias=P.f32_vec(pre_ + "cond_mlp.2.bias"), Cact=mods[pre_]) for pre_, _ in front], "adaln.cond_gemm.front")
             arr = self._array(N.SeaGemmGroup, [dict(A=hids[pre_], W=P.act(pre_ + "cond_mlp.2.weight"), bias=P.f32_vec(pre_ + "cond_mlp.2.bias"),
                                                     Cact=mods[pre_]) for pre_, _ in later], ops.fill_gemm_group)
-            self._riders = _Riders(arr, sum(((M + 127) // 128) * ((2 * d + 127) // 128) for _, d in later), F, fm.rider_caps)
+            if fm.cond_memo and front_rows is not None and list(hids) == [pre_ for pre_, _ in later]:
+                n_st = (len(later) + 1) * M * 2
+                self._memo_rows = self._buf(n_st + len(later) * ((M + 63) // 64), dtype=torch.int32, zero=True)
+                self._rider_tiles = self._memo_rows[n_st:].view(len(later), (M + 63) // 64)
+                self.memo_tile_count = self._buf(2, dtype=torch.int32, zero=True)
+            self._riders = _Riders(arr, sum(((M + 127) // 128) * ((2 * d + 127) // 128) for _, d in later), F, fm.rider_caps, self._rider_tiles, self.memo_tile_count)
             self._keep.append(arr)
             return mods
 
@@ -684,16 +698,28 @@
                 groups.append(g)
             if chain:
                 groups = []
+                deferred: Dict[int, Dict[int, Tuple[torch.Tensor, list]]] = {}
+
+                def place(reader: int, y: torch.Tensor, entry: dict, here: list, own_host: int = -1) -> bool:
+                    host = reader - 1
+                    if not fm.defer_proj or host <= own_host:
+                        here.append(entry)
+                        return False
+                    deferred.setdefault(host, {}).setdefault(id(y), (y, []))[1].append(entry)
+                    return True
+
                 for i in range(F):
-                    proj = []
+                    proj, stored = [], False
                     for s_, j in enumerate([j for j in range(F) if j != i]):
                         ca = f"{pre}cross_attn.{i}.{j}."
-                        proj.append(dict(W=P.act(ca + "q.weight"), bias=P.f32_vec(ca + "q.bias"), col0=0, Q=Qc2[i][s_]))
+                        q_reader = min(i, 1)
+                        stored |= place(q_reader, nd_old[i], dict(W=P.act(ca + "q.weight"), bias=P.f32_vec(ca + "q.bias"), col0=0, Q=Qc2[i][s_]), proj)
                     for a in range(i):
                         ca = f"{pre}cross_attn.{a}.{i}."
-                        proj.append(dict(W=P.act(ca + "k.weight", 2 * D), bias=P.f32_vec(ca + "k.bias", 2 * D), col0=D, K=Kc[l][a][i], Vt=Vc[l][a][i]))
+                        stored |= place(a, nd_old[i], dict(W=P.act(ca + "k.weight", 2 * D), bias=P.f32_vec(ca + "k.bias", 2 * D), col0=D, K=Kc[l][a][i], Vt=Vc[l][a][i]), proj)
                     g = dict(a2=att_e[i], W2=P.act(f"{pre}attn.self.{i}.projection.weight"), Xin=xr[i], X=xr[i], proj=proj,
-                             down=dict(W=P.act(f"{pre}cross_down.{i}.weight"), bias=P.f32_vec(f"{pre}cross_down.{i}.bias"), **self._norm_params(f"{pre}ln_cross.{i}.")))
+                             down=dict(W=P.act(f"{pre}cross_down.{i}.weight"), bias=P.f32_vec(f"{pre}cross_down.{i}.bias"), **(dict(Yact=nd_old[i]) if stored else {}),
+                                       **self._norm_params(f"{pre}ln_cross.{i}.")))
                     if first:
                         g.update(ldxin=FE, Xin_is_x=i * Eo * 4)
                     groups.append(g)
@@ -763,16 +789,19 @@
                 for i in range(F):
                     others = [j for j in range(F) if j != i]
                     self._attn([dict(Q=Qc2[i][s_], K=Kc[l][i][j], Vt=Vc[l][i][j], O=att_c[s_]) for s_, j in enumerate(others)], hd_c, D, f"cross{i}.attention")
-                    proj = []
+                    proj, stored = [], False
                     for b_ in range(i + 1, F):
                         ca = f"{pre}cross_attn.{b_}.{i}."
-                        proj.append(dict(W=P.act(ca + "k.weight", 2 * D), bias=P.f32_vec(ca + "k.bias", 2 * D), col0=D, K=Kc[l][b_][i], Vt=Vc[l][b_][i]))
+                        stored |= place(b_, nd_new[i], dict(W=P.act(ca + "k.weight", 2 * D), bias=P.f32_vec(ca + "k.bias", 2 * D), col0=D, K=Kc[l][b_][i], Vt=Vc[l][b_][i]), proj, own_host=i)
                     down = None
                     if i < F - 1:
-                        down = dict(W=P.act(f"{pre}cross_down.{i}.weight"), bias=P.f32_vec(f"{pre}cross_down.{i}.bias"), **self._norm_params(f"{pre}ln_cross.{i}."))
+                        down = dict(W=P.act(f"{pre}cross_down.{i}.weight"), bias=P.f32_vec(f"{pre}cross_down.{i}.bias"), **(dict(Yact=nd_new[i]) if stored else {}),
+                                    **self._norm_params(f"{pre}ln_cross.{i}."))
+                    extra = [dict(y=y_, proj=entries) for y_, entries in deferred.pop(i, {}).values()]
                     self._chain([dict(att=[att_c[s_] for s_ in range(len(others))], Wp=[P.act(f"{pre}cross_attn.{i}.{j}.projection.weight") for j in others],
                                       W2=P.act(f"{pre}cross_up.{i}.weight"), b2=P.f32_vec(f"{pre}cross_up.{i}.bias"), bias_scale=float(F - 1), Xin=xr[i], X=xr[i],
-                                      down=down, proj=proj)], rope_c, hd_c, f"cross{i}.tail")
+                                      down=down, proj=proj)] + extra, rope_c, hd_c, f"cross{i}.tail")
+                assert not deferred, "every deferred projection entry has a host in front of its reader"
             elif F > 1 and xmode == "sea":
                 self._down_norm(pre, range(F), xa, dn, nd_old, "cross", "_old")
                 for i in range(F):
@@ -847,7 +876,10 @@
                          out=self._mods[lc]) if fm.front3 else None
             memo = dict(stamps=self._buf(M, 2, dtype=torch.int32, zero=True), mods=self._mods[mp], epoch=P.memo_epoch, count=self.memo_count) if fm.cond_memo else None
             if memo is not None and i == 0 and rows is not None:
-                memo["rows"] = self._buf(rows[1] + 1, M, 2, dtype=torch.int32, zero=True)
+                if self._rider_tiles is not None:
+                    memo["rows"], memo["tile_off"] = self._memo_rows, (rows[1] + 1) * M * 2
+                else:
+                    memo["rows"] = self._buf(rows[1] + 1, M, 2, dtype=torch.int32, zero=True)
             ops.fill_adaln_qkv(g_, X=xr[i], cond=None, w1=P.f32_vec(mp + "cond_mlp.0.weight", 2 * E), b1=P.f32_vec(mp + "cond_mlp.0.bias"), W2c=P.act(mp + "cond_mlp.2.weight"),
                                b2c=P.f32_vec(mp + "cond_mlp.2.bias"), gamma=P.f32_vec(mp + "weight"), beta=P.f32_vec(mp + "bias"), Wqkv=P.act(f"{pre}attn.self.{i}.q.weight", 3 * E),
                                bqkv=P.f32_vec(f"{pre}attn.self.{i}.q.bias", 3 * E), Q=Qs[i], K=Ks[i], Vt=Vs[i], ldx=(F * Eo if first else None), third=third, memo=memo)
@@ -1173,6 +1205,10 @@
                 c.op, c.p0, c.n, c.p1, c.f0, c.dtype = N.OP_CHAIN, addr(a[0]), a[1], addr(r.keep[1]), a[8], a[9]
                 c.l0, c.i0, c.i1, c.i2 = addr(a[3]), a[4], a[5], a[6]
                 c.l1 = addr(r.keep[3]) if r.keep[3] is not None else 0
+            elif r.fn is L.sea_row_chain_riders_memo:
+                c.op, c.p0, c.n, c.p1, c.f0, c.dtype = N.OP_CHAIN, addr(a[0]), a[1], addr(r.keep[1]), a[10], a[11]
+                c.l0, c.i0, c.i1, c.i2, c.l2, c.l3 = addr(a[3]), a[4], a[5], a[6], a[8], a[9]
+                c.l1 = addr(r.keep[3]) if r.keep[3] is not None else 0
             elif r.fn is L.sea_gemm_rownorm:
                 c.op, c.p0, c.n, c.f0, c.dtype = N.OP_GEMM_NORM, addr(a[0]), a[1], a[2], a[3]
             elif r.fn is L.sea_rownorm:
diff --git a/sea_amd/ops.py b/sea_amd/ops.py
--- a/sea_amd/ops.py
+++ b/sea_amd/ops.py
@@ -298,6 +298,7 @@
             raise ValueError(f"adaln_qkv memo: stamps {tuple(st.shape)} {st.dtype} / mods {tuple(tab.shape)} do not fit M = {X.shape[0]}, 2E = {W2c.shape[0]}")
         g.memo_stamps, g.memo_mods, g.ldmemo = st.data_ptr(), tab.data_ptr(), tab.stride(0)
         g.memo_epoch, g.memo_count, g.memo_rows = memo["epoch"].data_ptr(), N.ptr(memo.get("count")), N.ptr(memo.get("rows"))
+        g.pad_ = int(memo.get("tile_off", 0))
     g.X, g.ldx, g.cond = X.data_ptr(), (ldx if ldx is not None else X.stride(0)), N.ptr(cond)
     g.w1, g.b1, g.W2c, g.ldw2c, g.b2c = w1.data_ptr(), b1.data_ptr(), W2c.data_ptr(), W2c.stride(0), N.ptr(b2c)
     g.gamma, g.beta, g.Wqkv, g.ldw, g.bqkv = gamma.data_ptr(), N.ptr(beta), Wqkv.data_ptr(), Wqkv.stride(0), N.ptr(bqkv)
@@ -334,8 +335,17 @@
     return dtype == torch.bfloat16 and (D, E) in ((128, 256), (64, 128)) and 0 <= n_seg and n_seg * D <= E and hd in (16, 32)
 
 
-def fill_row_chain(P: N.SeaRowChain, W2, Xin, X, att: Sequence[torch.Tensor] = (), Wp: Sequence[torch.Tensor] = (), a2=None, b2=None, bias_scale: float = 1.0, Xact=None,
-                   down: Optional[Dict] = None, proj: Sequence[Dict] = (), ldxin: Optional[int] = None) -> None:
+def fill_row_chain(P: N.SeaRowChain, W2=None, Xin=None, X=None, att: Sequence[torch.Tensor] = (), Wp: Sequence[torch.Tensor] = (), a2=None, b2=None, bias_scale: float = 1.0,
+                   Xact=None, down: Optional[Dict] = None, proj: Sequence[Dict] = (), ldxin: Optional[int] = None, y=None) -> None:
+    if len(proj) > N.CHAIN_MAX_PROJ:
+        raise ValueError(f"row_chain: {len(proj)} projection entries (at most {N.CHAIN_MAX_PROJ})")
+    if y is not None:
+        if W2 is not None or X is not None or att or a2 is not None or down is not None or not proj:
+            raise ValueError("row_chain: a projection-only group takes y and proj alone")
+        P.n_seg, P.a2, P.lda2 = N.CHAIN_PROJ_ONLY, y.data_ptr(), y.stride(0)
+        P.M, P.D, P.E, P.has_down = y.shape[0], y.shape[1], 2 * y.shape[1], 0
+        _fill_chain_proj(P, proj)
+        return
     for s_, a in enumerate(att):
         P.att[s_] = a.data_ptr()
         P.Wp[s_] = Wp[s_].data_ptr()
@@ -361,8 +371,10 @@
         g.Yact, g.ldyact = N.ptr(yact), (yact.stride(0) if yact is not None else 0)
         g.mean, g.rstd = N.ptr(down.get("mean")), N.ptr(down.get("rstd"))
         g.M, g.N, g.K, g.n_seg = P.M, P.D, P.E, 1
-    if len(proj) > N.CHAIN_MAX_PROJ:
-        raise ValueError(f"row_chain: {len(proj)} projection entries (at most {N.CHAIN_MAX_PROJ})")
+    _fill_chain_proj(P, proj)
+
+
+def _fill_chain_proj(P: N.SeaRowChain, proj: Sequence[Dict]) -> None:
     P.n_proj = len(proj)
     for q, d in zip(P.proj, proj):
         W = d["W"]
diff --git a/sea_amd/plan_forms.py b/sea_amd/plan_forms.py
--- a/sea_amd/plan_forms.py
+++ b/sea_amd/plan_forms.py
@@ -39,6 +39,11 @@
     proj_norm: bool
     splitk: bool
     cond_memo: bool = field(default=False, compare=False)
+    defer_proj: bool = True
+
+    def __post_init__(self):
+        if not self.chain and self.defer_proj:
+            object.__setattr__(self, "defer_proj", False)
 
     @property
     def one_launch_front(self) -> bool:
@@ -105,4 +110,5 @@
         mlp_fc1=mlp_fc1, mlp_norm_in=mlp_norm_in, mlp_block=mlp_block, mlp_fc2_proj=mlp_fc2_proj,
         down_norm=(fuse_norm if inference else kind == TRAINING and sw("norm", "1") != "0") and D <= 256 and D % 16 == 0,
         proj_norm=fuse_norm and Eo <= 256 and Eo % 16 == 0 and Eo == E and sw("projnorm", "1") != "0", splitk=sw("splitk", "1") != "0",
-        cond_memo=front_chain and riders and sw("cond_memo", "1") != "0")
+        cond_memo=front_chain and riders and sw("cond_memo", "1") != "0",
+        defer_proj=chain and sw("defer_proj", "1") != "0")
diff --git a/sea_amd/ptrcheck.py b/sea_amd/ptrcheck.py
--- a/sea_amd/ptrcheck.py
+++ b/sea_amd/ptrcheck.py
@@ -146,7 +146,9 @@
             if st.memo_count:
                 yield "memo_count", st.memo_count, 8
             if st.memo_rows:
-                yield "memo_rows", st.memo_rows, st.M * 8
+                yield "memo_rows", st.memo_rows, max(st.M * 8, (st.pad_ + (st.M + 63) // 64) * 4 if st.pad_ else 0)
+    elif isinstance(st, N.SeaRowChain) and st.n_seg == N.CHAIN_PROJ_ONLY:
+        yield "a2", st.a2, ((st.M - 1) * st.lda2 + st.D) * esz
     elif isinstance(st, N.SeaRowChain):
         K2 = st.D if st.n_seg > 0 else st.E
         for s_ in range(st.n_seg):
@@ -240,8 +242,37 @@
                 yield label, a[k], a[4] * 4
         if isinstance(a[6], int):
             yield "ws", a[6], a[7] * 4
+    elif name == "sea_row_chain_riders_memo":
+        if isinstance(a[8], int) and a[4] > 0:
+            yield "rider_hit", a[8], a[4] * ((a[3][0].M + 63) // 64) * 4
+        if isinstance(a[9], int):
+            yield "rider_count", a[9], 8
     elif name == "sea_ib_bwd_dc" and isinstance(a[1], int) and isinstance(r.keep, N.SeaIbBwdParams):
         yield "dc", a[1], r.keep.M * 4
+
+
+def _chain_outputs(r, esz: int) -> Iterable[Tuple[str, int, int]]:
+    arr = r.args[0] if r.args and isinstance(r.args[0], C.Array) and getattr(r.args[0], "_type_", None) is N.SeaRowChain else None
+    common = next((k for k in (r.keep if isinstance(r.keep, tuple) else ()) if isinstance(k, N.SeaQkvCommon)), None)
+    if arr is None or common is None:
+        return
+    H, hd, T, cap, pos0 = common.H, common.hd, common.T, common.cap, common.pos0
+    for gi in range(r.args[1]):
+        st = arr[gi]
+        if st.n_seg != N.CHAIN_PROJ_ONLY or T <= 0:
+            continue
+        Bn = st.M // T
+        for e in range(st.n_proj):
+            q = st.proj[e]
+            if q.Qout:
+                yield f"[{gi}].proj[{e}].Qout", q.Qout, Bn * H * T * hd * esz
+            slab = (Bn * H - 1) * cap * hd
+            if q.Kout:
+                yield f"[{gi}].proj[{e}].Kout", q.Kout, (slab + (pos0 + T) * hd) * esz
+            if q.Vtout:
+                yield f"[{gi}].proj[{e}].Vtout", q.Vtout, (slab + (hd - 1) * cap + pos0 + T) * esz
+            if q.Vout:
+                yield f"[{gi}].proj[{e}].Vout", q.Vout, (slab + (pos0 + T) * hd) * esz
 
 
 def check_records(records, ranges: Ranges, esz: int, what: str) -> int:
@@ -266,6 +297,11 @@
                     if hit is not None and nbytes > 0 and p + nbytes > hit[1]:
                         raise RuntimeError(f"sea_amd pointer audit ({what}): launch '{r.name}': {type(st).__name__}.{field} = {p:#x} + {nbytes} bytes runs "
                                            f"{p + nbytes - hit[1]} bytes past the end of its buffer ({hit[2]})")
+        for field, p, nbytes in _chain_outputs(r, esz):
+            hit = ranges.find(p)
+            if hit is not None and p + nbytes > hit[1]:
+                raise RuntimeError(f"sea_amd pointer audit ({what}): launch '{r.name}': SeaRowChain{field} = {p:#x} + {nbytes} bytes runs "
+                                   f"{p + nbytes - hit[1]} bytes past the end of its buffer ({hit[2]})")
         for field, p, nbytes in _raw_extents(r, esz):
             hit = ranges.find(p)
             if hit is not None and nbytes > 0 and p + nbytes > hit[1]:
```

After: 4289. 23.2% lower.
